# laurabragagnolo/SkelSplat

Hardware: AMD Instinct MI355X
Metric: rendered+backpropagated views/s (differentiable skeletal-Gaussian rasterizer fwd+bwd) (higher is better)
Workload: dtype f32

## Files before the change

include/skelsplat_hip.h:

```cpp
#ifndef SKELSPLAT_HIP_H
#define SKELSPLAT_HIP_H

#include <stddef.h>
#include <stdint.h>

#ifdef __cplusplus
extern "C" {
#endif

#define SKS_MAX_VIEWS 64
#define SKS_MAX_CHANNELS 32
#define SKS_SMALL_P 256

#define SKS_ANTIALIASING 1u
#define SKS_CLAMP01      2u
#define SKS_FORCE_BINNED 4u
#define SKS_DEBUG_SYNC   8u

#define SKS_NO_NT_STORES 16u

#define SKS_RAW_PARAMS   32u
#define SKS_RAW_GRADS    128u
#define SKS_BIN_CLEAN    64u
#define SKS_BIN_GROUPS_SHIFT 16
#define SKS_BIN_GROUPS(n) ((unsigned)(((n) - 1) & 7) << SKS_BIN_GROUPS_SHIFT)
#define SKS_FILL_LINEAR (1u << 21)
#define SKS_FILL_ROWS (1u << 22)
#define SKS_BWD_LDS_LIST (1u << 20)
#define SKS_BWD_WG_SHIFT 23
#define SKS_NO_EARLY_FILL (1u << 30)
#define SKS_EARLY_FILL(n) (((unsigned)(n) & 7u) << SKS_BIN_GROUPS_SHIFT)

const char* sks_last_error(void);
int sks_version(void);

int sks_scratch_bytes(int V, int P, int C, int W, int H, size_t bin_capacity,
                      size_t* geom_bytes, size_t* binning_bytes, size_t* accum_bytes);

#define SKS_REGIME_PATH        0
#define SKS_REGIME_COVER       1
#define SKS_REGIME_CW          2
#define SKS_REGIME_PPT         3
#define SKS_REGIME_HALF        4
#define SKS_REGIME_ROWMODE     5
#define SKS_REGIME_PB          6
#define SKS_REGIME_FSPLIT      7
#define SKS_REGIME_W_MAGIC     8
#define SKS_REGIME_BWD         9
#define SKS_REGIME_GX         10
#define SKS_REGIME_GY         11
#define SKS_REGIME_BPC        12
#define SKS_REGIME_WAVE_GROUPS 13
#define SKS_REGIME_LEAD       14
#define SKS_REGIME_INTS       16
int sks_launch_regime(int V, int P, int C, int W, int H, unsigned flags, int out_aligned128, int* out);

#define SKS_LIST_WAVE_SORT     0
#define SKS_LIST_WAVE_K        1
#define SKS_LIST_SORT_LDS      2
#define SKS_LIST_LONG_LIST     3
#define SKS_LIST_CLASSES       4
#define SKS_LIST_BAND_THREADS  5
#define SKS_LIST_REGIME_INTS   8
int sks_list_regime(int* out);

int sks_forward(int V, int P, int C, int W, int H,
                const float* viewmatrix, const float* projmatrix,
                const float* tanfovx , const float* tanfovy ,
                const float* means3D, const float* features, const float* opacities,
                const float* scales, const float* rotations, const float* cov3D_precomp,
                float scale_modifier, unsigned flags,
                float* out_color, float* out_invdepth, int* radii,
                void* geom, void* binning, size_t bin_capacity, int* num_rendered_dev,
                float* final_T, uint32_t* n_contrib, void* stream);

int sks_backward(int V, int P, int C, int W, int H,
                 const float* viewmatrix, const float* projmatrix,
                 const float* tanfovx , const float* tanfovy ,
                 const float* bg,
                 const float* means3D, const float* features, const float* opacities,
                 const float* scales, const float* rotations, const float* cov3D_precomp,
                 float scale_modifier, unsigned flags,
                 const int* radii, const void* geom, const void* binning, size_t bin_capacity,
                 const float* dL_dout_color, const float* dL_dout_invdepth,
                 void* accum,
                 float* dL_dmeans3D, float* dL_dmeans2D, float* dL_dopacity,
                 float* dL_dscales, float* dL_drotations, float* dL_dcov3D, float* dL_dfeatures,
                 float* dL_dmeans3D_mean ,
                 void* stream);

int sks_prefill_planes(int V, int P, int C, int W, int H, unsigned flags, int* planes_wave, int* planes_geom);
int sks_forward_prefilled(int V, int P, int C, int W, int H,
                          const float* viewmatrix, const float* projmatrix,
                          const float* tanfovx , const float* tanfovy ,
                          const float* means3D, const float* features, const float* opacities,
                          const float* scales, const float* rotations, const float* cov3D_precomp,
                          float scale_modifier, unsigned flags,
                          float* out_color, float* out_invdepth, int* radii,
                          void* geom, void* binning, size_t bin_capacity, int* num_rendered_dev,
                          float* final_T, uint32_t* n_contrib, int prefilled_planes, void* stream);
int sks_backward_prefill(int V, int P, int C, int W, int H,
                         const float* viewmatrix, const float* projmatrix,
                         const float* tanfovx , const float* tanfovy ,
                         const float* bg,
                         const float* means3D, const float* features, const float* opacities,
                         const float* scales, const float* rotations, const float* cov3D_precomp,
                         float scale_modifier, unsigned flags,
                         const int* radii, const void* geom, const void* binning, size_t bin_capacity,
                         const float* dL_dout_color, const float* dL_dout_invdepth,
                         void* accum,
                         float* dL_dmeans3D, float* dL_dmeans2D, float* dL_dopacity,
                         float* dL_dscales, float* dL_drotations, float* dL_dcov3D, float* dL_dfeatures,
                         float* dL_dmeans3D_mean,
                         float* next_color, float* next_invdepth, int planes_wave, int planes_geom, void* stream);

#define SKS_FB_NO_JOIN 1u
int sks_forward_backward(int V, int P, int C, int W, int H,
                         const float* viewmatrix, const float* projmatrix,
                         const float* tanfovx , const float* tanfovy ,
                         const float* means3D, const float* features, const float* opacities,
                         const float* scales, const float* rotations, const float* cov3D_precomp,
                         float scale_modifier, unsigned flags,
                         float* out_color, float* out_invdepth, int* radii,
                         void* geom, void* binning, size_t bin_capacity, int* num_rendered_dev,
                         const float* bg, const float* dL_dout_color, const float* dL_dout_invdepth, void* accum,
                         float* dL_dmeans3D, float* dL_dmeans2D, float* dL_dopacity,
                         float* dL_dscales, float* dL_drotations, float* dL_dcov3D, float* dL_dfeatures,
                         float* dL_dmeans3D_mean, void* stream, void* aux_stream, unsigned fb_flags);

int sks_mean_views(int V, int P, const float* dL_dmeans3D, int shard_world, float* mean_out , void* stream);

int sks_mark_visible(int P, const float* means3D, const float* viewmatrix, const float* projmatrix,
                     uint8_t* present, void* stream);

int sks_export_lists(int V, int W, int H, const void* binning, size_t bin_capacity,
                     uint32_t* point_list, uint32_t* ranges, void* stream);

int sks_masked_l2(int V, size_t n_per_view, const float* render, const float* gt, float* dL_unscaled, double* sums,
                  void* stream);
int sks_masked_l2_launch(size_t n_per_view, int* out );
int sks_masked_l2_loss(int V, size_t n_per_view, const float* render, const float* gt, float* dL_unscaled, double* sums,
                       float* loss , float* scale , int mean, void* stream);

#define SKS_SOFTARGMAX_STATS 6
size_t sks_softargmax_scratch_bytes(int planes, int W, int H);
int sks_softargmax_fwd(int planes, int W, int H, float beta, const float* img, float* xy ,
                       float* stats , void* scratch, size_t scratch_bytes, void* stream);
int sks_softargmax_bwd(int planes, int W, int H, float beta, const float* img, const float* stats ,
                       const float* dL_dxy , float* dL_dimg, void* stream);

int sks_heatmaps(int V, int J, int W, int H, const float* row, const float* col, const float* cmin, const float* den,
                 float* out, double* gt_totals, void* stream);
#define SKS_HEATMAP_MAX_RADIUS 262144
int sks_heatmap_factors(int V, int J, int W, int H, const float* means3D, const float* scales, const float* rotations,
                        float scale_modifier, const float* poses_2d, const float* viewmatrix, const float* tanfovx,
                        const float* tanfovy, float* row, float* col, float* cmin, float* den,
                        int frames ,
                        const int* view_wh ,
                        void* stream);
int sks_heatmap_totals(int V, int J, int W, int H, const float* row, const float* col, const float* cmin, const float* den,
                       const int* view_wh, double* gt_totals, void* stream);

int sks_triangulate(int N, int V, int J, const double* proj, size_t rig_stride, const float* poses_2d,
                    const double* poses_2d_f64, const unsigned char* valid, float* xyz, double* xyzw, int* n_used,
                    void* stream);

int sks_triangulate_robust(int N, int V, int J, const double* proj, size_t rig_stride, const float* poses_2d,
                           const double* poses_2d_f64, const unsigned char* valid, double reject_px, int min_inliers,
                           unsigned char* inliers, int* n_consensus, float* xyz, double* xyzw, int* n_used, void* stream);

int sks_fuse_predictions(int N, int V, int J, const double* proj, size_t rig_stride, const float* poses_3d,
                         const double* poses_3d_f64, const float* poses_2d, const double* poses_2d_f64,
                         const unsigned char* valid, int norm_f32, float* xyz, double* xyz_f64, double* reproj_err,
                         int* n_used, void* stream);

#define SKS_REFINE_MAX_ITERS 16
int sks_reproject(int N, int V, int J, const double* proj, size_t rig_stride, const float* xyz, const double* xyz_f64,
                  const float* poses_2d, const double* poses_2d_f64, const unsigned char* valid, double* uv, double* err,
                  unsigned char* in_front, double* per_joint, double* per_view, double* per_frame, int* n_used, void* stream);
int sks_eval_reprojection(int N, int V, int J, const double* err, const int* group_ids, int n_groups, double* out, void* stream);
int sks_triangulate_refine(int N, int V, int J, const double* proj, size_t rig_stride, const float* poses_2d,
                           const double* poses_2d_f64, const unsigned char* valid, const float* xyz0, const double* xyz0_f64,
                           double huber_px, int max_iters, float* xyz, double* xyz_f64, double* cost, int* iters, void* stream);

#define SKS_SMOOTH_MAX_JOINTS       256
#define SKS_SMOOTH_MAX_HALF_WINDOW  32
#define SKS_SMOOTH_BOX              0
#define SKS_SMOOTH_TRICUBE          1
#define SKS_SMOOTH_TILE       0
#define SKS_SMOOTH_GROUPS     1
#define SKS_SMOOTH_THREADS    2
#define SKS_SMOOTH_LDS_BYTES  3
#define SKS_SMOOTH_LAUNCH_INTS 4
int sks_smooth_sequence(int N, int J, const float* xyz, const float* cov6, const float* weights, const unsigned char* valid,
                        const int* group_ids, int half_window, int degree, int taper, double cov_floor, float* out_xyz,
                        float* out_vel, float* out_cov6, int* n_used, void* stream);
int sks_smooth_launch(int N, int J, int half_window, int* out );
int sks_eval_accel(int N, int J, const float* xyz, const float* gt, const int* group_ids, int n_groups, double* out, void* stream);

#define SKS_BONES_MAX_JOINTS   32
#define SKS_BONES_MAX_GROUPS   256
#define SKS_BONES_MAX_ITERS    16
#define SKS_BONES_MEASURE_GROUPS     0
#define SKS_BONES_MEASURE_THREADS    1
#define SKS_BONES_LENGTHS_GROUPS     2
#define SKS_BONES_LENGTHS_THREADS    3
#define SKS_BONES_LENGTHS_LDS_BYTES  4
#define SKS_BONES_PROJECT_GROUPS     5
#define SKS_BONES_PROJECT_THREADS    6
#define SKS_BONES_PROJECT_LDS_BYTES  7
#define SKS_BONES_LAUNCH_INTS        8
int sks_bone_measure(int N, int J, int B, const int* bones , const float* xyz, const float* cov6,
                     const unsigned char* valid, double max_sigma_mm, float* measured, void* stream);
int sks_bone_lengths(int N, int B, const float* measured, const int* groups, int n_groups, float* length, float* mad, int* n_used,
                     void* stream);
int sks_bone_project(int N, int J, int B, const int* bones , const float* xyz, const float* cov6,
                     const unsigned char* valid, const int* groups, int n_groups, const float* lengths, double cov_floor,
                     int max_iters, double tol_mm, float* out_xyz, float* residual, int* n_trips, int* n_active, void* stream);
int sks_bones_launch(int N, int J, int B, int n_groups, int* out );

int sks_fused_ssim_fwd(int B, int CH, int H, int W, float C1, float C2, const float* img1, const float* img2,
                       float* ssim_map, float* dm_dmu1, float* dm_dsigma1_sq, float* dm_dsigma12, void* stream);

int sks_fused_ssim_bwd(int B, int CH, int H, int W, float C1, float C2, const float* img1, const float* img2,
                       const float* dL_dmap, const float* dm_dmu1, const float* dm_dsigma1_sq, const float* dm_dsigma12,
                       float* dL_dimg1, void* stream);
int sks_fused_ssim_bwd_uniform(int B, int CH, int H, int W, const float* img1, const float* img2, const float* dL_value,
                               float dL_scale, int crop, const float* dm_dmu1, const float* dm_dsigma1_sq,
                               const float* dm_dsigma12, float* dL_dimg1, void* stream);
#define SKS_SSIM_SUM_SLOTS 64
#define SKS_SSIM_SCRATCH_BYTES (SKS_SSIM_SUM_SLOTS * 8)
int sks_fused_ssim_mean(int B, int CH, int H, int W, float C1, float C2, const float* img1, const float* img2, int crop,
                        float* dm_dmu1, float* dm_dsigma1_sq, float* dm_dsigma12, double* scratch, float* mean_out,
                        void* stream);

int sks_knn3_meandist2(int P, const float* points, float* mean_dist2, void* stream);
size_t sks_knn3_scratch_bytes(int P);
int sks_knn3_meandist2_grid(int P, const float* points, float* mean_dist2, void* scratch, size_t scratch_bytes, void* stream);

int sks_gt_tile_stats(int V, int C, int W, int H, const float* gt, float* tile_S, float* tile_N, double* totals, void* stream);
int sks_geometry(int V, int P, int C, int W, int H, const float* viewmatrix, const float* projmatrix,
                 const float* tanfovx , const float* tanfovy , const float* means3D,
                 const float* opacities, const float* scales, const float* rotations, const float* cov3D_precomp,
                 float scale_modifier, unsigned flags, int* radii, void* geom,
                 const int* view_wh , int frames ,
                 void* stream);
int sks_backward_fused_loss(int V, int P, int C, int W, int H, const float* viewmatrix, const float* projmatrix,
                            const float* tanfovx , const float* tanfovy , const float* bg,
                            const float* means3D, const float* features, const float* opacities, const float* scales,
                            const float* rotations, const float* cov3D_precomp, float scale_modifier, unsigned flags,
                            const int* radii, const void* geom, const float* gt, const float* tile_S, const float* tile_N,
                            const double* gt_totals, void* accum, float* dL_dmeans3D, float* dL_dmeans2D,
                            float* dL_dopacity, float* dL_dscales, float* dL_drotations, float* dL_dcov3D,
                            double* loss_sums, float* packed_raw_grads ,
                            const int* view_wh , const size_t* gt_offsets ,
                            const float* const* hm_factors , void* stream);

int sks_loop_pack_grads(int V, int P, const float* dL_dmeans3D, const float* dL_dscales, const float* dL_drotations,
                        const float* dL_dopacity, const float* raw_scaling, const float* raw_rotation,
                        const float* raw_opacity, const double* loss_sums, float* packed, void* stream);
int sks_loop_adam_step(int V, int P, const float* grads, float* slots, unsigned long long group_mask, int last_view,
                       float* xyz, float* scaling, float* rotation, float* opacity, float* exp_avg, float* exp_avg_sq,
                       int* counters, int acc_steps, const double* lr_sched ,
                       const double* lrs , const double* adam ,
                       float lambda_consistency, const int* limb ,
                       int shard_world ,
                       void* stream);
// ... 154 lines not shown
```

skelsplat_amd/_lib.py:

```python
import ctypes as C
import os

_HERE = os.path.dirname(os.path.abspath(__file__))
LIB_PATH = os.path.join(_HERE, "libskelsplat_hip.so")
_lib = None

SKS_MAX_VIEWS = 64
SKS_MAX_CHANNELS = 32
SKS_SMALL_P = 256
SKS_ANTIALIASING = 1
SKS_CLAMP01 = 2
SKS_FORCE_BINNED = 4
SKS_DEBUG_SYNC = 8
SKS_NO_NT_STORES = 16
SKS_RAW_PARAMS = 32
SKS_BIN_CLEAN = 64
SKS_RAW_GRADS = 128
SKS_FB_NO_JOIN = 1
SKS_BIN_GROUPS_SHIFT = 16
SKS_BWD_WG_SHIFT = 23
SKS_SSIM_SCRATCH_BYTES = 64 * 8
SKS_SOFTARGMAX_STATS = 6
SKS_REPORT_MAX_SAVES = 8
SKS_EVAL_MAX_GROUPS = 64
SKS_CALIBRATION_MAX_K = 8
SKS_REFINE_MAX_ITERS = 16
SKS_SMOOTH_MAX_JOINTS = 256
SKS_SMOOTH_MAX_HALF_WINDOW = 32
SKS_SMOOTH_BOX, SKS_SMOOTH_TRICUBE = 0, 1
SKS_SMOOTH_LAUNCH_INTS = 4
SKS_BONES_MAX_JOINTS = 32
SKS_BONES_MAX_GROUPS = 256
SKS_BONES_MAX_ITERS = 16
SKS_BONES_LAUNCH_INTS = 8
SKS_ALIGN_RIGID, SKS_ALIGN_SIMILARITY, SKS_ALIGN_SCALE = 0, 1, 2
SKS_PREVIEW_LAUNCH_INTS = 4
SKS_HEATMAP_MAX_RADIUS = 1 << 18


SKS_NO_EARLY_FILL = 1 << 30
SKS_BWD_LDS_LIST = 1 << 20
SKS_FILL_LINEAR = 1 << 21
SKS_FILL_ROWS = 1 << 22


def SKS_EARLY_FILL(n):
    return (int(n) & 7) << SKS_BIN_GROUPS_SHIFT


def SKS_BIN_GROUPS(n):
    return ((int(n) - 1) & 7) << SKS_BIN_GROUPS_SHIFT


_vp, _i, _u, _f, _sz = C.c_void_p, C.c_int, C.c_uint, C.c_float, C.c_size_t

_CAMERAS = (("V", _i), ("P", _i), ("C", _i), ("W", _i), ("H", _i), ("viewmatrix", _vp), ("projmatrix", _vp),
            ("tanfovx", _vp), ("tanfovy", _vp))
_GAUSSIANS = (("means3D", _vp), ("features", _vp), ("opacities", _vp), ("scales", _vp), ("rotations", _vp),
              ("cov3D_precomp", _vp), ("scale_modifier", _f), ("flags", _u))
_UPSTREAM = (("dL_dout_color", _vp), ("dL_dout_invdepth", _vp), ("accum", _vp))
_GRADS = (("dL_dmeans3D", _vp), ("dL_dmeans2D", _vp), ("dL_dopacity", _vp), ("dL_dscales", _vp), ("dL_drotations", _vp),
          ("dL_dcov3D", _vp), ("dL_dfeatures", _vp), ("dL_dmeans3D_mean", _vp))
_FORWARD_IO = (("out_color", _vp), ("out_invdepth", _vp), ("radii", _vp), ("geom", _vp), ("binning", _vp),
               ("bin_capacity", _sz), ("num_rendered_dev", _vp))
FORWARD_PARAMS = _CAMERAS + _GAUSSIANS + _FORWARD_IO + (("final_T", _vp), ("n_contrib", _vp), ("stream", _vp))
BACKWARD_PARAMS = _CAMERAS + (("bg", _vp),) + _GAUSSIANS + (("radii", _vp), ("geom", _vp), ("binning", _vp), ("bin_capacity", _sz)) \
    + _UPSTREAM + _GRADS + (("stream", _vp),)
FORWARD_PREFILLED_PARAMS = FORWARD_PARAMS[:-1] + (("prefilled_planes", _i), ("stream", _vp))
BACKWARD_PREFILL_PARAMS = BACKWARD_PARAMS[:-1] + (("next_color", _vp), ("next_invdepth", _vp), ("planes_wave", _i), ("planes_geom", _i),
                                                  ("stream", _vp))
FORWARD_BACKWARD_PARAMS = _CAMERAS + _GAUSSIANS + _FORWARD_IO + (("bg", _vp),) + _UPSTREAM + _GRADS \
    + (("stream", _vp), ("aux_stream", _vp), ("fb_flags", _u))

FWD, BWD, FWD_BWD = ({name: i for i, (name, _) in enumerate(params)}
                     for params in (FORWARD_PARAMS, BACKWARD_PARAMS, FORWARD_BACKWARD_PARAMS))
FWD_BWD_SOURCES = tuple(("fwd", FWD[n]) if n in FWD else ("bwd", BWD[n]) if n in BWD else None for n in FWD_BWD)

_ull = C.c_ulonglong
_VIEWS_DV = (("viewmatrix", _vp), ("projmatrix", _vp), ("views_dev", _vp))
RIG_SELECT_PARAMS = (("R", _i), ("V", _i), ("frames", _i), ("rig_ids", _vp), ("bank_viewmatrix", _vp), ("bank_projmatrix", _vp),
                     ("bank_tan", _vp), ("slot_wh", _vp), ("bank_proj", _vp), ("bank_sched", _vp), ("viewmatrix", _vp),
                     ("projmatrix", _vp), ("views_dev", _vp), ("proj", _vp), ("lr_sched_dev", _vp), ("error_word", _vp),
                     ("stream", _vp))
GEOMETRY_DV_PARAMS = (("V", _i), ("P", _i), ("C", _i), ("W", _i), ("H", _i)) + _VIEWS_DV + (
    ("means3D", _vp), ("opacities", _vp), ("scales", _vp), ("rotations", _vp), ("cov3D_precomp", _vp), ("scale_modifier", _f),
    ("flags", _u), ("radii", _vp), ("geom", _vp), ("frames", _i), ("stream", _vp))
HEATMAP_FACTORS_DV_PARAMS = (("V", _i), ("J", _i), ("W", _i), ("H", _i), ("means3D", _vp), ("scales", _vp), ("rotations", _vp),
                             ("scale_modifier", _f), ("poses_2d", _vp), ("viewmatrix", _vp), ("views_dev", _vp), ("row", _vp),
                             ("col", _vp), ("cmin", _vp), ("den", _vp), ("frames", _i), ("stream", _vp))
HEATMAP_TOTALS_DV_PARAMS = (("V", _i), ("J", _i), ("W", _i), ("H", _i), ("row", _vp), ("col", _vp), ("cmin", _vp), ("den", _vp),
                            ("views_dev", _vp), ("gt_totals", _vp), ("stream", _vp))
OPTIMISER_PARAMS = (("slots", _vp), ("group_mask", _ull), ("last_view", _i), ("xyz", _vp), ("scaling", _vp), ("rotation", _vp),
                    ("opacity", _vp), ("exp_avg", _vp), ("exp_avg_sq", _vp), ("counters", _vp), ("acc_steps", _i),
                    ("lr_sched", _vp), ("lrs", _vp), ("adam", _vp), ("lambda_consistency", _f), ("limb", _vp))
OPTIMISER_DV_PARAMS = tuple(("lr_sched_dev", ct) if name == "lr_sched" else (name, ct) for name, ct in OPTIMISER_PARAMS)
_ES = (("es_state", _vp), ("es_window", _i), ("es_tolerance", _f))
ES_PARAMS, ES_FRAMES_PARAMS = _ES + (("es_host_flag", _vp),), _ES + (("es_host_flags", _vp),)
_ADAM_STEP = (("V", _i), ("P", _i), ("grads", _vp)) + OPTIMISER_PARAMS + (("shard_world", _i),)
_STEP_RENDER = (("features", _vp), ("scale_modifier", _f), ("flags", _u), ("radii", _vp), ("geom", _vp), ("gt", _vp),
                ("gt_totals", _vp), ("accum", _vp), ("loss_sums", _vp), ("packed", _vp))
_STEP_HEATMAPS = (("view_wh", _vp), ("gt_offsets", _vp), ("frames", _i), ("hm_factors", _vp))
_STEP = _CAMERAS + _STEP_RENDER + OPTIMISER_PARAMS + _STEP_HEATMAPS
_STEP_DV = (("V", _i), ("P", _i), ("C", _i), ("W", _i), ("H", _i)) + _VIEWS_DV + _STEP_RENDER + OPTIMISER_DV_PARAMS + _STEP_HEATMAPS
LOOP_ADAM_STEP_PARAMS = _ADAM_STEP + (("stream", _vp),)
LOOP_ADAM_STEP_ES_PARAMS = _ADAM_STEP + (("loss_sums", _vp),) + ES_PARAMS + (("stream", _vp),)
LOOP_FUSED_STEP_PARAMS = _STEP + (("stream", _vp),)
LOOP_FUSED_STEP_ES_PARAMS = _STEP + ES_FRAMES_PARAMS + (("stream", _vp),)
LOOP_FUSED_STEP_DV_PARAMS = _STEP_DV + (("stream", _vp),)
LOOP_FUSED_STEP_ES_DV_PARAMS = _STEP_DV + ES_FRAMES_PARAMS + (("stream", _vp),)
STEP_PARAMS = {"sks_loop_adam_step": LOOP_ADAM_STEP_PARAMS, "sks_loop_adam_step_es": LOOP_ADAM_STEP_ES_PARAMS,
               "sks_loop_fused_step": LOOP_FUSED_STEP_PARAMS, "sks_loop_fused_step_es": LOOP_FUSED_STEP_ES_PARAMS}
DV_PARAMS = {"sks_rig_select": RIG_SELECT_PARAMS, "sks_geometry_dv": GEOMETRY_DV_PARAMS,
             "sks_heatmap_factors_dv": HEATMAP_FACTORS_DV_PARAMS, "sks_heatmap_totals_dv": HEATMAP_TOTALS_DV_PARAMS,
             "sks_loop_fused_step_dv": LOOP_FUSED_STEP_DV_PARAMS, "sks_loop_fused_step_es_dv": LOOP_FUSED_STEP_ES_DV_PARAMS}
VW_PARAMS = (("vw_mode", _i), ("vw_threshold", _f), ("vw_weights", _vp), ("vw_similarity", _vp))
VW_MODES = {None: 0, "scale": 1, "select": 2}
LOOP_ADAM_STEP_VW_PARAMS = LOOP_ADAM_STEP_ES_PARAMS[:-1] + VW_PARAMS + (("stream", _vp),)
LOOP_FUSED_STEP_VW_PARAMS = LOOP_FUSED_STEP_ES_PARAMS[:-1] + VW_PARAMS + (("stream", _vp),)
LOOP_FUSED_STEP_VW_DV_PARAMS = LOOP_FUSED_STEP_ES_DV_PARAMS[:-1] + VW_PARAMS + (("stream", _vp),)
VW_STEP_PARAMS = {"sks_loop_adam_step_vw": LOOP_ADAM_STEP_VW_PARAMS, "sks_loop_fused_step_vw": LOOP_FUSED_STEP_VW_PARAMS,
                  "sks_loop_fused_step_vw_dv": LOOP_FUSED_STEP_VW_DV_PARAMS}


def vw_mode(view_weighting):
    if view_weighting not in VW_MODES:
        raise ValueError(f"view_weighting = {view_weighting!r}: expected None, 'scale' or 'select'")
    return VW_MODES[view_weighting]


SIGNATURES = {
    "sks_last_error": (C.c_char_p, []),
    "sks_version": (_i, []),
    "sks_scratch_bytes": (_i, [_i, _i, _i, _i, _i, _sz, C.POINTER(_sz), C.POINTER(_sz), C.POINTER(_sz)]),
    "sks_launch_regime": (_i, [_i, _i, _i, _i, _i, _u, _i, C.POINTER(_i)]),
    "sks_list_regime": (_i, [C.POINTER(_i)]),
    "sks_forward": (_i, [ct for _, ct in FORWARD_PARAMS]),
    "sks_backward": (_i, [ct for _, ct in BACKWARD_PARAMS]),
    "sks_forward_backward": (_i, [ct for _, ct in FORWARD_BACKWARD_PARAMS]),
    "sks_forward_prefilled": (_i, [ct for _, ct in FORWARD_PREFILLED_PARAMS]),
    "sks_backward_prefill": (_i, [ct for _, ct in BACKWARD_PREFILL_PARAMS]),
    "sks_prefill_planes": (_i, [_i, _i, _i, _i, _i, _u, C.POINTER(_i), C.POINTER(_i)]),
    "sks_mark_visible": (_i, [_i, _vp, _vp, _vp, _vp, _vp]),
    "sks_mean_views": (_i, [_i, _i, _vp, _i, _vp, _vp]),
    "sks_export_lists": (_i, [_i, _i, _i, _vp, _sz, _vp, _vp, _vp]),
    "sks_masked_l2": (_i, [_i, _sz, _vp, _vp, _vp, _vp, _vp]),
    "sks_masked_l2_launch": (_i, [_sz, C.POINTER(_i)]),
    "sks_masked_l2_loss": (_i, [_i, _sz, _vp, _vp, _vp, _vp, _vp, _vp, _i, _vp]),
    "sks_fused_ssim_fwd": (_i, [_i, _i, _i, _i, _f, _f, _vp, _vp, _vp, _vp, _vp, _vp, _vp]),
    "sks_fused_ssim_bwd": (_i, [_i, _i, _i, _i, _f, _f, _vp, _vp, _vp, _vp, _vp, _vp, _vp, _vp]),
    "sks_fused_ssim_bwd_uniform": (_i, [_i, _i, _i, _i, _vp, _vp, _vp, _f, _i, _vp, _vp, _vp, _vp, _vp]),
    "sks_fused_ssim_mean": (_i, [_i, _i, _i, _i, _f, _f, _vp, _vp, _i, _vp, _vp, _vp, _vp, _vp, _vp]),
    "sks_knn3_meandist2": (_i, [_i, _vp, _vp, _vp]),
    "sks_knn3_scratch_bytes": (_sz, [_i]),
    "sks_knn3_meandist2_grid": (_i, [_i, _vp, _vp, _vp, _sz, _vp]),
    "sks_softargmax_scratch_bytes": (_sz, [_i, _i, _i]),
    "sks_softargmax_fwd": (_i, [_i, _i, _i, _f, _vp, _vp, _vp, _vp, _sz, _vp]),
    "sks_softargmax_bwd": (_i, [_i, _i, _i, _f, _vp, _vp, _vp, _vp, _vp]),
    "sks_heatmaps": (_i, [_i, _i, _i, _i, _vp, _vp, _vp, _vp, _vp, _vp, _vp]),
    "sks_heatmap_factors": (_i, [_i, _i, _i, _i, _vp, _vp, _vp, _f, _vp, _vp, _vp, _vp, _vp, _vp, _vp, _vp, _i, _vp, _vp]),
    "sks_heatmap_totals": (_i, [_i, _i, _i, _i, _vp, _vp, _vp, _vp, _vp, _vp, _vp]),
    "sks_gt_tile_stats": (_i, [_i, _i, _i, _i, _vp, _vp, _vp, _vp, _vp]),
    "sks_geometry": (_i, [_i, _i, _i, _i, _i, _vp, _vp, _vp, _vp, _vp, _vp, _vp, _vp, _vp, _f, _u, _vp, _vp, _vp, _i, _vp]),
    "sks_backward_fused_loss": (_i, [_i, _i, _i, _i, _i, _vp, _vp, _vp, _vp, _vp, _vp, _vp, _vp, _vp, _vp, _vp, _f, _u,
                                     _vp, _vp, _vp, _vp, _vp, _vp, _vp, _vp, _vp, _vp, _vp, _vp, _vp, _vp, _vp, _vp, _vp, _vp, _vp]),
    "sks_loop_pack_grads": (_i, [_i, _i, _vp, _vp, _vp, _vp, _vp, _vp, _vp, _vp, _vp, _vp]),
    "sks_loop_shard_floats": (_sz, [_i, _i, _i]),
    "sks_adam_multi": (_i, [_i, _vp, _vp, _vp, _vp, _vp, _vp, _vp, C.c_double, C.c_double, C.c_double, _vp]),
    "sks_triangulate": (_i, [_i, _i, _i, _vp, _sz, _vp, _vp, _vp, _vp, _vp, _vp, _vp]),
    "sks_triangulate_robust": (_i, [_i, _i, _i, _vp, _sz, _vp, _vp, _vp, C.c_double, _i, _vp, _vp, _vp, _vp, _vp, _vp]),
    "sks_fuse_predictions": (_i, [_i, _i, _i, _vp, _sz, _vp, _vp, _vp, _vp, _vp, _i, _vp, _vp, _vp, _vp, _vp]),
    "sks_reproject": (_i, [_i, _i, _i, _vp, _sz, _vp, _vp, _vp, _vp, _vp, _vp, _vp, _vp, _vp, _vp, _vp, _vp, _vp]),
    "sks_eval_reprojection": (_i, [_i, _i, _i, _vp, _vp, _i, _vp, _vp]),
    "sks_triangulate_refine": (_i, [_i, _i, _i, _vp, _sz, _vp, _vp, _vp, _vp, _vp, C.c_double, _i, _vp, _vp, _vp, _vp, _vp]),
    "sks_smooth_sequence": (_i, [_i, _i, _vp, _vp, _vp, _vp, _vp, _i, _i, _i, C.c_double, _vp, _vp, _vp, _vp, _vp]),
    "sks_smooth_launch": (_i, [_i, _i, _i, _vp]),
    "sks_eval_accel": (_i, [_i, _i, _vp, _vp, _vp, _i, _vp, _vp]),
    "sks_bone_measure": (_i, [_i, _i, _i, _vp, _vp, _vp, _vp, C.c_double, _vp, _vp]),
    "sks_bone_lengths": (_i, [_i, _i, _vp, _vp, _i, _vp, _vp, _vp, _vp]),
    "sks_bone_project": (_i, [_i, _i, _i, _vp, _vp, _vp, _vp, _vp, _i, _vp, C.c_double, _i, C.c_double, _vp, _vp, _vp, _vp, _vp]),
    "sks_bones_launch": (_i, [_i, _i, _i, _i, _vp]),
    **{name: (_i, [ct for _, ct in params]) for name, params in {**STEP_PARAMS, **DV_PARAMS, **VW_STEP_PARAMS}.items()},
    "sks_pose_errors": (_i, [_i, _i, _vp, _vp, _vp, _vp, _vp]),
    "sks_loop_report": (_i, [_i, _i, _i, _vp, _vp, _i, _vp, _vp, _vp, _i, _i, _vp, _vp, _vp, _i, _vp, _vp, _vp]),
    "sks_eval_sequence": (_i, [_i, _i, _vp, _vp, _vp, _i, _vp, _vp, _vp]),
    "sks_joint_uncertainty": (_i, [_i, _i, _vp, _vp, _vp, _f, _vp, _vp, _vp, _vp, _vp]),
    "sks_view_footprints": (_i, [_i, _i, _i, _i, _vp, _vp, _vp, _f, _vp, _vp, _vp, _vp, _vp, _i, _vp, _vp]),
    "sks_calibration": (_i, [_i, _i, _vp, _vp, _i, _vp, _vp, _vp]),
    "sks_align_poses": (_i, [_i, _i, _vp, _vp, _vp, _i, _vp, _vp, _vp, _vp, _vp]),
    "sks_eval_sequence_aligned": (_i, [_i, _i, _vp, _vp, _vp, _vp, _i, _vp, _sz, _vp, _vp]),
    "sks_eval_sequence_aligned_scratch_bytes": (_sz, [_i, _i]),
    "sks_preview_planes": (_i, [_i, _i, _i, _i, _vp, _vp, _vp, _vp, _vp]),
    "sks_preview_factors": (_i, [_i, _i, _i, _i, _vp, _vp, _vp, _vp, _vp, _vp, _vp, _vp, _vp]),
    "sks_preview_scratch_bytes": (_sz, [_i, _i, _i]),
    "sks_preview_launch": (_i, [_i, _i, _i, _vp]),
    "sks_prof_enable": (_i, [_i]),
    "sks_prof_spin": (_i, [C.c_double, _vp]),
    "sks_prof_read": (_i, [_i, C.POINTER(C.c_double), C.POINTER(C.c_longlong)]),
    "sks_prof_count": (_i, [_i, C.POINTER(C.c_longlong)]),
    "sks_prof_read_quantiles": (_i, [_i, C.POINTER(C.c_double), C.POINTER(C.c_double), C.POINTER(C.c_longlong)]),
}


_PREFILL_SYMBOLS = ("sks_forward_prefilled", "sks_backward_prefill", "sks_prefill_planes")
HAS_PREFILL = True


def load(build_if_missing=True):
    global _lib
    if _lib is not None:
        return _lib
    if build_if_missing:
        try:
            from . import build as _b
            if _b._stale():
                _b.build()
        except Exception as e:
            if not os.path.exists(LIB_PATH):
                raise ImportError(f"libskelsplat_hip.so is missing and could not be built: {e}") from e
    if not os.path.exists(LIB_PATH):
        raise ImportError(f"{LIB_PATH} not found; run `python -m skelsplat_amd.build`")
    override = os.environ.get("SKS_LIB_OVERRIDE")
    lib = C.CDLL(override or LIB_PATH)
    global HAS_PREFILL
    for name, (res, args) in SIGNATURES.items():
        if override and name in _PREFILL_SYMBOLS and not hasattr(lib, name):
            HAS_PREFILL = False
            continue
        if override and name in VW_STEP_PARAMS and not hasattr(lib, name):
            continue
        fn = getattr(lib, name)
        fn.restype = res
        fn.argtypes = args
    _lib = lib
    return lib


def check(rc, what):
    if rc != 0:
        msg = load().sks_last_error().decode(errors="replace")
        raise RuntimeError(f"{what} failed (code {rc}): {msg}")


def scratch_bytes(V, P, C_, W, H, bin_capacity=0):
    g, b, a = _sz(0), _sz(0), _sz(0)
    check(load().sks_scratch_bytes(V, P, C_, W, H, bin_capacity, C.byref(g), C.byref(b), C.byref(a)), "sks_scratch_bytes")
    return g.value, b.value, a.value


REGIME_FIELDS = ("path", "cover", "cw", "ppt", "half", "rowmode", "pb", "fsplit", "w_magic", "bwd", "gx", "gy", "bpc", "wave_groups",
                 "lead")
REGIME_INTS = 16
PATH_SMALL, PATH_BINNED = 0, 1
COVER_NONE, COVER_PER_VIEW, COVER_PER_PLANE = 0, 1, 2
BWD_WAVE, BWD_GATHER, BWD_TILE = 0, 1, 2


def launch_regime(V, P, C_, W, H, flags=0, out_aligned128=True):
    out = (_i * REGIME_INTS)()
    check(load().sks_launch_regime(V, P, C_, W, H, flags, 1 if out_aligned128 else 0, out), "sks_launch_regime")
    return {name: out[i] for i, name in enumerate(REGIME_FIELDS)}


LIST_REGIME_FIELDS = ("wave_sort", "wave_k", "sort_lds", "long_list", "classes", "band_threads")
LIST_REGIME_INTS = 8


def list_regime():
    out = (_i * LIST_REGIME_INTS)()
    check(load().sks_list_regime(out), "sks_list_regime")
    return {name: out[i] for i, name in enumerate(LIST_REGIME_FIELDS)}


def masked_l2_launch(n_per_view):
    out = (_i * 2)()
    check(load().sks_masked_l2_launch(n_per_view, out), "sks_masked_l2_launch")
    return out[0], out[1]


PREVIEW_LAUNCH_FIELDS = ("load_bytes", "store_bytes", "groups_sum", "groups_pack")


def preview_launch(W, H, aligned=True):
    out = (_i * SKS_PREVIEW_LAUNCH_INTS)()
    check(load().sks_preview_launch(W, H, 1 if aligned else 0, C.cast(out, _vp)), "sks_preview_launch")
    return {name: out[i] for i, name in enumerate(PREVIEW_LAUNCH_FIELDS)}


SMOOTH_LAUNCH_FIELDS = ("tile", "groups", "threads", "lds_bytes")


def smooth_launch(N, J, half_window):
    out = (_i * SKS_SMOOTH_LAUNCH_INTS)()
    check(load().sks_smooth_launch(N, J, half_window, C.cast(out, _vp)), "sks_smooth_launch")
    return {name: out[i] for i, name in enumerate(SMOOTH_LAUNCH_FIELDS)}


BONES_LAUNCH_FIELDS = ("measure_groups", "measure_threads", "lengths_groups", "lengths_threads", "lengths_lds_bytes",
                       "project_groups", "project_threads", "project_lds_bytes")


def bones_launch(N, J, B, n_groups=1):
    out = (_i * SKS_BONES_LAUNCH_INTS)()
    check(load().sks_bones_launch(N, J, B, n_groups, C.cast(out, _vp)), "sks_bones_launch")
    return {name: out[i] for i, name in enumerate(BONES_LAUNCH_FIELDS)}


def prefill_planes(V, P, C_, W, H, flags=0):
    nw, ng = _i(0), _i(0)
    check(load().sks_prefill_planes(V, P, C_, W, H, flags, C.byref(nw), C.byref(ng)), "sks_prefill_planes")
    return nw.value, ng.value


def ptr(t):
    if t is None or t.numel() == 0:
        return None
    return t.data_ptr()


def farray(vals):
    return (C.c_float * len(vals))(*[float(v) for v in vals])


def prof_count(kind):
    n = C.c_longlong(0)
    check(load().sks_prof_count(kind, C.byref(n)), "sks_prof_count")
    return n.value


def prof_enable(on, every=1, kinds=(0, 1), recorded=False):
    skip = sum(1 << (16 + k) for k in (0, 1) if k not in kinds)
    check(load().sks_prof_enable((min(0xffff, max(1, int(every))) | skip | ((1 << 18) if recorded else 0)) if on else 0),
          "sks_prof_enable")


def prof_read_quantiles(kind):
    q = (C.c_double * 3)()
    ms, n = C.c_double(0), C.c_longlong(0)
    check(load().sks_prof_read_quantiles(kind, q, C.byref(ms), C.byref(n)), "sks_prof_read_quantiles")
    return ms.value, n.value, (q[0], q[1], q[2])


def prof_read(kind):
    ms, n = C.c_double(0), C.c_longlong(0)
    check(load().sks_prof_read(kind, C.byref(ms), C.byref(n)), "sks_prof_read")
    return ms.value, n.value
```

skelsplat_amd/csrc/sks_common.inc:

```
thread_local char g_err[512] = "";

int fail(int code, const char* fmt, ...)
{
    va_list ap;
    va_start(ap, fmt);
    vsnprintf(g_err, sizeof(g_err), fmt, ap);
    va_end(ap);
    return code;
}

#define HIP_TRY(expr)                                                                          \
    do {                                                                                       \
        hipError_t e_ = (expr);                                                                \
        if (e_ != hipSuccess) return fail((int)e_, "%s: %s", #expr, hipGetErrorString(e_));    \
    } while (0)

#define STAGE_CHECK(name)                                                                      \
    do {                                                                                       \
        HIP_TRY(hipGetLastError());                                                            \
        if (flags & SKS_DEBUG_SYNC) {                                                          \
            hipError_t e_ = hipStreamSynchronize(st);                                          \
            if (e_ != hipSuccess) return fail((int)e_, "stage %s: %s", name, hipGetErrorString(e_)); \
        }                                                                                      \
    } while (0)

constexpr int PROF_MAX = 16384;
struct ProfKind {
    hipEvent_t b[PROF_MAX], e[PROF_MAX];
    int created = 0, n = 0;
    hipEvent_t xb[PROF_MAX], xe[PROF_MAX];
    bool hasx[PROF_MAX];
    int xcreated = 0;
};
struct ProfState {
    bool on = false;
    int every = 1;
    int skip = 0;
    bool recorded = false;
    int seen[2] = { 0, 0 };
    ProfKind kind[2];
    hipEvent_t park_b = nullptr, park_e = nullptr;
    bool parked = false;
    hipStream_t park_st = nullptr;
};
thread_local ProfState* tl_prof = nullptr;

struct ProfScope {
    ProfKind* k = nullptr;
    hipStream_t st;
    bool ext;
    bool began = false;
    ProfScope(int kind, hipStream_t s, bool ext_ = false, bool take_parked = false) : st(s), ext(ext_)
    {
        ProfState* ps = tl_prof;
        if (!ps) return;
        const bool parked = kind == 0 && ps->parked && take_parked && ps->park_st == s;
        if (kind == 0) ps->parked = false;
        if (!ps->on || ((ps->skip >> kind) & 1)) return;
        if (ps->seen[kind]++ % ps->every != 0) return;
        ProfKind& p = ps->kind[kind];
        if (p.n >= PROF_MAX) return;
        if (p.n >= p.created) {
            if (hipEventCreate(&p.b[p.created]) != hipSuccess || hipEventCreate(&p.e[p.created]) != hipSuccess) return;
            p.created++;
        }
        p.hasx[p.n] = false;
        if (parked) {
            while (p.xcreated <= p.n) {
                if (hipEventCreate(&p.xb[p.xcreated]) != hipSuccess || hipEventCreate(&p.xe[p.xcreated]) != hipSuccess) return;
                p.xcreated++;
            }
            hipEvent_t t = p.xb[p.n]; p.xb[p.n] = ps->park_b; ps->park_b = t;
            t = p.xe[p.n]; p.xe[p.n] = ps->park_e; ps->park_e = t;
            p.hasx[p.n] = true;
        }
        k = &p;
        if (ps->recorded) ext = false;
        if (!ext) (void)hipEventRecord(p.b[p.n], st);
    }
    hipEvent_t eb() const { return k->b[k->n]; }
    hipEvent_t ee() const { return k->e[k->n]; }
    ~ProfScope()
    {
        if (!k) return;
        if (!ext) (void)hipEventRecord(k->e[k->n], st);
        k->n++;
    }
};
inline bool prof_next_forward_sampled()
{
    const ProfState* ps = tl_prof;
    return ps && ps->on && !(ps->skip & 1) && ps->seen[0] % ps->every == 0 && ps->kind[0].n < PROF_MAX;
}
inline bool prof_has_parked(hipStream_t st) { return tl_prof && tl_prof->parked && tl_prof->park_st == st; }
inline void prof_park_begin(hipStream_t st)
{
    ProfState* ps = tl_prof;
    ps->parked = false;
    if (!ps->park_b && (hipEventCreate(&ps->park_b) != hipSuccess || hipEventCreate(&ps->park_e) != hipSuccess)) { ps->park_b = ps->park_e = nullptr; return; }
    ps->park_st = st;
    ps->parked = hipEventRecord(ps->park_b, st) == hipSuccess;
}
inline void prof_park_end(hipStream_t st)
{
    ProfState* ps = tl_prof;
    if (ps && ps->parked && ps->park_st == st && hipEventRecord(ps->park_e, st) != hipSuccess) ps->parked = false;
}
inline hipError_t prof_elapsed(ProfKind& p, int i, float* ms)
{
    hipError_t e = hipEventSynchronize(p.e[i]);
    if (e == hipSuccess) e = hipEventElapsedTime(ms, p.b[i], p.e[i]);
    if (e == hipSuccess && p.hasx[i]) {
        float x = 0;
        e = hipEventSynchronize(p.xe[i]);
        if (e == hipSuccess) e = hipEventElapsedTime(&x, p.xb[i], p.xe[i]);
        *ms += x;
    }
    return e;
}
#define SKS_LAUNCH(prof, kernel, grid, block, lds, stream, ...)                                                  \
    do {                                                                                                         \
        if ((prof).k)                                                                                            \
            hipExtLaunchKernelGGL(kernel, grid, block, lds, stream, (prof).began ? nullptr : (prof).eb(), (prof).ee(), 0, __VA_ARGS__); \
        else hipLaunchKernelGGL(kernel, grid, block, lds, stream, __VA_ARGS__);                                  \
    } while (0)
#define SKS_LAUNCH_FIRST(prof, kernel, grid, block, lds, stream, ...)                                            \
    do {                                                                                                         \
        if ((prof).k && (prof).ext) hipExtLaunchKernelGGL(kernel, grid, block, lds, stream, (prof).eb(), nullptr, 0, __VA_ARGS__); \
        else hipLaunchKernelGGL(kernel, grid, block, lds, stream, __VA_ARGS__);    \
        (prof).began = (prof).k != nullptr;                                                                      \
    } while (0)

constexpr int NACC = 8;
constexpr int BWD_SPLITS = 16;
constexpr int BWD_WG_PAIRS16 = 400;
constexpr int BWD_WG_PAIRS8 = 4096;

struct ViewTan {
    float x[SKS_MAX_VIEWS];
    float y[SKS_MAX_VIEWS];
    int w[SKS_MAX_VIEWS];
    int h[SKS_MAX_VIEWS];
};
struct ViewOff {
    unsigned long long off[SKS_MAX_VIEWS];
};
struct ViewTanDev {
    const float* x;
    const float* y;
    const int* w;
    const int* h;
    const double* sched;
};
inline ViewTanDev views_dev_from(const void* views_dev, const double* sched = nullptr)
{
    const ViewTan* t = (const ViewTan*)views_dev;
    return ViewTanDev{ t->x, t->y, t->w, t->h, sched };
}
inline bool fill_views(ViewTan& vt, ViewOff* vo, int V, int C, int W, int H, const float* tanfovx, const float* tanfovy,
                       const int* view_wh, const size_t* plane_off)
{
    for (int v = 0; v < V; v++) {
        vt.x[v] = tanfovx[v];
        vt.y[v] = tanfovy[v];
        vt.w[v] = view_wh ? view_wh[2 * v] : W;
        vt.h[v] = view_wh ? view_wh[2 * v + 1] : H;
        if (vt.w[v] < 1 || vt.h[v] < 1 || vt.w[v] > W || vt.h[v] > H) return false;
        if (vo) vo->off[v] = plane_off ? (unsigned long long)plane_off[v] : (unsigned long long)v * C * H * W;
    }
    return true;
}

struct Geom {
    float4* co;
    float4* xyd;
    uint4* rect;
    uint32_t* cover;
};

__host__ __device__ inline size_t align256(size_t x) { return (x + 255) & ~(size_t)255; }

struct Activated {
    float opacity, s[3], q[4], qnorm;
};
__device__ __forceinline__ Activated activate(bool raw, float op, const float s[3], const float q[4])
{
    Activated a;
    if (raw) {
        a.opacity = 1.0f / (1.0f + expf_fixed(-op));
#pragma unroll
        for (int k = 0; k < 3; k++) a.s[k] = expf_fixed(s[k]);
        const float nn = q[0] * q[0] + q[1] * q[1] + q[2] * q[2] + q[3] * q[3];
        a.qnorm = fmaxf(sqrtf(nn), 1e-12f);
#pragma unroll
        for (int k = 0; k < 4; k++) a.q[k] = q[k] / a.qnorm;
    } else {
        a.opacity = op;
        a.qnorm = 1.0f;
#pragma unroll
        for (int k = 0; k < 3; k++) a.s[k] = s[k];
#pragma unroll
        for (int k = 0; k < 4; k++) a.q[k] = q[k];
    }
    return a;
}

#ifndef SKS_COVER_MAX_WORDS
#define SKS_COVER_MAX_WORDS 6144
#endif
constexpr int COVER_MAX_WORDS = SKS_COVER_MAX_WORDS;
__host__ __device__ inline int cover_cw(int W) { return (1 + (((W + TILE - 1) / TILE) + 31) / 32 + 3) & ~3; }
inline bool cover_enabled(int P, int W, int H)
{
    return P <= SKS_SMALL_P && ((H + TILE - 1) / TILE) * cover_cw(W) <= COVER_MAX_WORDS;
}
inline bool cover_per_plane(int P, int W, int H, int C)
{
    return cover_enabled(P, W, H) && (C + 1) * ((H + TILE - 1) / TILE) * cover_cw(W) <= COVER_MAX_WORDS;
}
inline Geom geom_from(void* base, int V, int P, int W, int H)
{
    char* p = (char*)base;
    Geom g;
    size_t n = (size_t)V * P;
    g.co = (float4*)p; p += align256(n * sizeof(float4));
    g.xyd = (float4*)p; p += align256(n * sizeof(float4));
    g.rect = (uint4*)p; p += align256(n * sizeof(uint4));
    g.cover = cover_enabled(P, W, H) ? (uint32_t*)p : nullptr;
    return g;
}
inline size_t geom_bytes(int V, int P, int W, int H, int C)
{
    const int planes = cover_per_plane(P, W, H, C) ? C + 1 : 1;
    return 3 * align256((size_t)V * P * 16) + align256((size_t)V * planes * ((H + TILE - 1) / TILE) * cover_cw(W) * 4);
}

constexpr int BIN_WAVE_SORT = 64;
constexpr int WSORT_K = 4;
constexpr int SORT_LDS = 2048;
constexpr int LONG_LIST = 256;
constexpr int BIN_ROWS = 2;
constexpr int BIN_CLASSES = 8;
constexpr int BIN_HDR_CLASS = 8;
constexpr int BIN_MAX_GROUPS = 7;
#ifndef SKS_BIN_FB_GROUPS
#define SKS_BIN_FB_GROUPS 1
#endif
constexpr int BIN_FB_GROUPS = SKS_BIN_FB_GROUPS;
inline int bin_groups_default()
{
    static const int n = [] {
        const char* e = getenv("SKS_BIN_GROUPS");
        const int want = (e && atoi(e) > 0) ? atoi(e) : BIN_FB_GROUPS;
        return want < 1 ? 1 : (want > BIN_MAX_GROUPS ? BIN_MAX_GROUPS : want);
    }();
    return n;
}
inline void bin_groups(unsigned flags, int V, int& vg, int& ng)
{
    const unsigned field = (flags >> SKS_BIN_GROUPS_SHIFT) & 7u;
// ... 60 lines not shown
```

skelsplat_amd/csrc/sks_fwd_small.inc:

```
__device__ __forceinline__ float clamp01(float x) { return fminf(fmaxf(x, 0.0f), 1.0f); }

struct FwdArgs {
    int P, C, W, H;
    unsigned flags;
    Geom g;
    const float* features;
    float* out_color;
    float* out_invdepth;
    float* final_T;
    uint32_t* n_contrib;
    int tslots;
    unsigned cp1_magic;
    int ncomp;
    int cover_planes;
    unsigned w_magic;
};

inline int composite_slots(unsigned flags, int V, int P)
{
    const int t = (int)((flags >> 26) & 15u);
    return t ? t : ((long long)V * P <= 128 ? 4 : 8);
}

typedef float v4f __attribute__((ext_vector_type(4)));
// ... 256 lines not shown
            if (tid == 0) { s_n = 0; s_min = 0x7fffffff; }
            __syncthreads();
            if (tid < P) {
                const uint4 r = L.rect[tid];
                if ((int)r.x <= tx && tx < (int)r.z && (int)r.y <= ty && ty < (int)r.w) {
                    atomicMin(&s_min, tid);
                    const int sl = atomicAdd(&s_n, 1);
                    L.key[sl] = ((unsigned long long)__float_as_uint(gxyd[tid].z) << 32) | (unsigned)tid;
                }
            }
            __syncthreads();
            const int n = s_n;
            if (s_min == g) {
                if (tid < n) {
                    const unsigned long long key = L.key[tid];
                    int rank = 0;
                    for (int j = 0; j < n; j++) rank += (L.key[j] < key) ? 1 : 0;
                    const int id = (int)(unsigned)key;
                    const float4 xyd = gxyd[id];
                    L.xy[rank] = make_float2(xyd.x, xyd.y);
                    L.co[rank] = gco[id];
                    L.invd[rank] = xyd.w;
#pragma unroll
                    for (int ch = 0; ch < CG; ch++) L.feat[rank * CG + ch] = ch < C ? a.features[id * C + ch] : 0.0f;
                }
                __syncthreads();
                unsigned chm = 0xffffffffu;
                if (a.cover_planes) {
                    bool nz = false;
                    if (tid < CG)
                        for (int k = 0; k < n; k++) nz = nz || L.feat[k * CG + tid] != 0.0f;
                    if (tid < 64) {
                        const unsigned long long bl = __ballot(nz);
                        if (tid == 0) s_chm = (unsigned)bl;
                    }
                    __syncthreads();
                    chm = s_chm;
                }
                const int x = tx * TILE + (tid & 15), y = ty * TILE + (tid >> 4);
                if (x < W && y < H) {
                    const float pxf = (float)x, pyf = (float)y;
                    float T = 1.0f, inv = 0.0f, acc[CG];
#pragma unroll
                    for (int ch = 0; ch < CG; ch++) acc[ch] = 0.0f;
                    uint32_t contributor = 0, last = 0;
                    for (int k = 0; k < n; k++) {
                        contributor++;
                        const float2 xy = L.xy[k];
                        const float4 co = L.co[k];
                        const float dx = xy.x - pxf, dy = xy.y - pyf;
                        const float power = -0.5f * (co.x * dx * dx + co.z * dy * dy) - co.y * dx * dy;
                        if (power > 0.0f) continue;
                        const float alpha = fminf(0.99f, co.w * expf_fixed(power));
                        if (alpha < 1.0f / 255.0f) continue;
                        const float test_T = T * (1 - alpha);
                        if (test_T < 0.0001f) break;
#pragma unroll
                        for (int ch = 0; ch < CG; ch++) acc[ch] += L.feat[k * CG + ch] * alpha * T;
                        inv += L.invd[k] * alpha * T;
                        T = test_T;
                        last = contributor;
                    }
                    const size_t pix = (size_t)y * W + x;
#pragma unroll
                    for (int ch = 0; ch < CG; ch++)
                        if (ch < C && ((chm >> ch) & 1u)) outc[(size_t)ch * HW + pix] = do_clamp ? clamp01(acc[ch]) : acc[ch];
                    outi[pix] = inv;
                    if (a.final_T) a.final_T[(size_t)v * HW + pix] = T;
                    if (a.n_contrib) a.n_contrib[(size_t)v * HW + pix] = last;
                }
            }
            __syncthreads();
        }
        return;
    }
    fwd_fill_role<PPT, NT, HALF>(a, cp1_magic, xq, band_id, zid, gy, pb, cover);
}

struct EarlyFill {
    float* out_color;
    float* out_invdepth;
    int C, W, H, gy;
    int gplanes;
    int ngeom;
    int zid0;
    int fsplit, pb;
    unsigned cp1_magic;
    unsigned row_magic;
    unsigned fs_magic;
};

template <int PPT, bool NT>
__global__ __launch_bounds__(256) void k_geom_fwd_fill(EarlyFill f, int P, ViewTan vt, const float* __restrict__ vms,
                                                       const float* __restrict__ pms, const float* __restrict__ means,
                                                       const float* __restrict__ opac, const float* __restrict__ scales,
                                                       const float* __restrict__ rots, const float* __restrict__ cov3Dp, float smod,
                                                       unsigned flags, Geom g, int* __restrict__ radii,
                                                       const float* __restrict__ features, int cover_planes)
{
    const int b = blockIdx.x;
    if (b < f.ngeom) {
        const int v = f.gplanes == 1 ? b : (int)(((unsigned)b * f.cp1_magic) >> 20);
        extern __shared__ __attribute__((aligned(16))) char s_dyn[];
        geom_fwd_block((uint32_t*)s_dyn, 0, v, b - v * f.gplanes, P, f.W, f.H, vt, vms, pms, means, opac, scales, rots, cov3Dp, smod, flags, g, radii, 0,
                       nullptr, nullptr, features, f.C, nullptr, nullptr, cover_planes);
        return;
    }
    const unsigned e = (unsigned)(b - f.ngeom);
    const unsigned rows = (unsigned)(f.fsplit * f.gy);
    const unsigned zr = f.row_magic ? __umulhi(e, f.row_magic) : e;
    const unsigned rem = e - zr * rows;
    const int band = (int)(f.fs_magic ? __umulhi(rem, f.fs_magic) : rem);
    const int q = (int)rem - band * f.fsplit;
    const int zid = f.zid0 + (int)zr;
    const int v = (int)(((unsigned)zid * f.cp1_magic) >> 20);
    const int plane = zid - v * (f.C + 1);
    const size_t HW = (size_t)f.H * f.W;
    const int Nb = min(TILE, f.H - band * TILE) * f.W;
    float* out = (plane == f.C ? f.out_invdepth + (size_t)v * HW : f.out_color + ((size_t)v * f.C + plane) * HW) + (size_t)band * TILE * f.W;
    const int shift = (int)((reinterpret_cast<uintptr_t>(out) >> 2) & 31u);
    fill_bare<PPT, NT>(out, nullptr, nullptr, q * (256 * PPT) * f.pb + (int)threadIdx.x * PPT - shift, Nb, min(f.pb, 32));
}

struct PreFill {
    float* out_color;
    float* out_invdepth;
    int C, W, H, gy;
    int zid0;
    unsigned nfill;
    int fsplit, pb;
    int zs;
    unsigned cp1_magic;
    unsigned row_magic;
    unsigned fs_magic;
};

__device__ __forceinline__ void prefill_block(const PreFill& f, unsigned e)
{
    if (e >= f.nfill) return;
    const unsigned rows = (unsigned)(f.fsplit * f.gy);
    const unsigned zr = f.row_magic ? __umulhi(e, f.row_magic) : e;
    const unsigned rem = e - zr * rows;
    const int band = (int)(f.fs_magic ? __umulhi(rem, f.fs_magic) : rem);
    const int q = (int)rem - band * f.fsplit;
    const int zid = f.zid0 + (int)zr;
    const int v = (int)(((unsigned)zid * f.cp1_magic) >> 20);
    const int plane = zid - v * (f.C + 1);
    const size_t HW = (size_t)f.H * f.W;
    const int Nb = min(TILE, f.H - band * TILE) * f.W;
    float* out = (plane == f.C ? f.out_invdepth + (size_t)v * HW : f.out_color + ((size_t)v * f.C + plane) * HW) + (size_t)band * TILE * f.W;
    const int shift = (int)((reinterpret_cast<uintptr_t>(out) >> 2) & 31u);
    fill_bare<4, true>(out, nullptr, nullptr, q * 1024 * f.pb + (int)threadIdx.x * 4 - shift, Nb, min(f.pb, 32));
}
```

skelsplat_amd/csrc/sks_geom_fwd.inc:

```
template <class VT>
__device__ __forceinline__ uint4 geom_fwd_one(int P, const VT& vt, const float* __restrict__ vms,
                                              const float* __restrict__ pms, const float* __restrict__ means,
                                              const float* __restrict__ opac, const float* __restrict__ scales,
                                              const float* __restrict__ rots, const float* __restrict__ cov3Dp,
                                              float smod, unsigned flags, const Geom& g, int* __restrict__ radii,
                                              int v, int idx, bool live, bool store = true)
{
    const size_t o = (size_t)v * P + (live ? idx : 0);
    const float* V = vms + 16 * v;
    const float* PM = pms + 16 * v;
    const float tan_fovx = vt.x[v], tan_fovy = vt.y[v];
    const int W = vt.w[v], H = vt.h[v];
    const float focal_y = H / (2.0f * tan_fovy);
    const float focal_x = W / (2.0f * tan_fovx);
    const int gx = (W + TILE - 1) / TILE, gy = (H + TILE - 1) / TILE;

    int radius_out = 0;
    uint4 rect = make_uint4(0, 0, 0, 0);
    float4 co = make_float4(0, 0, 0, 0), xyd = make_float4(0, 0, 1.0f, 1.0f);

    const int li = live ? idx : 0;
    const float p_orig[3] = { means[3 * li], means[3 * li + 1], means[3 * li + 2] };
    float p_view[3];
    transformPoint4x3(p_orig, V, p_view);
    const bool culled = !(p_view[2] > 0.2f);
    if (live && !culled) {
        float p_hom[4];
        transformPoint4x4(p_orig, PM, p_hom);
        const float p_w = 1.0f / (p_hom[3] + 0.0000001f);
        const float p_proj[3] = { p_hom[0] * p_w, p_hom[1] * p_w, p_hom[2] * p_w };
        float cov3D[6];
        if (cov3Dp) {
#pragma unroll
            for (int i = 0; i < 6; i++) cov3D[i] = cov3Dp[6 * li + i];
        } else {
            const float s[3] = { scales[3 * li], scales[3 * li + 1], scales[3 * li + 2] };
            const float q[4] = { rots[4 * li], rots[4 * li + 1], rots[4 * li + 2], rots[4 * li + 3] };
            const Activated ac = activate(flags & SKS_RAW_PARAMS, 0.0f, s, q);
            computeCov3D(ac.s, smod, ac.q, cov3D);
        }
        Cov2D c;
        cov2d(p_orig, focal_x, focal_y, tan_fovx, tan_fovy, cov3D, V, c);
        float cov_x = c.cov.m[0][0], cov_y = c.cov.m[0][1], cov_z = c.cov.m[1][1];
        constexpr float h_var = 0.3f;
        const float det_cov = cov_x * cov_z - cov_y * cov_y;
        cov_x += h_var;
        cov_z += h_var;
        const float det_cov_plus_h_cov = cov_x * cov_z - cov_y * cov_y;
        float h_convolution_scaling = 1.0f;
        if (flags & SKS_ANTIALIASING) h_convolution_scaling = sqrtf(fmaxf(0.000025f, det_cov / det_cov_plus_h_cov));
        const float det = det_cov_plus_h_cov;
        if (det != 0.0f) {
            const float det_inv = 1.f / det;
            const float conic[3] = { cov_z * det_inv, -cov_y * det_inv, cov_x * det_inv };
            const float mid = 0.5f * (cov_x + cov_z);
            const float lambda1 = mid + sqrtf(fmaxf(0.1f, mid * mid - det));
            const float lambda2 = mid - sqrtf(fmaxf(0.1f, mid * mid - det));
            const float my_radius = ceilf(3.f * sqrtf(fmaxf(lambda1, lambda2)));
            const float px = ndc2Pix(p_proj[0], W), py = ndc2Pix(p_proj[1], H);
            int xmin, ymin, xmax, ymax;
            getRect(px, py, (int)my_radius, gx, gy, xmin, ymin, xmax, ymax);
            if ((xmax - xmin) * (ymax - ymin) != 0) {
                radius_out = (int)my_radius;
                rect = make_uint4(xmin, ymin, xmax, ymax);
                const float op_raw = opac[li];
                const float op = (flags & SKS_RAW_PARAMS) ? 1.0f / (1.0f + expf_fixed(-op_raw)) : op_raw;
                co = make_float4(conic[0], conic[1], conic[2], op * h_convolution_scaling);
                xyd = make_float4(px, py, p_view[2], 1 / p_view[2]);
            }
        }
    }
    if (live && store) {
        radii[o] = radius_out;
        g.co[o] = co;
        g.xyd[o] = xyd;
        g.rect[o] = rect;
    }
    return rect;
}

#ifndef SKS_GEOM_COVER_THREADS
#define SKS_GEOM_COVER_THREADS 256
#endif
__device__ __forceinline__ void geom_fwd_block(uint32_t* s_cov, int bx, int v, int pz, int P, int W, int H, const ViewTan& vt, const float* __restrict__ vms,
                                               const float* __restrict__ pms, const float* __restrict__ means,
                                               const float* __restrict__ opac, const float* __restrict__ scales,
                                               const float* __restrict__ rots, const float* __restrict__ cov3Dp,
                                               float smod, unsigned flags, const Geom& g, int* __restrict__ radii, int vf,
                                               uint32_t* __restrict__ count, uint32_t* __restrict__ touched,
                                               const float* __restrict__ features, int C,
                                               uint2* __restrict__ fmask, uint32_t* __restrict__ bin_hdr, int cover_planes)
{
    const int idx = bx * blockDim.x + threadIdx.x;
    const bool live = idx < P;
    if (vf > 0) {
        const int fr = v / vf;
        means += (size_t)fr * P * 3;
        opac += (size_t)fr * P;
        if (scales) scales += (size_t)fr * P * 3;
        if (rots) rots += (size_t)fr * P * 4;
        if (cov3Dp) cov3Dp += (size_t)fr * P * 6;
    }
    const uint4 rect = geom_fwd_one(P, vt, vms, pms, means, opac, scales, rots, cov3Dp, smod, flags, g, radii, v, idx, live, pz == 0);
    if (bin_hdr && bx == 0 && v == 0 && pz == 0 && threadIdx.x < 64) bin_hdr[threadIdx.x] = 0u;
    if (count) {
        const int wt = (int)(rect.z - rect.x), n = wt * (int)(rect.w - rect.y);
        if (live) touched[(size_t)v * P + idx] = (uint32_t)n;
        if (live && v == 0) {
            unsigned fm = 0u;
            float f0 = 0.0f;
            for (int ch = C - 1; ch >= 0; ch--) {
                const float f = features[(size_t)idx * C + ch];
                if (f != 0.0f) { fm |= 1u << ch; f0 = f; }
            }
            fmask[idx] = make_uint2(fm, __float_as_uint(f0));
        }
    }
    if (g.cover) {
        const int gy = (H + TILE - 1) / TILE;
        const int cw = cover_cw(W), pw = gy * cw;
        for (int i = threadIdx.x; i < pw; i += blockDim.x) s_cov[i] = 0u;
        __syncthreads();
        bool mine = live && rect.z > rect.x && rect.w > rect.y;
        if (mine && cover_planes && pz < C) mine = features[(size_t)idx * C + pz] != 0.0f;
        if (mine) {
#pragma nounroll
            for (unsigned y = rect.y; y < rect.w; y++) {
                atomicOr(&s_cov[y * cw], 1u);
#pragma nounroll
                for (unsigned w0 = rect.x >> 5; w0 <= (rect.z - 1u) >> 5; w0++) {
                    const unsigned lo = max(rect.x, w0 << 5) & 31u, hi = min(rect.z - 1u, (w0 << 5) + 31u) & 31u;
                    atomicOr(&s_cov[y * cw + 1 + w0], (0xffffffffu >> (31u - hi)) & (0xffffffffu << lo));
                }
            }
        }
        __syncthreads();
        uint32_t* out = g.cover + ((size_t)v * (cover_planes ? C + 1 : 1) + (cover_planes ? pz : 0)) * pw;
        for (int i = threadIdx.x; i < pw; i += blockDim.x) out[i] = s_cov[i];
    }
}

__global__ __launch_bounds__(SKS_GEOM_COVER_THREADS > 256 ? SKS_GEOM_COVER_THREADS : 256) void k_geom_fwd(int P, int W, int H, ViewTan vt, const float* __restrict__ vms,
                                                   const float* __restrict__ pms, const float* __restrict__ means,
                                                   const float* __restrict__ opac, const float* __restrict__ scales,
                                                   const float* __restrict__ rots, const float* __restrict__ cov3Dp,
                                                   float smod, unsigned flags, Geom g, int* __restrict__ radii, int vf,
                                                   uint32_t* __restrict__ count = nullptr, uint32_t* __restrict__ touched = nullptr,
                                                   const float* __restrict__ features = nullptr, int C = 0,
                                                   uint2* __restrict__ fmask = nullptr, uint32_t* __restrict__ bin_hdr = nullptr,
                                                   int cover_planes = 0)
{
    __shared__ uint32_t s_cov[COVER_MAX_WORDS];
    geom_fwd_block(s_cov, blockIdx.x, blockIdx.y, blockIdx.z, P, W, H, vt, vms, pms, means, opac, scales, rots, cov3Dp, smod, flags, g, radii, vf,
                   count, touched, features, C, fmask, bin_hdr, cover_planes);
}

__global__ __launch_bounds__(256) void k_geom_fwd_dv(int P, ViewTanDev vt, const float* __restrict__ vms, const float* __restrict__ pms,
                                                      const float* __restrict__ means, const float* __restrict__ opac,
                                                      const float* __restrict__ scales, const float* __restrict__ rots,
                                                      const float* __restrict__ cov3Dp, float smod, unsigned flags, Geom g,
                                                      int* __restrict__ radii, int vf)
{
    const int idx = blockIdx.x * 256 + threadIdx.x;
    const int v = blockIdx.y;
    if (vf > 0) {
        const int fr = v / vf;
        means += (size_t)fr * P * 3;
        opac += (size_t)fr * P;
        if (scales) scales += (size_t)fr * P * 3;
        if (rots) rots += (size_t)fr * P * 4;
        if (cov3Dp) cov3Dp += (size_t)fr * P * 6;
    }
    geom_fwd_one(P, vt, vms, pms, means, opac, scales, rots, cov3Dp, smod, flags, g, radii, v, idx, idx < P);
}

__global__ void k_mark_visible(int P, const float* __restrict__ means, const float* __restrict__ V,
                               uint8_t* __restrict__ present)
{
    const int idx = blockIdx.x * 256 + threadIdx.x;
    if (idx >= P) return;
    const float p[3] = { means[3 * idx], means[3 * idx + 1], means[3 * idx + 2] };
    float pv[3];
    transformPoint4x3(p, V, pv);
    const bool culled = !(pv[2] > 0.2f);
    present[idx] = !culled;
}
```

skelsplat_amd/csrc/sks_raster.hip:

```cpp
#include <hip/hip_runtime.h>
#include <hip/hip_ext.h>
#include <stdarg.h>
#include <stdlib.h>
#include <stdio.h>
#include <string.h>
#include <initializer_list>
#include <type_traits>

#include "../../include/skelsplat_hip.h"
#include "sks_math.h"
#include "sks_loop_dev.h"

using namespace sks;

namespace {

#include "sks_common.inc"
#include "sks_geom_fwd.inc"
#include "sks_fwd_small.inc"
#include "sks_bwd_small.inc"
#include "sks_geom_bwd.inc"
#include "sks_binned.inc"

inline int pick_cg(int C) { return C <= 4 ? 4 : C <= 16 ? 16 : C <= 20 ? 20 : 32; }
// ... 99 lines not shown
void launch_fwd_small(const FwdArgs& a_in, int V, int gy, int zfill, hipStream_t st, const ProfScope& prof)
{
    FwdArgs a = a_in;
    const int ncomp = a.tslots * a.P * V;
    a.ncomp = ncomp;
    int fsplit, pb;
    fill_geometry(a, a.g.cover != nullptr, false, fsplit, pb);
    if (zfill == 0) fsplit = 0;
    const int rows_zy = (zfill > 0 ? zfill : 1) * gy;
    const int xc = (ncomp + rows_zy - 1) / rows_zy;
    const int cap = (a.P + 15) & ~15;
    const size_t lds = DynList<CG>::bytes(cap, CG);
    dim3 grid(fsplit + xc, gy, zfill > 0 ? zfill : 1);
    const bool nt = !(a.flags & SKS_NO_NT_STORES);
    if (a.W % 4 == 0) {
        if (nt) SKS_LAUNCH(prof, (k_render_fwd_sparse<CG, 4, true>), grid, dim3(256), lds, st, a, a.cp1_magic, gy, fsplit, pb, (const uint32_t*)a.g.cover);
        else SKS_LAUNCH(prof, (k_render_fwd_sparse<CG, 4, false>), grid, dim3(256), lds, st, a, a.cp1_magic, gy, fsplit, pb, (const uint32_t*)a.g.cover);
    } else if (fill_half_mode(a)) {
        SKS_LAUNCH(prof, (k_render_fwd_sparse<CG, 4, true, true>), grid, dim3(256), lds, st, a, a.cp1_magic, gy, fsplit, pb, (const uint32_t*)a.g.cover);
    } else {
        SKS_LAUNCH(prof, (k_render_fwd_sparse<CG, 1, false>), grid, dim3(256), lds, st, a, a.cp1_magic, gy, fsplit, pb, (const uint32_t*)a.g.cover);
    }
}

#ifndef SKS_EARLY_FILL_BYTES
#define SKS_EARLY_FILL_BYTES (36u << 20)
#endif
inline int early_fill_planes(unsigned flags, int planes, size_t plane_bytes)
{
    const int field = (int)((flags >> SKS_BIN_GROUPS_SHIFT) & 7u);
    if (field == 7) return planes;
    if (field) return (planes * field + 15) / 16;
    const size_t want = ((size_t)SKS_EARLY_FILL_BYTES + plane_bytes / 2) / plane_bytes;
    return (int)(want < (size_t)(planes / 4) ? want : (size_t)(planes / 4));
}

inline unsigned magic32(unsigned d) { return (unsigned)(((1ull << 32) + d - 1) / d); }

bool early_fill_cut(const FwdArgs& a_in, int V, int gy, int gplanes, int zid0, int zid1, int& fsplit, int& pb)
{
    FwdArgs a = a_in;
    a.flags |= SKS_FILL_LINEAR;
    fill_geometry(a, true, false, fsplit, pb);
    const long long rows = (long long)fsplit * gy, nfill = rows * (zid1 - zid0);
    return fsplit >= 1 && pb >= 1 && nfill * rows < (1ll << 32) && (long long)V * gplanes + nfill < (1ll << 31);
}

void launch_geom_fill(const FwdArgs& a, const FwdCall& c, int gy, int gplanes, int zid0, int zid1, int fsplit, int pb, const ViewTan& vt,
                      ProfScope& prof)
{
    const hipStream_t st = c.stream;
    const long long rows = (long long)fsplit * gy, nfill = rows * (zid1 - zid0);
    const int ngeom = c.cam.V * gplanes;
    const EarlyFill f{ a.out_color, a.out_invdepth, a.C, a.W, a.H, gy, gplanes, ngeom, zid0, fsplit, pb, a.cp1_magic,
                       rows > 1 ? magic32((unsigned)rows) : 0u, fsplit > 1 ? magic32((unsigned)fsplit) : 0u };
    const dim3 grid((unsigned)(ngeom + nfill));
    const size_t lds = (size_t)gy * cover_cw(a.W) * 4;
    const bool nt = !(a.flags & SKS_NO_NT_STORES);
    const int ppt = (a.W % 4 == 0 || fill_half_mode(a)) ? 4 : 1;
#define SKS_GF_ARGS f, a.P, vt, c.cam.viewmatrix, c.cam.projmatrix, c.g.means3D, c.g.opacities, c.g.scales, c.g.rotations, c.g.cov3D_precomp, \
                    c.g.scale_modifier, a.flags, a.g, c.io.radii, a.features, a.cover_planes
    if (ppt == 4 && nt) SKS_LAUNCH_FIRST(prof, (k_geom_fwd_fill<4, true>), grid, dim3(256), lds, st, SKS_GF_ARGS);
    else if (ppt == 4) SKS_LAUNCH_FIRST(prof, (k_geom_fwd_fill<4, false>), grid, dim3(256), lds, st, SKS_GF_ARGS);
    else SKS_LAUNCH_FIRST(prof, (k_geom_fwd_fill<1, false>), grid, dim3(256), lds, st, SKS_GF_ARGS);
#undef SKS_GF_ARGS
}

#ifndef SKS_GEOM_BINNED_THREADS
#define SKS_GEOM_BINNED_THREADS 256
#endif
void launch_geom_fwd(const FwdCall& c, const ViewTan& vt, const Geom& g, const Bin& b, bool small, int gplanes, hipEvent_t done)
{
    const Cameras& cam = c.cam;
    const int gthreads = small ? 256 : SKS_GEOM_BINNED_THREADS;
    const dim3 grid((cam.P + gthreads - 1) / gthreads, cam.V, gplanes);
#define SKS_G_ARGS cam.P, cam.W, cam.H, vt, cam.viewmatrix, cam.projmatrix, c.g.means3D, c.g.opacities, c.g.scales, c.g.rotations, c.g.cov3D_precomp, \
                   c.g.scale_modifier, c.g.flags, g, c.io.radii, 0, b.count, b.touched, c.g.features, cam.C, b.fmask, b.hdr,                          \
                   (small && cover_per_plane(cam.P, cam.W, cam.H, cam.C)) ? 1 : 0
    if (done) hipExtLaunchKernelGGL(k_geom_fwd, grid, dim3(gthreads), 0, c.stream, nullptr, done, 0, SKS_G_ARGS);
    else hipLaunchKernelGGL(k_geom_fwd, grid, dim3(gthreads), 0, c.stream, SKS_G_ARGS);
#undef SKS_G_ARGS
}

template <int CG>
void launch_fwd_binned(const FwdArgs& a, const BinView& bv, int V, int gx, int gy, const uint32_t* cover, hipStream_t st)
{
    int fsplit, pb;
    fill_geometry(a, true, true, fsplit, pb);
    const int xc = ((gx + TGROUP - 1) / TGROUP + a.C) / (a.C + 1);
    dim3 grid(fsplit + xc, gy, (a.C + 1) * V);
    const bool nt = !(a.flags & SKS_NO_NT_STORES);
    if (a.W % 4 == 0) {
        if (nt) hipLaunchKernelGGL((k_render_fwd_binned<CG, 4, true>), grid, dim3(256), 0, st, a, bv, gx, gy, fsplit, pb, cover);
        else hipLaunchKernelGGL((k_render_fwd_binned<CG, 4, false>), grid, dim3(256), 0, st, a, bv, gx, gy, fsplit, pb, cover);
    } else if (fill_half_mode(a)) {
        hipLaunchKernelGGL((k_render_fwd_binned<CG, 4, true, true>), grid, dim3(256), 0, st, a, bv, gx, gy, fsplit, pb, cover);
    } else {
        hipLaunchKernelGGL((k_render_fwd_binned<CG, 1, false>), grid, dim3(256), 0, st, a, bv, gx, gy, fsplit, pb, cover);
    }
}

inline int bin_scan_bands(int gx) { return gx >= SCAN_T * 8 ? 1 : (SCAN_T * 8) / gx; }

inline int bwd_tile_blocks()
{
    static const int n = [] {
        int dev = 0, cus = 256;
        if (hipGetDevice(&dev) == hipSuccess) {
            hipDeviceProp_t pr;
            if (hipGetDeviceProperties(&pr, dev) == hipSuccess && pr.multiProcessorCount > 0) cus = pr.multiProcessorCount;
        }
        const char* e = getenv("SKS_BWD_TILE_BLOCKS");
        return (e && atoi(e) > 0) ? atoi(e) : cus * BWD_TILE_BLOCKS_PER_CU;
    }();
    return n;
}

inline int bwd_wave_groups(int V, int P, unsigned flags)
{
    unsigned t = (flags >> SKS_BWD_WG_SHIFT) & 7u;
    static const int env = [] { const char* e = getenv("SKS_BWD_WG"); return e ? atoi(e) : 0; }();
    if (!t && env > 0) t = (unsigned)env;
    if (t) return t > 5 ? 1 : (BWD_SPLITS >> (t - 1));
    const int pairs = V * P;
    return pairs <= BWD_WG_PAIRS16 ? 16 : (pairs <= BWD_WG_PAIRS8 ? 8 : 4);
}

template <bool ES = false>
inline void launch_bwd_loss(const BwdArgs& a, const ViewTan& vt, const ViewOff& vo, int V, hipStream_t st)
{
    const dim3 grid(a.P, V, bwd_wave_groups(V, a.P, a.flags));
    if (a.hm_row) with_cg(a.C, [&](auto cg) { hipLaunchKernelGGL((k_render_bwd_wave<decltype(cg)::value, false, true, true, ES>), grid, dim3(256), 0, st, a, vt, vo); });
    else with_cg(a.C, [&](auto cg) { hipLaunchKernelGGL((k_render_bwd_wave<decltype(cg)::value, false, true, false, ES>), grid, dim3(256), 0, st, a, vt, vo); });
}

struct PrefillReq {
    float* color;
    float* invdepth;
    int planes_wave, planes_geom;
};
#ifndef SKS_PREFILL_PASSES
#define SKS_PREFILL_PASSES 2
#endif
inline int prefill_passes()
{
    static const int n = [] { const char* e = getenv("SKS_PREFILL_PB"); return (e && atoi(e) > 0) ? atoi(e) : SKS_PREFILL_PASSES; }();
    return n > 32 ? 32 : n;
}
inline bool prefill_possible(int P, int W, int H, unsigned flags)
{
    return P >= 1 && P <= 64 && is_small(P, flags) && !(flags & (SKS_NO_NT_STORES | SKS_DEBUG_SYNC | SKS_BWD_LDS_LIST)) &&
           (W % 4 == 0 || (W % 4 == 2 && H % 2 == 0));
}
bool prefill_cut(PreFill& f, float* color, float* invdepth, int V, int C, int W, int H, int zid0, int nz, long long per_unit, long long max_units)
{
    const int gy = TileGrid(W, H).gy;
    const int passes = (TILE * W + fill_lead(color, invdepth, W, H) + 1023) / 1024;
    const int pb = prefill_passes();
    const int fsplit = (passes + pb - 1) / pb;
    const long long rows = (long long)fsplit * gy, nfill = rows * nz;
    if (zid0 < 0 || nz < 1 || zid0 + nz > (C + 1) * V || nfill * rows >= (1ll << 32) || (nfill + per_unit - 1) / per_unit > max_units) return false;
    f = PreFill{ color, invdepth, C, W, H, gy, zid0, (unsigned)nfill, fsplit, pb, 0, ((1u << 20) + (unsigned)C) / (unsigned)(C + 1),
                 rows > 1 ? magic32((unsigned)rows) : 0u, fsplit > 1 ? magic32((unsigned)fsplit) : 0u };
    return true;
}

inline bool bwd_small_wave(int P, unsigned flags) { return P <= 64 && !(flags & SKS_BWD_LDS_LIST); }

template <int CG>
void launch_bwd_small(const BwdArgs& a, const ViewTan& vt, const ViewOff& vo, int V, bool dfeat, hipStream_t st, const ProfScope& prof,
                      const PreFill* pf = nullptr)
{
    if (bwd_small_wave(a.P, a.flags)) {
        dim3 grid(a.P, V, bwd_wave_groups(V, a.P, a.flags));
        if (pf) {
            PreFill f = *pf;
            f.zs = (int)grid.z;
            grid.z += (unsigned)((f.nfill + (unsigned)(a.P * V) - 1) / (unsigned)(a.P * V));
            if (dfeat) SKS_LAUNCH(prof, (k_render_bwd_wave<CG, true, false, false, false, PreFill>), grid, dim3(256), 0, st, a, vt, vo, f);
            else SKS_LAUNCH(prof, (k_render_bwd_wave<CG, false, false, false, false, PreFill>), grid, dim3(256), 0, st, a, vt, vo, f);
            return;
        }
        if (dfeat) SKS_LAUNCH(prof, (k_render_bwd_wave<CG, true, false>), grid, dim3(256), 0, st, a, vt, vo);
        else SKS_LAUNCH(prof, (k_render_bwd_wave<CG, false, false>), grid, dim3(256), 0, st, a, vt, vo);
        return;
    }
    dim3 grid(a.P, V, BWD_SPLITS);
    const size_t lds = GatherLds<CG>::bytes((a.P + 15) & ~15, CG, a.C);
    if (lds > 48 * 1024) {
        (void)hipFuncSetAttribute(reinterpret_cast<const void*>(&k_render_bwd_gather<CG, true>),
                                  hipFuncAttributeMaxDynamicSharedMemorySize, (int)lds);
        (void)hipFuncSetAttribute(reinterpret_cast<const void*>(&k_render_bwd_gather<CG, false>),
                                  hipFuncAttributeMaxDynamicSharedMemorySize, (int)lds);
    }
    if (dfeat) SKS_LAUNCH(prof, (k_render_bwd_gather<CG, true>), grid, dim3(256), lds, st, a);
    else SKS_LAUNCH(prof, (k_render_bwd_gather<CG, false>), grid, dim3(256), lds, st, a);
}

__global__ void k_spin_us(unsigned long long ticks)
{
    const unsigned long long t0 = wall_clock64();
    while (wall_clock64() - t0 < ticks) __builtin_amdgcn_s_sleep(8);
}

struct FwdHook {
    hipEvent_t geom_done;
    int (*after_geom)(void* ctx);
    int (*after_group)(void* ctx, int g, int v0, int nv);
    void* ctx;
};
constexpr int FB_MAX_EVENTS = BIN_MAX_GROUPS;
constexpr int FB_OVERLAP_MAX_PAIRS = BWD_WG_PAIRS16;
struct FbEvents {
    hipEvent_t geom = nullptr, done = nullptr;
    hipEvent_t grp[FB_MAX_EVENTS] = {};
    int dev = -1;
};
thread_local FbEvents tl_fb_events;
int fb_events(int ngroups, FbEvents*& out)
{
    FbEvents& ev = tl_fb_events;
    int cur_dev = 0;
    HIP_TRY(hipGetDevice(&cur_dev));
    if (ev.geom && ev.dev != cur_dev) {
        (void)hipEventDestroy(ev.geom);
        (void)hipEventDestroy(ev.done);
        for (hipEvent_t& e : ev.grp)
            if (e) { (void)hipEventDestroy(e); e = nullptr; }
        ev.geom = ev.done = nullptr;
    }
    unsigned evf = hipEventDisableTiming | hipEventDisableSystemFence;
    if (const char* e = getenv("SKS_FB_EVENT_FLAGS")) evf = (unsigned)strtoul(e, nullptr, 0);
    if (!ev.geom) {
        ev.dev = cur_dev;
        HIP_TRY(hipEventCreateWithFlags(&ev.geom, evf));
        HIP_TRY(hipEventCreateWithFlags(&ev.done, evf));
    }
    for (int gi = 0; gi < ngroups && gi < FB_MAX_EVENTS; gi++)
        if (!ev.grp[gi]) HIP_TRY(hipEventCreateWithFlags(&ev.grp[gi], evf));
    out = &ev;
    return 0;
}

}

extern "C" {

const char* sks_last_error(void) { return g_err; }
void sks_set_error_(const char* msg)
{
    snprintf(g_err, sizeof(g_err), "%s", msg);
}
int sks_version(void) { return 14; }

int sks_scratch_bytes(int V, int P, int C, int W, int H, size_t bin_capacity, size_t* geom, size_t* binning, size_t* accum)
{
    if (int rc = check_common(V, P, C, W, H)) return rc;
    const TileGrid t(W, H);
    if (geom) *geom = geom_bytes(V, P > 0 ? P : 1, W, H, C);
    if (binning) *binning = bin_bytes(V, P, t.NT, bin_capacity, C + 1, (size_t)t.gy * cover_cw(W));
    if (accum) *accum = (size_t)V * (P > 0 ? P : 1) * BWD_SPLITS * (NACC + C) * sizeof(float);
    return 0;
}

int sks_launch_regime(int V, int P, int C, int W, int H, unsigned flags, int out_aligned128, int* out)
{
    if (int rc = check_common(V, P, C, W, H)) return rc;
    if (!out) return fail(-2, "sks_launch_regime: out must be provided");
    const TileGrid t(W, H);
    const bool small = is_small(P, flags);
    const bool cover = small && cover_enabled(P, W, H), per_plane = cover && cover_per_plane(P, W, H, C);
    FwdArgs a{};
    a.P = P, a.C = C, a.W = W, a.H = H, a.flags = flags;
    a.out_color = a.out_invdepth = (float*)(uintptr_t)(out_aligned128 ? 128 : 16);
    int fsplit = 0, pb = 0;
    fill_geometry(a, small ? cover : true, !small, fsplit, pb);
    const int ppt = (W % 4 == 0 || fill_half_mode(a)) ? 4 : 1;
    memset(out, 0, SKS_REGIME_INTS * sizeof(int));
    out[SKS_REGIME_PATH] = small ? 0 : 1;
    out[SKS_REGIME_COVER] = small ? (per_plane ? 2 : cover ? 1 : 0) : 2;
    out[SKS_REGIME_CW] = cover_cw(W);
    out[SKS_REGIME_PPT] = ppt;
    out[SKS_REGIME_HALF] = fill_half_mode(a) ? 1 : 0;
    out[SKS_REGIME_ROWMODE] = pb < 0 ? 1 : 0;
    out[SKS_REGIME_PB] = pb < 0 ? -pb : pb;
    out[SKS_REGIME_FSPLIT] = fsplit;
    out[SKS_REGIME_W_MAGIC] = fill_w_magic(W) ? 1 : 0;
    out[SKS_REGIME_BWD] = !small ? 2 : bwd_small_wave(P, flags) ? 0 : 1;
    out[SKS_REGIME_GX] = t.gx;
    out[SKS_REGIME_GY] = t.gy;
    out[SKS_REGIME_BPC] = small ? 0 : bin_scan_bands(t.gx);
    out[SKS_REGIME_LEAD] = fill_lead(a);
    out[SKS_REGIME_WAVE_GROUPS] = (small && bwd_small_wave(P, flags)) ? bwd_wave_groups(V, P, flags) : 0;
    return 0;
}

int sks_list_regime(int* out)
{
    if (!out) return fail(-2, "sks_list_regime: out must be provided");
    memset(out, 0, SKS_LIST_REGIME_INTS * sizeof(int));
    out[SKS_LIST_WAVE_SORT] = BIN_WAVE_SORT;
    out[SKS_LIST_WAVE_K] = 64 * WSORT_K;
    out[SKS_LIST_SORT_LDS] = SORT_LDS;
    out[SKS_LIST_LONG_LIST] = LONG_LIST;
    out[SKS_LIST_CLASSES] = BIN_CLASSES;
    out[SKS_LIST_BAND_THREADS] = BAND_TS;
    return 0;
}

}

namespace {

int forward_impl(const FwdCall& c, const FwdHook* hook, int prefilled)
{
    const Cameras& cam = c.cam;
    const int V = cam.V, P = cam.P, C = cam.C, W = cam.W, H = cam.H;
    const unsigned flags = c.g.flags;
    const size_t bin_capacity = c.io.bin_capacity;
    if (int rc = check_common(cam)) return rc;
    const hipStream_t st = c.stream;
    if (prefilled < 0 || prefilled > (C + 1) * V) return fail(-1, "prefilled_planes=%d out of range [0,%d]", prefilled, (C + 1) * V);
    if (!c.io.out_color || !c.io.out_invdepth) return fail(-2, "out_color / out_invdepth must be provided");
    if (((uintptr_t)c.io.out_color | (uintptr_t)c.io.out_invdepth) & 15u)
        return fail(-2, "out_color / out_invdepth must be 16-byte aligned (the planes are written with 16-byte stores)");
    const size_t HW = (size_t)H * W;
    if (P == 0) {
        HIP_TRY(hipMemsetAsync(c.io.out_color, 0, (size_t)V * C * HW * 4, st));
        HIP_TRY(hipMemsetAsync(c.io.out_invdepth, 0, (size_t)V * HW * 4, st));
        if (c.final_T) return fail(-2, "final_T not available for P == 0");
        return 0;
    }
    if (int rc = require({ cam.viewmatrix, cam.projmatrix, cam.tanfovx, cam.tanfovy, c.g.means3D, c.g.features, c.g.opacities, c.io.radii, c.io.geom }))
        return rc;
    if (int rc = need_cov(c.g.scales, c.g.rotations, c.g.cov3D_precomp)) return rc;
    ViewTan vt;
    ViewOff vo;
    fill_views(vt, &vo, V, C, W, H, cam.tanfovx, cam.tanfovy, nullptr, nullptr);
    Geom g = geom_from(c.io.geom, V, P, W, H);
    const TileGrid t(W, H);
    const int gx = t.gx, gy = t.gy, NT = t.NT;

    const bool small = is_small(P, flags);
    Bin b{};
    if (!small) {
        if (!c.io.binning) return fail(-2, "binned path needs a binning buffer");
        if (bin_capacity < 1) return fail(-1, "binned path needs bin_capacity >= 1");
        b = bin_from(c.io.binning, V, P, NT, bin_capacity);
    }
    if (!small) g.cover = nullptr;
    const int gplanes = (small && g.cover && cover_per_plane(P, W, H, C)) ? C + 1 : 1;
    FwdArgs a{ P, C, W, H, flags, g, c.g.features, c.io.out_color, c.io.out_invdepth, c.final_T, c.n_contrib, composite_slots(flags, V, P),
               ((1u << 20) + (unsigned)C) / (unsigned)(C + 1), 0, (!small || (g.cover && cover_per_plane(P, W, H, C))) ? 1 : 0,
               fill_w_magic(W) };
    const int planes = (C + 1) * V;
    int pre = 0;
    if (prefilled > 0 && small && !hook && !c.final_T && !c.n_contrib && !(flags & SKS_DEBUG_SYNC) &&
        !(prof_next_forward_sampled() && !prof_has_parked(st)))
        pre = prefilled;
    const int zp = planes - pre;
    int early = 0;
    if (small && !hook && g.cover && !c.final_T && !c.n_contrib && !(flags & (SKS_DEBUG_SYNC | SKS_NO_EARLY_FILL))) {
        early = early_fill_planes(flags, planes, HW * 4);
        if (early > zp) early = zp;
    }
    int efs = 0, epb = 0;
    if (early > 0 && early_fill_cut(a, V, gy, gplanes, zp - early, zp, efs, epb)) {
        ProfScope prof(0, st, true, pre > 0);
        launch_geom_fill(a, c, gy, gplanes, zp - early, zp, efs, epb, vt, prof);
        with_cg(C, [&](auto cg) { launch_fwd_small<decltype(cg)::value>(a, V, gy, zp - early, st, prof); });
        HIP_TRY(hipGetLastError());
        return 0;
    }
    launch_geom_fwd(c, vt, g, b, small, gplanes, (hook && small) ? hook->geom_done : nullptr);
    STAGE_CHECK("geometry");
    if (hook && small && hook->after_geom) {
        if (int rc = hook->after_geom(hook->ctx)) return rc;
    }

    if (small) {
        {
            ProfScope prof(0, st, true, pre > 0);
            with_cg(C, [&](auto cg) { launch_fwd_small<decltype(cg)::value>(a, V, gy, zp, st, prof); });
        }
        STAGE_CHECK("render(small)");
        return 0;
    }
    uint32_t* cover = b.coverp;
    const int cw = cover_cw(W);
    hipLaunchKernelGGL(k_bin_band_count, dim3(gy, V), dim3(BAND_TC), (size_t)2 * gx * 4, st, P, gx, g, b);
    int vg, ng;
    bin_groups(flags, V, vg, ng);
    {
        const int bpc = bin_scan_bands(gx);
        const int nchunk_t = (gy + bpc - 1) / bpc, nchunk_g = (P + SCAN_G - 1) / SCAN_G;
        hipLaunchKernelGGL(k_bin_scan, dim3(nchunk_t + nchunk_g, V), dim3(SCAN_T), (size_t)bpc * cw * 4, st, P, gx, gy, cw, bpc,
                           nchunk_t, bin_capacity, b, cover, c.io.num_rendered_dev, V, C + 1, vg);
    }
    hipLaunchKernelGGL(k_bin_band_scatter, dim3(gy, V), dim3(BAND_TS), (size_t)2 * gx * 4, st, P, gx, bin_capacity, g, b, C, cw);
    STAGE_CHECK("binning");
    const BinView bv_all = bin_view(b, NT, bin_capacity);
    {
        ProfScope prof(0, st);
        for (int gi = 0; gi < ng; gi++) {
            const int v0 = gi * vg, nv = (V - v0 < vg) ? V - v0 : vg;
            FwdArgs ag = a;
            ag.out_color = a.out_color + (size_t)v0 * C * HW;
            ag.out_invdepth = a.out_invdepth + (size_t)v0 * HW;
            if (a.final_T) ag.final_T = a.final_T + (size_t)v0 * HW;
            if (a.n_contrib) ag.n_contrib = a.n_contrib + (size_t)v0 * HW;
            BinView bv = bv_all;
            bv.ranges += (size_t)v0 * NT;
            bv.tidx += (size_t)v0 * NT;
            bv.aux += (size_t)v0 * NT * TILE * TILE;
            bv.e_co += (size_t)v0 * bin_capacity;
            bv.e_xyd += (size_t)v0 * bin_capacity;
            bv.e_ids += (size_t)v0 * bin_capacity;
            bv.part += (size_t)v0 * bin_capacity * BIN_ROWS * NACC;
            const uint32_t* cov_g = cover + (size_t)v0 * (C + 1) * gy * cw;
            with_cg(C, [&](auto cg) { launch_fwd_binned<decltype(cg)::value>(ag, bv, nv, gx, gy, cov_g, st); });
            if (hook && hook->after_group)
                if (int rc = hook->after_group(hook->ctx, gi, v0, nv)) return rc;
        }
    }
    STAGE_CHECK("render(binned)");
    return 0;
}

constexpr unsigned BWD_RENDER = 1u, BWD_GEOM = 2u;
int backward_impl(const BwdCall& c, unsigned phases, int group, const PrefillReq* pre)
{
    const Cameras& cam = c.cam;
    const int V = cam.V, P = cam.P, C = cam.C, W = cam.W, H = cam.H;
    const unsigned flags = c.g.flags;
    const Grads& gr = c.grads;
    if (int rc = check_common(cam)) return rc;
    if (P == 0) return 0;
    const hipStream_t st = c.stream;
    if (int rc = require({ cam.viewmatrix, cam.projmatrix, cam.tanfovx, cam.tanfovy, c.g.means3D, c.g.features, c.g.opacities, c.radii, c.geom,
                           c.up.dL_dout_color, c.up.accum, gr.dL_dmeans3D, gr.dL_dmeans2D, gr.dL_dopacity }))
        return rc;
    if (int rc = need_cov(c.g.scales, c.g.rotations, c.g.cov3D_precomp)) return rc;
    ViewTan vt;
    ViewOff vo;
    fill_views(vt, &vo, V, C, W, H, cam.tanfovx, cam.tanfovy, nullptr, nullptr);
    Geom g = geom_from(const_cast<void*>(c.geom), V, P, W, H);
    const TileGrid t(W, H);
    const int gx = t.gx, NT = t.NT;
    BwdArgs a{ P, C, W, H, flags, g, c.g.features, c.bg, c.up.dL_dout_color, c.up.dL_dout_invdepth, (float*)c.up.accum, nullptr, nullptr };
    const bool dfeat = gr.dL_dfeatures != nullptr;
    const bool small = is_small(P, flags);
    int vg = V, ng = 1;
    if (!small) bin_groups(flags, V, vg, ng);
    if (group >= ng) return fail(-1, "view group %d of %d", group, ng);
    const bool geom_all = gr.dL_dmeans3D_mean && V * P <= 256 && small;
    PreFill pfw{}, pfg{};
    bool have_pfw = false, have_pfg = false;
    if (pre && pre->planes_wave + pre->planes_geom > 0) {
        const int planes = (C + 1) * V, n = pre->planes_wave + pre->planes_geom;
        const int n_geom = geom_all ? pre->planes_geom : 0, nw = n - n_geom;
        if (nw > 0) {
            if (!prefill_cut(pfw, pre->color, pre->invdepth, V, C, W, H, planes - n, nw, (long long)P * V, 65535 - BWD_SPLITS))
                return fail(-1, "sks_backward_prefill: %d planes of %dx%d do not fit the compositing backward's launch", nw, W, H);
            have_pfw = true;
        }
        if (n_geom > 0) {
            if (!prefill_cut(pfg, pre->color, pre->invdepth, V, C, W, H, planes - n_geom, n_geom, 1, (1ll << 31) - 2))
                return fail(-1, "sks_backward_prefill: %d planes of %dx%d do not fit the geometry backward's launch", n_geom, W, H);
            have_pfg = true;
        }
        if (prof_next_forward_sampled()) prof_park_begin(st);
    }
    if ((phases & BWD_RENDER) && small) {
        ProfScope prof(1, st, true);
        const PreFill* pf = have_pfw ? &pfw : nullptr;
        with_cg(C, [&](auto cg) { launch_bwd_small<decltype(cg)::value>(a, vt, vo, V, dfeat, st, prof, pf); });
        STAGE_CHECK("render-backward(small)");
    } else if (phases & BWD_RENDER) {
        if (!c.binning) return fail(-2, "binned path needs the forward's binning buffer");
        Bin b = bin_from(const_cast<void*>(c.binning), V, P, NT, c.bin_capacity);
        BinView bv = bin_view(b, NT, c.bin_capacity);
        if (dfeat && group <= 0) HIP_TRY(hipMemsetAsync(c.up.accum, 0, (size_t)V * P * (NACC + C) * sizeof(float), st));
        dim3 grid(bwd_tile_blocks());
        const unsigned magic_nt = magic32((unsigned)NT), magic_gx = magic32((unsigned)gx);
        const bool extra = c.bg != nullptr || c.up.dL_dout_invdepth != nullptr;
        for (int gi = group < 0 ? 0 : group; gi < (group < 0 ? ng : group + 1); gi++) {
            const uint4* tl = b.tlist + (size_t)gi * vg * NT;
            const uint32_t* hd = b.hdr + gi * BIN_CLASSES;
            ProfScope prof(1, st);
            if (dfeat) hipLaunchKernelGGL((k_render_bwd_tile<true, true>), grid, dim3(BWD_TILE_THREADS), 0, st, a, bv, gx, V, magic_nt, magic_gx, tl, hd);
            else if (extra) hipLaunchKernelGGL((k_render_bwd_tile<false, true>), grid, dim3(BWD_TILE_THREADS), 0, st, a, bv, gx, V, magic_nt, magic_gx, tl, hd);
            else hipLaunchKernelGGL((k_render_bwd_tile<false, false>), grid, dim3(BWD_TILE_THREADS), 0, st, a, bv, gx, V, magic_nt, magic_gx, tl, hd);
        }
        STAGE_CHECK("render-backward(binned)");
    }
    if (!(phases & BWD_GEOM)) return 0;
    GeomBwdArgs ga{ P, C, W, H, flags, cam.viewmatrix, cam.projmatrix, c.g.means3D, c.g.opacities, c.g.scales, c.g.rotations, c.g.cov3D_precomp,
                    c.g.scale_modifier, c.radii, (const float*)c.up.accum, small ? BWD_SPLITS : 0, nullptr, nullptr, nullptr, gr.dL_dmeans3D, gr.dL_dmeans2D,
                    gr.dL_dopacity, gr.dL_dscales, gr.dL_drotations, gr.dL_dcov3D, gr.dL_dfeatures };
    if (!small) {
        Bin b = bin_from(const_cast<void*>(c.binning), V, P, NT, c.bin_capacity);
        ga.rect = g.rect;
        ga.goff = b.goff;
        ga.part = b.part;
        ga.cap = c.bin_capacity;
        ga.bin_hdr = b.hdr;
    }
    if (geom_all) {
        if (have_pfg) hipLaunchKernelGGL((k_geom_bwd_all<PreFill>), dim3(1u + pfg.nfill), dim3(256), 0, st, ga, vt, V, gr.dL_dmeans3D_mean, pfg);
        else hipLaunchKernelGGL((k_geom_bwd_all<>), dim3(1), dim3(256), 0, st, ga, vt, V, gr.dL_dmeans3D_mean);
    } else {
        if (small) hipLaunchKernelGGL(k_geom_bwd, dim3((P + 255) / 256, V), dim3(256), 0, st, ga, vt);
        else {
            const int v0 = group < 0 ? 0 : group * vg, nv = group < 0 ? V : ((V - v0 < vg) ? V - v0 : vg);
            ga.v0 = v0;
            hipLaunchKernelGGL(k_geom_bwd_binned, dim3((P + GEOMB_G - 1) / GEOMB_G, nv), dim3(256), 0, st, ga, vt);
        }
        if (gr.dL_dmeans3D_mean && (small || group < 0 || group == ng - 1))
            hipLaunchKernelGGL(k_mean_views, dim3((3 * P + 255) / 256), dim3(256), 0, st, V, P, gr.dL_dmeans3D, gr.dL_dmeans3D_mean);
    }
    if (have_pfw || have_pfg) prof_park_end(st);
    STAGE_CHECK("geometry-backward");
    return 0;
}

const float NO_TAN[SKS_MAX_VIEWS] = {};
const double NO_SCHED[5] = { 1.0, 1.0, 1.0, 0.0, 1.0 };
int loop_fused_step_impl(const StepCall& c)
{
    const Cameras& cam = c.cam;
    const sksloop::Optimiser& opt = c.opt;
    const int V = cam.V, P = cam.P, C = cam.C, W = cam.W, H = cam.H, frames = c.hm.frames;
    const float* const* const hm_factors = c.hm.hm_factors;
    if (int rc = check_common(cam)) return rc;
    if (P < 1 || P > 64) return fail(-1, "fused step needs 1 <= P <= 64 (got %d)", P);
    if (int rc = check_frames(V, frames)) return rc;
    if (c.vw.mode < 0 || c.vw.mode > 2) return fail(-1, "fused step: vw_mode = %d, expected 0 (off), 1 (scale) or 2 (select)", c.vw.mode);
    if (c.es.es_state && (c.es.es_window < 1 || c.es.es_window > sksloop::ES_MAX_WINDOW))
        return fail(-1, "fused step: early-stopping window %d out of range [1, %d]", c.es.es_window, sksloop::ES_MAX_WINDOW);
    const int Vf = V / frames;
    if (int rc = require({ cam.viewmatrix, cam.projmatrix, cam.tanfovx, cam.tanfovy, c.r.features, c.r.radii, c.r.geom,
                           c.r.gt ? (const void*)c.r.gt : (const void*)hm_factors, c.r.gt_totals, c.r.accum, c.r.loss_sums, c.r.packed }))
        return rc;
    if (int rc = check_hm_factors(hm_factors)) return rc;
    const hipStream_t st = c.stream;
    ViewTan vt;
    ViewOff vo;
    if (!fill_views(vt, &vo, V, C, W, H, cam.tanfovx, cam.tanfovy, c.hm.view_wh, c.hm.gt_offsets)) return bad_view_wh();
    if (int rc = check_wh_offsets(hm_factors, c.hm.view_wh, c.hm.gt_offsets)) return rc;
    const unsigned flags = c.r.flags | SKS_RAW_PARAMS | SKS_CLAMP01;
    sksloop::AdamArgs aa;
    if (const char* err = sksloop::fill_adam_args(aa, Vf, P, c.r.packed, opt)) return fail(-2, "%s", err);
    const bool es = c.es.es_state != nullptr;
    if (es) { aa.es_state = c.es.es_state; aa.es_window = c.es.es_window; aa.es_tol = c.es.es_tolerance; aa.es_host_flag = c.es.es_host_flags; }
    Geom g = geom_from(c.r.geom, V, P, W, H);
    g.cover = nullptr;
    BwdArgs a{ P, C, W, H, flags, g, c.r.features, nullptr, c.r.gt, nullptr, (float*)c.r.accum, nullptr, nullptr };
    if (hm_factors) { a.hm_row = hm_factors[0]; a.hm_col = hm_factors[1]; a.hm_cmin = hm_factors[2]; a.hm_den = hm_factors[3]; }
    if (es) { a.es_stop = c.es.es_state + 1; a.es_stride = 2 + 2 * c.es.es_window; a.es_views = Vf; }
    {
        ProfScope prof(1, st);
        if (!es) launch_bwd_loss(a, vt, vo, V, st);
        else launch_bwd_loss<true>(a, vt, vo, V, st);
    }
    STAGE_CHECK("render-backward(fused loss)");
    GeomBwdArgs ga{ P, C, W, H, flags, cam.viewmatrix, cam.projmatrix, opt.xyz, opt.opacity, opt.scaling, opt.rotation, nullptr, c.r.scale_modifier,
                    c.r.radii, (const float*)c.r.accum, BWD_SPLITS, c.r.gt_totals, c.r.loss_sums, c.r.packed, nullptr, nullptr, nullptr, nullptr,
                    nullptr, nullptr, nullptr };
    if (c.vw.mode) {
        const sksloop::ViewWeightArgs vw = c.vw;
        if (c.views_dev) {
            const ViewTanDev vd = views_dev_from(c.views_dev, c.lr_sched_dev);
            if (es) hipLaunchKernelGGL((k_step_tail_vw<true, ViewTanDev>), dim3(frames), dim3(256), 0, st, ga, vd, aa, Vf, g, c.r.radii, vw);
            else hipLaunchKernelGGL((k_step_tail_vw<false, ViewTanDev>), dim3(frames), dim3(256), 0, st, ga, vd, aa, Vf, g, c.r.radii, vw);
        } else if (es) hipLaunchKernelGGL(k_step_tail_vw<true>, dim3(frames), dim3(256), 0, st, ga, vt, aa, Vf, g, c.r.radii, vw);
        else hipLaunchKernelGGL(k_step_tail_vw<false>, dim3(frames), dim3(256), 0, st, ga, vt, aa, Vf, g, c.r.radii, vw);
    } else if (c.views_dev) {
        const ViewTanDev vd = views_dev_from(c.views_dev, c.lr_sched_dev);
        if (es) hipLaunchKernelGGL((k_step_tail<true, ViewTanDev>), dim3(frames), dim3(256), 0, st, ga, vd, aa, Vf, g, c.r.radii);
        else hipLaunchKernelGGL((k_step_tail<false, ViewTanDev>), dim3(frames), dim3(256), 0, st, ga, vd, aa, Vf, g, c.r.radii);
    } else if (es) hipLaunchKernelGGL(k_step_tail<true>, dim3(frames), dim3(256), 0, st, ga, vt, aa, Vf, g, c.r.radii);
    else hipLaunchKernelGGL(k_step_tail<false>, dim3(frames), dim3(256), 0, st, ga, vt, aa, Vf, g, c.r.radii);
    STAGE_CHECK("step tail");
    return 0;
}

}

extern "C" {

#define SKS_TAKE_CAMERAS(r)                                                                                                                    \
    ((r).V = V, (r).P = P, (r).C = C, (r).W = W, (r).H = H, (r).viewmatrix = viewmatrix, (r).projmatrix = projmatrix, (r).tanfovx = tanfovx, (r).tanfovy = tanfovy)
#define SKS_TAKE_GAUSSIANS(r)                                                                                                                  \
    ((r).means3D = means3D, (r).features = features, (r).opacities = opacities, (r).scales = scales, (r).rotations = rotations,                \
     (r).cov3D_precomp = cov3D_precomp, (r).scale_modifier = scale_modifier, (r).flags = flags)
#define SKS_TAKE_FORWARD_IO(r)                                                                                                                 \
    ((r).out_color = out_color, (r).out_invdepth = out_invdepth, (r).radii = radii, (r).geom = geom, (r).binning = binning,                    \
     (r).bin_capacity = bin_capacity, (r).num_rendered_dev = num_rendered_dev)
#define SKS_TAKE_UPSTREAM(r) ((r).dL_dout_color = dL_dout_color, (r).dL_dout_invdepth = dL_dout_invdepth, (r).accum = accum)
#define SKS_TAKE_GRADS(r)                                                                                                                      \
    ((r).dL_dmeans3D = dL_dmeans3D, (r).dL_dmeans2D = dL_dmeans2D, (r).dL_dopacity = dL_dopacity, (r).dL_dscales = dL_dscales,                 \
     (r).dL_drotations = dL_drotations, (r).dL_dcov3D = dL_dcov3D, (r).dL_dfeatures = dL_dfeatures, (r).dL_dmeans3D_mean = dL_dmeans3D_mean)
#define SKS_TAKE_FWD_CALL(c, ft, nc) \
    (SKS_TAKE_CAMERAS((c).cam), SKS_TAKE_GAUSSIANS((c).g), SKS_TAKE_FORWARD_IO((c).io), (c).final_T = (ft), (c).n_contrib = (nc), (c).stream = (hipStream_t)stream)
#define SKS_TAKE_BWD_CALL(c)                                                                                                                   \
    (SKS_TAKE_CAMERAS((c).cam), (c).bg = bg, SKS_TAKE_GAUSSIANS((c).g), (c).radii = radii, (c).geom = geom, (c).binning = binning,             \
     (c).bin_capacity = bin_capacity, SKS_TAKE_UPSTREAM((c).up), SKS_TAKE_GRADS((c).grads), (c).stream = (hipStream_t)stream)
#define SKS_TAKE_STEP_CALL(c, sched)                                                                                                           \
    (SKS_TAKE_CAMERAS((c).cam), (c).r.features = features, (c).r.scale_modifier = scale_modifier, (c).r.flags = flags, (c).r.radii = radii,    \
     (c).r.geom = geom, (c).r.gt = gt, (c).r.gt_totals = gt_totals, (c).r.accum = accum, (c).r.loss_sums = loss_sums, (c).r.packed = packed,   \
     SKS_TAKE_OPTIMISER((c).opt, sched), (c).hm.view_wh = view_wh, (c).hm.gt_offsets = gt_offsets, (c).hm.frames = frames,                     \
     (c).hm.hm_factors = hm_factors, (c).stream = (hipStream_t)stream)
#define SKS_TAKE_ES(r) ((r).es_state = es_state, (r).es_window = es_window, (r).es_tolerance = es_tolerance, (r).es_host_flags = es_host_flags)

int sks_forward(int V, int P, int C, int W, int H, const float* viewmatrix, const float* projmatrix,
                const float* tanfovx, const float* tanfovy, const float* means3D, const float* features,
                const float* opacities, const float* scales, const float* rotations, const float* cov3D_precomp,
                float scale_modifier, unsigned flags, float* out_color, float* out_invdepth, int* radii, void* geom,
                void* binning, size_t bin_capacity, int* num_rendered_dev, float* final_T, uint32_t* n_contrib,
                void* stream)
{
    FwdCall c;
    SKS_TAKE_FWD_CALL(c, final_T, n_contrib);
    return forward_impl(c, nullptr, 0);
}

int sks_backward(int V, int P, int C, int W, int H, const float* viewmatrix, const float* projmatrix,
                 const float* tanfovx, const float* tanfovy, const float* bg, const float* means3D,
                 const float* features, const float* opacities, const float* scales, const float* rotations,
                 const float* cov3D_precomp, float scale_modifier, unsigned flags, const int* radii, const void* geom,
                 const void* binning, size_t bin_capacity, const float* dL_dout_color, const float* dL_dout_invdepth,
                 void* accum, float* dL_dmeans3D, float* dL_dmeans2D, float* dL_dopacity, float* dL_dscales,
                 float* dL_drotations, float* dL_dcov3D, float* dL_dfeatures, float* dL_dmeans3D_mean, void* stream)
{
    BwdCall c;
    SKS_TAKE_BWD_CALL(c);
    return backward_impl(c, BWD_RENDER | BWD_GEOM, -1, nullptr);
}

int sks_forward_prefilled(int V, int P, int C, int W, int H, const float* viewmatrix, const float* projmatrix,
                          const float* tanfovx, const float* tanfovy, const float* means3D, const float* features,
                          const float* opacities, const float* scales, const float* rotations, const float* cov3D_precomp,
                          float scale_modifier, unsigned flags, float* out_color, float* out_invdepth, int* radii, void* geom,
                          void* binning, size_t bin_capacity, int* num_rendered_dev, float* final_T, uint32_t* n_contrib,
                          int prefilled_planes, void* stream)
{
    FwdCall c;
    SKS_TAKE_FWD_CALL(c, final_T, n_contrib);
    return forward_impl(c, nullptr, prefilled_planes);
}

int sks_backward_prefill(int V, int P, int C, int W, int H, const float* viewmatrix, const float* projmatrix,
                         const float* tanfovx, const float* tanfovy, const float* bg, const float* means3D,
                         const float* features, const float* opacities, const float* scales, const float* rotations,
                         const float* cov3D_precomp, float scale_modifier, unsigned flags, const int* radii, const void* geom,
                         const void* binning, size_t bin_capacity, const float* dL_dout_color, const float* dL_dout_invdepth,
                         void* accum, float* dL_dmeans3D, float* dL_dmeans2D, float* dL_dopacity, float* dL_dscales,
                         float* dL_drotations, float* dL_dcov3D, float* dL_dfeatures, float* dL_dmeans3D_mean,
                         float* next_color, float* next_invdepth, int planes_wave, int planes_geom, void* stream)
{
    if (int rc = check_common(V, P, C, W, H)) return rc;
    if (planes_wave < 0 || planes_geom < 0 || (long long)planes_wave + planes_geom > (long long)(C + 1) * V)
        return fail(-1, "sks_backward_prefill: planes_wave=%d planes_geom=%d out of range (the call has %d planes)", planes_wave, planes_geom, (C + 1) * V);
    const PrefillReq req{ next_color, next_invdepth, planes_wave, planes_geom };
    if (planes_wave + planes_geom > 0) {
        if (!prefill_possible(P, W, H, flags & ~SKS_NO_NT_STORES))
            return fail(-1, "sks_backward_prefill: no prefill for this call (wave-resident small path with 16-byte non-temporal stores only: "
                            "1 <= P <= 64, W %% 4 == 0 or W %% 4 == 2 with an even H, no SKS_NO_NT_STORES / SKS_DEBUG_SYNC / SKS_FORCE_BINNED)");
        if (!next_color || !next_invdepth) return fail(-2, "sks_backward_prefill: next_color / next_invdepth must be provided");
        if (((uintptr_t)next_color | (uintptr_t)next_invdepth) & 15u) return fail(-2, "next_color / next_invdepth must be 16-byte aligned");
    }
    BwdCall c;
    SKS_TAKE_BWD_CALL(c);
    return backward_impl(c, BWD_RENDER | BWD_GEOM, -1, planes_wave + planes_geom > 0 ? &req : nullptr);
}

#ifndef SKS_PREFILL_WAVE_BYTES
#define SKS_PREFILL_WAVE_BYTES 56000000u
#endif
#ifndef SKS_PREFILL_GEOM_BYTES
#define SKS_PREFILL_GEOM_BYTES 28000000u
#endif
int sks_prefill_planes(int V, int P, int C, int W, int H, unsigned flags, int* planes_wave, int* planes_geom)
{
    if (int rc = check_common(V, P, C, W, H)) return rc;
    if (!planes_wave || !planes_geom) return fail(-2, "sks_prefill_planes: planes_wave / planes_geom must be provided");
    *planes_wave = *planes_geom = 0;
    if (!prefill_possible(P, W, H, flags) || !cover_enabled(P, W, H)) return 0;
    const int planes = (C + 1) * V;
    const size_t plane_bytes = (size_t)H * W * 4;
    const int early = (flags & SKS_NO_EARLY_FILL) ? 0 : early_fill_planes(flags, planes, plane_bytes);
    int room = planes / 2 - early;
    if (room <= 0) return 0;
    if (W % 4 != 0 || C > 20 || V * P < 51 || V * P > 85 || bwd_wave_groups(V, P, flags) != 16) return 0;
    long long nw = ((long long)SKS_PREFILL_WAVE_BYTES + plane_bytes / 2) / plane_bytes;
    long long ng = ((long long)SKS_PREFILL_GEOM_BYTES + plane_bytes / 2) / plane_bytes;
    if (nw > room) nw = room;
    if (ng > room - nw) ng = room - nw;
    PreFill f;
    if (nw > 0 && !prefill_cut(f, nullptr, nullptr, V, C, W, H, planes - (int)(nw + ng), (int)nw, (long long)P * V, 65535 - BWD_SPLITS)) nw = 0;
    if (ng > 0 && !prefill_cut(f, nullptr, nullptr, V, C, W, H, planes - (int)ng, (int)ng, 1, (1ll << 31) - 2)) ng = 0;
    *planes_wave = (int)nw;
    *planes_geom = (int)ng;
    return 0;
}

int sks_forward_backward(int V, int P, int C, int W, int H, const float* viewmatrix, const float* projmatrix,
                         const float* tanfovx, const float* tanfovy, const float* means3D, const float* features,
                         const float* opacities, const float* scales, const float* rotations, const float* cov3D_precomp,
                         float scale_modifier, unsigned flags, float* out_color, float* out_invdepth, int* radii, void* geom,
                         void* binning, size_t bin_capacity, int* num_rendered_dev, const float* bg,
                         const float* dL_dout_color, const float* dL_dout_invdepth, void* accum, float* dL_dmeans3D,
                         float* dL_dmeans2D, float* dL_dopacity, float* dL_dscales, float* dL_drotations, float* dL_dcov3D,
                         float* dL_dfeatures, float* dL_dmeans3D_mean, void* stream, void* aux_stream, unsigned fb_flags)
{
    const bool small = is_small(P, flags);
    int vg = V, ng = 1;
    if (!small && V >= 1) bin_groups(flags, V, vg, ng);
    const hipStream_t st = (hipStream_t)stream, aux = (hipStream_t)aux_stream;
    FwdCall fwd;
    SKS_TAKE_FWD_CALL(fwd, nullptr, nullptr);
    BwdCall bwd;
    SKS_TAKE_BWD_CALL(bwd);
    struct Ctx {
        const BwdCall& bwd;
        hipStream_t s;
        bool ext, handed;
        int rc_aux;
    } c{ bwd, st, true, false, 0 };
    {
        static const bool ext_off = [] { const char* e = getenv("SKS_FB_EXT"); return e && atoi(e) == 0; }();
        if (ext_off) c.ext = false;
    }
    const bool no_join = (fb_flags & SKS_FB_NO_JOIN) != 0;
    const bool crowded = small && (long long)V * P > FB_OVERLAP_MAX_PAIRS && !no_join;
    if (!aux_stream || aux_stream == stream || P == 0 || (flags & SKS_DEBUG_SYNC) || (!small && ng < 2) || crowded) {
        fwd.g.flags |= SKS_NO_EARLY_FILL;
        if (int rc = forward_impl(fwd, nullptr, 0)) return rc;
        if (int rc = backward_impl(bwd, BWD_RENDER | BWD_GEOM, -1, nullptr)) return rc;
        if (no_join && aux_stream && aux_stream != stream) {
            FbEvents* ev = nullptr;
            if (int rc = fb_events(0, ev)) return rc;
            HIP_TRY(hipEventRecord(ev->done, st));
            HIP_TRY(hipStreamWaitEvent(aux, ev->done, 0));
        }
        return 0;
    }
    FbEvents* evp = nullptr;
    if (int rc = fb_events(small ? 0 : ng, evp)) return rc;
    FbEvents& ev = *evp;
    bwd.stream = aux;
    struct Run {
        static int after_geom(void* p)
        {
            Ctx& k = *(Ctx*)p;
            FbEvents& e = tl_fb_events;
            if (!k.ext) HIP_TRY(hipEventRecord(e.geom, k.s));
            HIP_TRY(hipStreamWaitEvent(k.bwd.stream, e.geom, 0));
            k.handed = true;
            return k.rc_aux = backward_impl(k.bwd, BWD_RENDER | BWD_GEOM, -1, nullptr);
        }
        static int after_group(void* p, int g, int, int)
        {
            Ctx& k = *(Ctx*)p;
            FbEvents& e = tl_fb_events;
            HIP_TRY(hipEventRecord(e.grp[g], k.s));
            HIP_TRY(hipStreamWaitEvent(k.bwd.stream, e.grp[g], 0));
            k.handed = true;
            return k.rc_aux = backward_impl(k.bwd, BWD_RENDER | BWD_GEOM, g, nullptr);
        }
    };
    const FwdHook hook{ (small && c.ext) ? ev.geom : nullptr, small ? &Run::after_geom : nullptr, small ? nullptr : &Run::after_group, &c };
    int rc = forward_impl(fwd, &hook, 0);
    if (rc == 0 && !c.handed) rc = fail(-3, "sks_forward_backward: the forward did not reach the point the backward starts from");
    if (c.handed && (!no_join || rc != 0)) {
        const hipError_t e1 = hipEventRecord(ev.done, aux);
        const hipError_t e2 = e1 == hipSuccess ? hipStreamWaitEvent(c.s, ev.done, 0) : e1;
        if (rc == 0 && e2 != hipSuccess) rc = fail((int)e2, "sks_forward_backward: joining the two streams: %s", hipGetErrorString(e2));
    }
    return rc;
}

int sks_mean_views(int V, int P, const float* dL_dmeans3D, int shard_world, float* mean_out, void* stream)
{
    if (V < 1 || P < 1 || shard_world < 1) return fail(-1, "mean_views: bad shape");
    if (!dL_dmeans3D || !mean_out) return fail(-2, "mean_views: missing pointer");
    hipLaunchKernelGGL(k_mean_views, dim3((3 * P + 255) / 256), dim3(256), 0, (hipStream_t)stream, V, P, dL_dmeans3D, mean_out,
                       shard_world);
    HIP_TRY(hipGetLastError());
    return 0;
}

int sks_gt_tile_stats(int V, int C, int W, int H, const float* gt, float* tile_S, float* tile_N, double* totals, void* stream)
{
    if (int rc = check_common(V, 1, C, W, H)) return rc;
    if (!gt || !totals) return fail(-2, "gt_tile_stats: missing pointer");
    hipStream_t st = (hipStream_t)stream;
    HIP_TRY(hipMemsetAsync(totals, 0, (size_t)V * 2 * sizeof(double), st));
    dim3 grid(TileGrid(W, H).gy, C, V);
    hipLaunchKernelGGL(k_gt_tile_stats, grid, dim3(256), 0, st, C, W, H, gt, tile_S, tile_N, totals);
    HIP_TRY(hipGetLastError());
    return 0;
}

int sks_backward_fused_loss(int V, int P, int C, int W, int H, const float* viewmatrix, const float* projmatrix,
                            const float* tanfovx, const float* tanfovy, const float* bg, const float* means3D,
                            const float* features, const float* opacities, const float* scales, const float* rotations,
                            const float* cov3D_precomp, float scale_modifier, unsigned flags, const int* radii,
                            const void* geom, const float* gt, const float* tile_S, const float* tile_N,
                            const double* gt_totals, void* accum, float* dL_dmeans3D, float* dL_dmeans2D,
                            float* dL_dopacity, float* dL_dscales, float* dL_drotations, float* dL_dcov3D,
                            double* loss_sums, float* packed_raw_grads, const int* view_wh, const size_t* gt_offsets,
                            const float* const* hm_factors, void* stream)
{
    if (int rc = check_common(V, P, C, W, H)) return rc;
    if (P < 1 || P > 64) return fail(-1, "fused-loss backward needs 1 <= P <= 64 (got %d)", P);
    hipStream_t st = (hipStream_t)stream;
    if (int rc = require({ viewmatrix, projmatrix, tanfovx, tanfovy, means3D, features, opacities, radii, geom,
                           gt ? (const void*)gt : (const void*)hm_factors, gt_totals, accum, dL_dmeans3D, dL_dmeans2D, dL_dopacity, loss_sums }))
        return rc;
    if (int rc = check_hm_factors(hm_factors)) return rc;
    if (int rc = need_cov(scales, rotations, cov3D_precomp)) return rc;
    ViewTan vt;
    ViewOff vo;
    if (!fill_views(vt, &vo, V, C, W, H, tanfovx, tanfovy, view_wh, gt_offsets)) return bad_view_wh();
    if (int rc = check_wh_offsets(hm_factors, view_wh, gt_offsets)) return rc;
    Geom g = geom_from(const_cast<void*>(geom), V, P, W, H);
    BwdArgs a{ P, C, W, H, flags | SKS_CLAMP01, g, features, bg, gt, nullptr, (float*)accum, tile_S, tile_N };
    if (hm_factors) { a.hm_row = hm_factors[0]; a.hm_col = hm_factors[1]; a.hm_cmin = hm_factors[2]; a.hm_den = hm_factors[3]; }
    {
        ProfScope prof(1, st);
        launch_bwd_loss(a, vt, vo, V, st);
    }
    STAGE_CHECK("fused loss + render-backward");
    GeomBwdArgs ga{ P, C, W, H, flags, viewmatrix, projmatrix, means3D, opacities, scales, rotations, cov3D_precomp,
                    scale_modifier, radii, (const float*)accum, BWD_SPLITS, gt_totals, loss_sums, packed_raw_grads, dL_dmeans3D, dL_dmeans2D,
                    dL_dopacity, dL_dscales, dL_drotations, dL_dcov3D, nullptr };
    hipLaunchKernelGGL(k_geom_bwd, dim3((P + 255) / 256, V), dim3(256), 0, st, ga, vt);
    STAGE_CHECK("geometry-backward");
    return 0;
}

int sks_geometry(int V, int P, int C, int W, int H, const float* viewmatrix, const float* projmatrix, const float* tanfovx,
                 const float* tanfovy, const float* means3D, const float* opacities, const float* scales,
                 const float* rotations, const float* cov3D_precomp, float scale_modifier, unsigned flags, int* radii,
                 void* geom, const int* view_wh, int frames, void* stream)
{
    if (int rc = check_common(V, P, C, W, H)) return rc;
    if (P < 1) return fail(-1, "P must be positive");
    if (int rc = check_frames(V, frames)) return rc;
    if (int rc = require({ viewmatrix, projmatrix, tanfovx, tanfovy, means3D, opacities, radii, geom })) return rc;
    if (int rc = need_cov(scales, rotations, cov3D_precomp)) return rc;
    hipStream_t st = (hipStream_t)stream;
    ViewTan vt;
    if (!fill_views(vt, nullptr, V, C, W, H, tanfovx, tanfovy, view_wh, nullptr)) return bad_view_wh();
    Geom g = geom_from(geom, V, P, W, H);
    g.cover = nullptr;
    hipLaunchKernelGGL(k_geom_fwd, dim3((P + 255) / 256, V), dim3(256), 0, st, P, W, H, vt, viewmatrix, projmatrix,
                       means3D, opacities, scales, rotations, cov3D_precomp, scale_modifier, flags, g, radii,
// ... 6 lines not shown
                    const float* means3D, const float* opacities, const float* scales, const float* rotations,
                    const float* cov3D_precomp, float scale_modifier, unsigned flags, int* radii, void* geom, int frames,
                    void* stream)
{
    if (int rc = check_common(V, P, C, W, H)) return rc;
    if (P < 1) return fail(-1, "P must be positive");
    if (int rc = check_frames(V, frames)) return rc;
    if (int rc = require({ viewmatrix, projmatrix, views_dev, means3D, opacities, radii, geom })) return rc;
    if (int rc = need_cov(scales, rotations, cov3D_precomp)) return rc;
    hipStream_t st = (hipStream_t)stream;
    Geom g = geom_from(geom, V, P, W, H);
    g.cover = nullptr;
    hipLaunchKernelGGL(k_geom_fwd_dv, dim3((P + 255) / 256, V), dim3(256), 0, st, P, views_dev_from(views_dev), viewmatrix,
                       projmatrix, means3D, opacities, scales, rotations, cov3D_precomp, scale_modifier, flags, g, radii,
                       frames > 1 ? V / frames : 0);
    STAGE_CHECK("geometry");
    return 0;
}

int sks_loop_fused_step(int V, int P, int C, int W, int H, const float* viewmatrix, const float* projmatrix,
                        const float* tanfovx, const float* tanfovy, const float* features, float scale_modifier,
                        unsigned flags, int* radii, void* geom, const float* gt, const double* gt_totals, void* accum,
                        double* loss_sums, float* packed, float* slots, unsigned long long group_mask, int last_view,
                        float* xyz, float* scaling, float* rotation, float* opacity, float* exp_avg, float* exp_avg_sq,
                        int* counters, int acc_steps, const double* lr_sched, const double* lrs, const double* adam,
                        float lambda_consistency, const int* limb, const int* view_wh, const size_t* gt_offsets, int frames,
                        const float* const* hm_factors, void* stream)
{
    StepCall c{};
    SKS_TAKE_STEP_CALL(c, lr_sched);
    return loop_fused_step_impl(c);
}

int sks_loop_fused_step_es(int V, int P, int C, int W, int H, const float* viewmatrix, const float* projmatrix,
                           const float* tanfovx, const float* tanfovy, const float* features, float scale_modifier,
                           unsigned flags, int* radii, void* geom, const float* gt, const double* gt_totals, void* accum,
                           double* loss_sums, float* packed, float* slots, unsigned long long group_mask, int last_view,
                           float* xyz, float* scaling, float* rotation, float* opacity, float* exp_avg, float* exp_avg_sq,
                           int* counters, int acc_steps, const double* lr_sched, const double* lrs, const double* adam,
                           float lambda_consistency, const int* limb, const int* view_wh, const size_t* gt_offsets, int frames,
                           const float* const* hm_factors, int* es_state, int es_window, float es_tolerance,
                           int* es_host_flags, void* stream)
{
    if (!es_state)
        return fail(-2, "loop_fused_step_es: es_state is required (sks_loop_fused_step is the step without a criterion)");
    if (es_window < 1 || es_window > sksloop::ES_MAX_WINDOW)
        return fail(-1, "loop_fused_step_es: window %d out of range [1, %d]", es_window, sksloop::ES_MAX_WINDOW);
    StepCall c{};
    SKS_TAKE_STEP_CALL(c, lr_sched);
    SKS_TAKE_ES(c.es);
    return loop_fused_step_impl(c);
}

int sks_loop_fused_step_dv(int V, int P, int C, int W, int H, const float* viewmatrix, const float* projmatrix,
                           const void* views_dev, const float* features, float scale_modifier, unsigned flags, int* radii,
                           void* geom, const float* gt, const double* gt_totals, void* accum, double* loss_sums, float* packed,
                           float* slots, unsigned long long group_mask, int last_view, float* xyz, float* scaling,
                           float* rotation, float* opacity, float* exp_avg, float* exp_avg_sq, int* counters, int acc_steps,
                           const double* lr_sched_dev, const double* lrs, const double* adam, float lambda_consistency,
                           const int* limb, const int* view_wh, const size_t* gt_offsets, int frames,
                           const float* const* hm_factors, void* stream)
{
    if (!views_dev || !lr_sched_dev) return fail(-2, "loop_fused_step_dv: views_dev and lr_sched_dev are required");
    const float *const tanfovx = NO_TAN, *const tanfovy = NO_TAN;
    StepCall c{};
    SKS_TAKE_STEP_CALL(c, NO_SCHED);
    c.views_dev = views_dev, c.lr_sched_dev = lr_sched_dev;
    return loop_fused_step_impl(c);
}

int sks_loop_fused_step_es_dv(int V, int P, int C, int W, int H, const float* viewmatrix, const float* projmatrix,
                              const void* views_dev, const float* features, float scale_modifier, unsigned flags, int* radii,
                              void* geom, const float* gt, const double* gt_totals, void* accum, double* loss_sums,
                              float* packed, float* slots, unsigned long long group_mask, int last_view, float* xyz,
                              float* scaling, float* rotation, float* opacity, float* exp_avg, float* exp_avg_sq, int* counters,
                              int acc_steps, const double* lr_sched_dev, const double* lrs, const double* adam,
                              float lambda_consistency, const int* limb, const int* view_wh, const size_t* gt_offsets,
                              int frames, const float* const* hm_factors, int* es_state, int es_window, float es_tolerance,
                              int* es_host_flags, void* stream)
{
    if (!views_dev || !lr_sched_dev) return fail(-2, "loop_fused_step_es_dv: views_dev and lr_sched_dev are required");
    if (!es_state)
        return fail(-2, "loop_fused_step_es_dv: es_state is required (sks_loop_fused_step_dv is the step without a criterion)");
    if (es_window < 1 || es_window > sksloop::ES_MAX_WINDOW)
        return fail(-1, "loop_fused_step_es_dv: window %d out of range [1, %d]", es_window, sksloop::ES_MAX_WINDOW);
    const float *const tanfovx = NO_TAN, *const tanfovy = NO_TAN;
    StepCall c{};
    SKS_TAKE_STEP_CALL(c, NO_SCHED);
    c.views_dev = views_dev, c.lr_sched_dev = lr_sched_dev;
    SKS_TAKE_ES(c.es);
    return loop_fused_step_impl(c);
}

#define SKS_TAKE_VW(r) ((r).mode = vw_mode, (r).threshold = vw_threshold, (r).weights = vw_weights, (r).similarity = vw_similarity)
int sks_loop_fused_step_vw(int V, int P, int C, int W, int H, const float* viewmatrix, const float* projmatrix,
                           const float* tanfovx, const float* tanfovy, const float* features, float scale_modifier,
                           unsigned flags, int* radii, void* geom, const float* gt, const double* gt_totals, void* accum,
                           double* loss_sums, float* packed, float* slots, unsigned long long group_mask, int last_view,
                           float* xyz, float* scaling, float* rotation, float* opacity, float* exp_avg, float* exp_avg_sq,
                           int* counters, int acc_steps, const double* lr_sched, const double* lrs, const double* adam,
                           float lambda_consistency, const int* limb, const int* view_wh, const size_t* gt_offsets, int frames,
                           const float* const* hm_factors, int* es_state, int es_window, float es_tolerance,
                           int* es_host_flags, int vw_mode, float vw_threshold, float* vw_weights, float* vw_similarity,
                           void* stream)
{
    StepCall c{};
    SKS_TAKE_STEP_CALL(c, lr_sched);
    if (es_state) SKS_TAKE_ES(c.es);
    SKS_TAKE_VW(c.vw);
    return loop_fused_step_impl(c);
}

int sks_loop_fused_step_vw_dv(int V, int P, int C, int W, int H, const float* viewmatrix, const float* projmatrix,
                              const void* views_dev, const float* features, float scale_modifier, unsigned flags, int* radii,
                              void* geom, const float* gt, const double* gt_totals, void* accum, double* loss_sums,
                              float* packed, float* slots, unsigned long long group_mask, int last_view, float* xyz,
                              float* scaling, float* rotation, float* opacity, float* exp_avg, float* exp_avg_sq, int* counters,
                              int acc_steps, const double* lr_sched_dev, const double* lrs, const double* adam,
                              float lambda_consistency, const int* limb, const int* view_wh, const size_t* gt_offsets,
                              int frames, const float* const* hm_factors, int* es_state, int es_window, float es_tolerance,
                              int* es_host_flags, int vw_mode, float vw_threshold, float* vw_weights, float* vw_similarity,
                              void* stream)
{
    if (!views_dev || !lr_sched_dev) return fail(-2, "loop_fused_step_vw_dv: views_dev and lr_sched_dev are required");
    const float *const tanfovx = NO_TAN, *const tanfovy = NO_TAN;
    StepCall c{};
    SKS_TAKE_STEP_CALL(c, NO_SCHED);
    c.views_dev = views_dev, c.lr_sched_dev = lr_sched_dev;
    if (es_state) SKS_TAKE_ES(c.es);
    SKS_TAKE_VW(c.vw);
    return loop_fused_step_impl(c);
}

int sks_prof_spin(double microseconds, void* stream)
{
    if (!(microseconds >= 0.0) || microseconds > 1e6) return fail(-1, "prof_spin: 0 .. 1e6 us");
    hipLaunchKernelGGL(k_spin_us, dim3(1), dim3(64), 0, (hipStream_t)stream, (unsigned long long)(microseconds * 100.0));
    HIP_TRY(hipGetLastError());
    return 0;
}

int sks_prof_enable(int on)
{
    if (!tl_prof) {
        if (!on) return 0;
        tl_prof = new ProfState();
    }
    tl_prof->on = on != 0;
    tl_prof->every = (on & 0xffff) > 1 ? (on & 0xffff) : 1;
    tl_prof->skip = (on >> 16) & 3;
    tl_prof->recorded = (on >> 18) & 1;
    tl_prof->seen[0] = tl_prof->seen[1] = 0;
    tl_prof->parked = false;
    return 0;
}

int sks_prof_count(int kind, long long* launches)
{
    if (kind < 0 || kind > 1 || !launches) return fail(-2, "bad profile query");
    *launches = tl_prof ? tl_prof->kind[kind].n : 0;
    return 0;
}

int sks_prof_read(int kind, double* total_ms, long long* launches)
{
    if (kind < 0 || kind > 1 || !total_ms || !launches) return fail(-2, "bad profile query");
    if (!tl_prof) { *total_ms = 0.0; *launches = 0; return 0; }
    ProfKind& p = tl_prof->kind[kind];
    double tot = 0;
    for (int i = 0; i < p.n; i++) {
        float ms = 0;
        HIP_TRY(prof_elapsed(p, i, &ms));
        tot += ms;
    }
    *total_ms = tot;
    *launches = p.n;
    p.n = 0;
    return 0;
}

int sks_prof_read_quantiles(int kind, double* q_ms , double* total_ms, long long* launches)
{
    if (kind < 0 || kind > 1 || !q_ms || !total_ms || !launches) return fail(-2, "bad profile query");
    if (!tl_prof) { q_ms[0] = q_ms[1] = q_ms[2] = 0.0; *total_ms = 0.0; *launches = 0; return 0; }
    ProfKind& p = tl_prof->kind[kind];
    static thread_local float t[PROF_MAX];
    double tot = 0;
    for (int i = 0; i < p.n; i++) {
        HIP_TRY(prof_elapsed(p, i, &t[i]));
        tot += t[i];
    }
    const int n = p.n;
    for (int i = 1; i < n; i++) {
        const float v = t[i];
        int j = i - 1;
        for (; j >= 0 && t[j] > v; j--) t[j + 1] = t[j];
        t[j + 1] = v;
    }
    q_ms[0] = n ? t[(int)(0.1 * (n - 1) + 0.5)] : 0.0;
    q_ms[1] = n ? t[(n - 1) / 2] : 0.0;
    q_ms[2] = n ? t[(int)(0.9 * (n - 1) + 0.5)] : 0.0;
    *total_ms = tot;
    *launches = n;
    p.n = 0;
    return 0;
}

int sks_mark_visible(int P, const float* means3D, const float* viewmatrix, const float* projmatrix, uint8_t* present,
                     void* stream)
{
    (void)projmatrix;
    if (P < 0) return fail(-1, "P negative");
    if (P == 0) return 0;
    if (int rc = require({ means3D, viewmatrix, present })) return rc;
    hipLaunchKernelGGL(k_mark_visible, dim3((P + 255) / 256), dim3(256), 0, (hipStream_t)stream, P, means3D, viewmatrix, present);
    HIP_TRY(hipGetLastError());
    return 0;
}

int sks_export_lists(int V, int W, int H, const void* binning, size_t bin_capacity, uint32_t* point_list,
                     uint32_t* ranges, void* stream)
{
    if (int rc = require({ binning, point_list, ranges })) return rc;
    const int NT = TileGrid(W, H).NT;
    Bin b = bin_from(const_cast<void*>(binning), V, 1, NT, bin_capacity);
    const size_t m = bin_capacity > (size_t)NT ? bin_capacity : (size_t)NT;
    hipLaunchKernelGGL(k_export_lists, dim3((unsigned)((m + 255) / 256), V), dim3(256), 0, (hipStream_t)stream, NT,
                       bin_capacity, b.ranges, b.nrend, point_list, ranges);
    hipLaunchKernelGGL(k_export_sorted, dim3((NT + 3) / 4, V), dim3(256), 0, (hipStream_t)stream, bin_view(b, NT, bin_capacity),
                       point_list);
    HIP_TRY(hipGetLastError());
    return 0;
}

}
```

skelsplat_amd/rasterizer.py:

```python
from collections import namedtuple
from typing import NamedTuple, Optional

import operator
import os

import torch
import torch.nn as nn

from . import _arena, _lib
from ._arena import _BIN_CAP_HINT, _BIN_CAP_SEEN, _BIN_PROBE
from ._base import (ForwardState, ViewBatch, _accum, _bg_channels, _f32c, _f32c_params, _fresh, _grad_dict,
                    _need_gpu, _scratch_bytes_cached, reset_scratch)
from ._tuning import (PLAIN_STORES, TUNE_CANDIDATES, TUNE_CANDIDATES_FRESH, TUNE_CANDIDATES_WITH_PLAIN, TUNE_WARM,
                      _FILL_BITS, _FILL_TUNE, _FILL_TUNE_LOG, _MEASURING, _pick, _time_candidates, _tune_flag_bits, fill_tuning,
                      tune_name)
from .sparse import (GtStats, HeatmapFactors, HeatmapSet, backward_fused_loss, geometry_views, gt_tile_stats,
                     loop_fused_step)

_ENV_TUNE = int(os.environ.get("SKS_FWD_TUNE", "0"), 0)
AUTOTUNE = os.environ.get("SKS_AUTOTUNE", "1") != "0"


class GaussianRasterizationSettings(NamedTuple):
    image_height: int
    image_width: int
    tanfovx: float
    tanfovy: float
    bg: torch.Tensor
    scale_modifier: float
    viewmatrix: torch.Tensor
    projmatrix: torch.Tensor
    sh_degree: int
    campos: torch.Tensor
    prefiltered: bool
    debug: bool
    antialiasing: bool


class Workspace:

    def __init__(self, prefill=None):
        self._t = {}
        self._plans = {}
        self._aux = {}
        self._pending_join = None
        if prefill is not None and prefill != 0:
            prefill = (int(prefill[0]), int(prefill[1]))
        self._prefill = prefill
        self._pf = None
        self._pf_off = prefill == 0

    def aux_stream(self, dev_index):
        st = self._aux.get(dev_index)
        if st is None:
            st = self._aux[dev_index] = torch.cuda.Stream(device=dev_index)
        return st

    def join(self, dev_index):
        torch.cuda.current_stream(dev_index).wait_stream(self.aux_stream(dev_index))
        self._pending_join = None

    def tune(self, step_fn, candidates=None, reps=8, rounds=3, confirm=True):
        plan = self._plans.get("fwd")
        if plan is None or torch.cuda.is_current_stream_capturing():
            return None, {}
        candidates = TUNE_CANDIDATES if candidates is None else candidates
        args, dev_index = plan.args, plan.dev_index
        base = args[_F_FLAGS] & ~_FILL_BITS

        def set_bits(bits):
            args[_F_FLAGS] = base | bits
        times = _time_candidates(set_bits, step_fn, candidates, reps, rounds, dev_index)
        best, med = _pick(times, candidates, set_bits, step_fn, reps, dev_index, confirm)
        set_bits(_tune_flag_bits(best))
        key = (dev_index, *(args[_lib.FWD[n]] for n in ("V", "P", "C", "W", "H")), "workspace")
        _FILL_TUNE[key] = _tune_flag_bits(best)
        _FILL_TUNE_LOG[key] = {tune_name(c): round(v, 2) for c, v in med.items()}
        return best, med

    def settle(self):
        if self._pending_join is not None:
            self.join(self._pending_join)

    def get(self, name, shape, dtype, device):
        key = (name, tuple(shape), dtype, device)
        t = self._t.get(key)
        if t is None:
            t = torch.empty(shape, dtype=dtype, device=device)
            self._t[key] = t
        return t


class _Prefill:
    __slots__ = ("shape", "sets", "results", "cur", "note", "fargs", "bplan", "bargs", "rule")

    def __init__(self, shape, color, invdepth, radii, st, args):
        self.shape = shape
        self.sets = [(color, invdepth), None]
        self.results = [(color, invdepth, radii, st), None]
        self.cur, self.note = 0, None
        self.fargs = list(args[:-1]) + [0, None]
        self.bplan = self.bargs = None
        self.rule = {}


_PREFILL_MAX_SET_BYTES = 1 << 30


def _sig(t):
    if t is None or t.numel() == 0:
        return None
    if t.dtype is not torch.float32 or not t.is_cuda or not t.is_contiguous():
        return False
    return (t.data_ptr(), t.shape)


_FwdRecord = namedtuple("_FwdRecord", "key keep args dev_index result arena")
_BwdRecord = namedtuple("_BwdRecord", "key keep args dev_index result")
_Block = namedtuple("_Block", "args dev_index dev shape")

_F_V, _F_FLAGS, _F_COLOR, _F_INVDEPTH, _F_RADII, _F_GEOM, _F_NUM_RENDERED = (
    _lib.FWD[n] for n in ("V", "flags", "out_color", "out_invdepth", "radii", "geom", "num_rendered_dev"))
_B_RADII, _B_GEOM, _B_DL_COLOR, _B_DL_INVDEPTH = (_lib.BWD[n] for n in ("radii", "geom", "dL_dout_color", "dL_dout_invdepth"))
_B_DFEAT = _lib.BWD["dL_dfeatures"]
_GRAD_SLOTS = tuple((k, _lib.BWD[n]) for k, n in (
    ("means3D", "dL_dmeans3D"), ("means2D", "dL_dmeans2D"), ("opacities", "dL_dopacity"), ("scales", "dL_dscales"),
    ("rotations", "dL_drotations"), ("cov3D", "dL_dcov3D"), ("features", "dL_dfeatures")))
_FB_STREAM, _FB_AUX_STREAM, _FB_FLAGS = (_lib.FWD_BWD[n] for n in ("stream", "aux_stream", "fb_flags"))
_FB_GATHER = operator.itemgetter(*(_lib.FWD["stream"] if src is None else src[1] + (len(_lib.FWD) if src[0] == "bwd" else 0)
                                   for src in _lib.FWD_BWD_SOURCES))


def _replay(fn, args, dev_index, stream_slot=-1):
    args[stream_slot] = torch._C._cuda_getCurrentRawStream(dev_index)
    if torch._C._cuda_getDevice() == dev_index:
        return fn(*args)
    with torch.cuda.device(dev_index):
        return fn(*args)


def forward_views(views: ViewBatch, means3D, features, opacities, scales, rotations, cov3D_precomp,
                  scale_modifier=1.0, antialiasing=False, clamp01=False, debug=False, force_binned=False,
                  bin_capacity=None, want_aux=False, tune_flags=0, check_capacity=True, workspace=None, plans=None):
    lib = _lib.load()
    key = None
    if features is not None and features.numel() and means3D is not None and means3D.dim() == 2 and means3D.shape[0] \
            and features.numel() // means3D.shape[0] > _lib.SKS_MAX_CHANNELS:
        return _forward_views_wide(views, means3D, features, opacities, scales, rotations, cov3D_precomp, scale_modifier, antialiasing,
                                   clamp01, debug, force_binned, bin_capacity, want_aux, tune_flags, check_capacity)
    if not want_aux and (workspace is not None or plans is not None):
        key = _fwd_key(views, means3D, features, opacities, scales, rotations, cov3D_precomp, scale_modifier, antialiasing,
                       clamp01, debug, force_binned, bin_capacity, tune_flags, check_capacity)
    if key is not None and workspace is None:
        hit = plans.get(key)
        if hit is not None:
            args_t, dev_index, dev, (V, P, C, H, W, gbytes, flags) = hit
            color = torch.empty((V, C, H, W), dtype=torch.float32, device=dev)
            invdepth = torch.empty((V, 1, H, W), dtype=torch.float32, device=dev)
            radii = torch.empty((V, P), dtype=torch.int32, device=dev)
            geom = torch.empty((gbytes,), dtype=torch.uint8, device=dev)
            args = list(args_t)
            args[_F_COLOR], args[_F_INVDEPTH], args[_F_RADII], args[_F_GEOM] = color.data_ptr(), invdepth.data_ptr(), radii.data_ptr(), geom.data_ptr()
            _lib.check(_replay(lib.sks_forward, args, dev_index), "sks_forward")
            st = ForwardState(views, P, C, flags, scale_modifier, radii, geom)
            st.plan_key = key
            return color, invdepth, radii, st
    if workspace is not None:
        workspace.settle()
    if key is not None and workspace is not None:
        plan = workspace._plans.get("fwd")
        if plan is not None and plan.key == key:
            pf = workspace._pf
            if pf is not None:
                rc = _forward_two_sets(lib, workspace, pf, plan)
                if rc != 0:
                    del workspace._plans["fwd"]
                    workspace._pf = None
                _lib.check(rc, "sks_forward")
                return pf.results[pf.cur]
            ticket = _replay_ticket(workspace, plan)
            rc = _replay(lib.sks_forward, plan.args, plan.dev_index)
            if rc != 0:
                del workspace._plans["fwd"]
            _lib.check(rc, "sks_forward")
            if ticket is None or (_arena.finish(ticket) or 0) <= ticket.cap:
                return plan.result
            del workspace._plans["fwd"]
    if workspace is not None and workspace._pf is not None:
        workspace._pf.note = None
    if views.mixed:
        raise RuntimeError("the dense forward writes one (V,C,H,W) tensor: all views of the batch must share the image size")
    if means3D is None or means3D.dim() != 2 or means3D.shape[1] != 3:
        raise RuntimeError("means3D must have dimensions (num_points, 3)")
    _need_gpu(means3D, "means3D")
    if means3D.shape[0] == 0:
        dev, V, W, H = means3D.device, views.V, views.W, views.H
        C = int(features.shape[-1])
        st = ForwardState(views, 0, C, 0, scale_modifier, torch.zeros((V, 0), dtype=torch.int32, device=dev))
        out = (torch.zeros((V, C, H, W), device=dev), torch.zeros((V, 1, H, W), device=dev), st.radii, st)
        if want_aux:
            out += (torch.ones((V, H, W), device=dev), torch.zeros((V, H, W), dtype=torch.int32, device=dev))
        return out
    means3D, features, opacities, scales, rotations, cov3D_precomp = _f32c_params(means3D, features, opacities, scales, rotations, cov3D_precomp)
    dev = means3D.device
    P = means3D.shape[0]
    feat2 = features.reshape(P, -1)
    C = feat2.shape[1]
    V, W, H = views.V, views.W, views.H
    flags = (_lib.SKS_ANTIALIASING if antialiasing else 0) | (_lib.SKS_CLAMP01 if clamp01 else 0) | \
            (_lib.SKS_DEBUG_SYNC if debug else 0) | (_lib.SKS_FORCE_BINNED if force_binned else 0) | int(tune_flags) | _ENV_TUNE
    if plans is not None and workspace is None and AUTOTUNE and not flags & _FILL_BITS and not _MEASURING[0] and not force_binned \
            and (dev.index, V, P, C, W, H, "fresh") not in _FILL_TUNE:
        tune_forward(views, means3D, feat2, opacities, scales, rotations, cov3D_precomp, scale_modifier, antialiasing, clamp01,
                     tune_flags=tune_flags)
    if not flags & _FILL_BITS and not _MEASURING[0]:
        flags |= _FILL_TUNE.get((dev.index, V, P, C, W, H, "workspace" if workspace is not None else "fresh"), 0)
    binned = force_binned or P > _lib.SKS_SMALL_P
    ticket = _arena.begin((dev.index, V, P, C, W, H), bin_capacity, check_capacity, torch.cuda.is_current_stream_capturing()) if binned else None
    cap = ticket.cap if binned else int(bin_capacity or 0)
    gbytes, bbytes, _ = _scratch_bytes_cached(V, max(P, 1), C, W, H, cap)
    def new(name, shape, dtype):
        if workspace is None:
            return torch.empty(shape, dtype=dtype, device=dev)
        return workspace.get(("fwd", name), shape, dtype, dev)

    color = new("color", (V, C, H, W), torch.float32)
    invdepth = new("invdepth", (V, 1, H, W), torch.float32)
    radii = new("radii", (V, P), torch.int32)
    geom = new("geom", (gbytes,), torch.uint8)
    binning = new("binning", (bbytes,), torch.uint8) if binned else None
    nrend = None if not binned else new("nrend", (V + 1,), torch.int32) if ticket.device else ticket.host
    final_T = torch.empty((V, H, W), dtype=torch.float32, device=dev) if want_aux else None
    n_contrib = torch.empty((V, H, W), dtype=torch.int32, device=dev) if want_aux else None
    args = [V, P, C, W, H, views.viewmatrix.data_ptr(), views.projmatrix.data_ptr(), views.tanfovx,
            views.tanfovy, _lib.ptr(means3D), _lib.ptr(feat2), _lib.ptr(opacities), _lib.ptr(scales),
            _lib.ptr(rotations), _lib.ptr(cov3D_precomp), float(scale_modifier), flags,
            color.data_ptr(), invdepth.data_ptr(), _lib.ptr(radii), geom.data_ptr(),
            _lib.ptr(binning), cap, _lib.ptr(nrend), _lib.ptr(final_T), _lib.ptr(n_contrib), None]
    _lib.check(_replay(lib.sks_forward, args, dev.index), "sks_forward")
    if binned:
        need = _arena.finish(ticket, nrend)
        if need is not None and need > cap:
            return forward_views(views, means3D, features, opacities, scales, rotations, cov3D_precomp, scale_modifier,
                                 antialiasing, clamp01, debug, force_binned, _arena.grown(need), want_aux, tune_flags,
                                 check_capacity, workspace)
    st = ForwardState(views, P, C, flags, scale_modifier, radii, geom, binning, cap, nrend)
    if want_aux:
        return color, invdepth, radii, st, final_T, n_contrib
    if key is None or not _recordable(key):
        return color, invdepth, radii, st
    if workspace is None:
        if not binned and P:
            if len(plans) > 64:
                plans.clear()
            plans[key] = _Block(list(args), dev.index, dev, (V, P, C, H, W, gbytes, flags))
            plans[("keep", key)] = (views, means3D, feat2, opacities, scales, rotations, cov3D_precomp)
            st.plan_key = key
    elif not torch.cuda.is_current_stream_capturing():
        keep = (means3D, feat2, opacities, scales, rotations, cov3D_precomp)
        arena = (ticket.key, cap, True if check_capacity is True else "lazy") if binned and check_capacity else None
        workspace._plans["fwd"] = _FwdRecord(key, (views, keep), args, dev.index, (color, invdepth, radii, st), arena)
        workspace._pf = None
        if not binned and P and not workspace._pf_off and _lib.HAS_PREFILL and 4 * (C + 1) * V * H * W <= _PREFILL_MAX_SET_BYTES:
            workspace._pf = _Prefill((V, P, C, W, H), color, invdepth, radii, st, args)
    else:
        workspace._pf_off = True
    return color, invdepth, radii, st


def _forward_two_sets(lib, workspace, pf, plan):
    note, pf.note = pf.note, None
    args = plan.args
    if note is not None:
        if workspace._pf_off or torch.cuda.is_current_stream_capturing():
            workspace._pf_off = True
        elif note[1] == torch._C._cuda_getCurrentRawStream(plan.dev_index):
            other = 1 - pf.cur
            color, invdepth = pf.sets[other]
            fargs = pf.fargs
            fargs[_F_FLAGS], fargs[_F_COLOR], fargs[_F_INVDEPTH], fargs[-2] = args[_F_FLAGS], color.data_ptr(), invdepth.data_ptr(), note[0]
            rc = _replay(lib.sks_forward_prefilled, fargs, plan.dev_index)
            if rc == 0:
                pf.cur = other
                args[_F_COLOR], args[_F_INVDEPTH] = fargs[_F_COLOR], fargs[_F_INVDEPTH]
            return rc
    elif not workspace._pf_off and torch.cuda.is_current_stream_capturing():
        workspace._pf_off = True
    return _replay(lib.sks_forward, args, plan.dev_index)


def _backward_prefill(lib, workspace, plan):
    pf = workspace._pf
    if pf is None or workspace._pf_off or plan.key[0] != id(pf.results[0][3]):
        return None
    if torch.cuda.is_current_stream_capturing():
        workspace._pf_off, pf.note = True, None
        return None
    fplan = workspace._plans.get("fwd")
    if fplan is None:
        return None
    fflags = fplan.args[_F_FLAGS]
    n = pf.rule.get(fflags)
    if n is None:
        V, P, C, W, H = pf.shape
        n = pf.rule[fflags] = _lib.prefill_planes(V, P, C, W, H, fflags) if workspace._prefill is None else workspace._prefill
    if workspace._prefill is None and plan.args[_B_DFEAT] is not None:
        return None
    if n[0] + n[1] == 0:
        return None
    if pf.sets[1] is None:
        color, invdepth, radii, st = pf.results[0]
        c2 = workspace.get(("fwd", "color2"), color.shape, color.dtype, color.device)
        i2 = workspace.get(("fwd", "invdepth2"), invdepth.shape, invdepth.dtype, invdepth.device)
        pf.sets[1], pf.results[1] = (c2, i2), (c2, i2, radii, st)
    if pf.bplan is not plan:
        pf.bplan, pf.bargs = plan, list(plan.args[:-1]) + [None, None, 0, 0, None]
    color, invdepth = pf.sets[1 - pf.cur]
    bargs = pf.bargs
    bargs[-5], bargs[-4], bargs[-3], bargs[-2] = color.data_ptr(), invdepth.data_ptr(), n[0], n[1]
    pf.note = None
    rc = _replay(lib.sks_backward_prefill, bargs, plan.dev_index)
    if rc == 0:
        pf.note = (n[0] + n[1], bargs[-1])
    return rc


def _replay_ticket(workspace, plan):
    if plan.arena is None:
        return None
    try:
        ticket = _arena.begin(*plan.arena, torch.cuda.is_current_stream_capturing())
    except RuntimeError:
        workspace._plans.pop("fwd", None)
        raise
    plan.args[_F_NUM_RENDERED] = _lib.ptr(ticket.host)
    plan.result[3].num_rendered_dev = ticket.host
    return ticket


def _forward_views_wide(views, means3D, features, opacities, scales, rotations, cov3D_precomp, scale_modifier, antialiasing, clamp01,
                        debug, force_binned, bin_capacity, want_aux, tune_flags, check_capacity):
    if want_aux:
        raise RuntimeError("final_T / n_contrib are not available beyond SKS_MAX_CHANNELS channels")
    if views.mixed:
        raise RuntimeError("the dense forward writes one (V,C,H,W) tensor: all views of the batch must share the image size")
    _need_gpu(means3D, "means3D")
    P = means3D.shape[0]
    feat2 = _f32c(features, "features").reshape(P, -1)
    C, V, W, H, dev = feat2.shape[1], views.V, views.W, views.H, means3D.device
    M = _lib.SKS_MAX_CHANNELS
    color = torch.empty((V, C, H, W), dtype=torch.float32, device=dev)
    invdepth = torch.empty((V, 1, H, W), dtype=torch.float32, device=dev)
    radii = torch.empty((V, P), dtype=torch.int32, device=dev)
    st = ForwardState(views, P, C, 0, scale_modifier, radii)
    st.chunks = []
    for v in range(V):
        one = ViewBatch(views.viewmatrix[v:v + 1], views.projmatrix[v:v + 1], [views.tanfovx[v]], [views.tanfovy[v]], W, H)
        for c0 in range(0, C, M):
            c1 = min(C, c0 + M)
            fc = feat2[:, c0:c1].contiguous()
            col, inv, rad, sub = forward_views(one, means3D, fc, opacities, scales, rotations, cov3D_precomp, scale_modifier,
                                               antialiasing, clamp01, debug, force_binned, bin_capacity, False, tune_flags, check_capacity)
            color[v, c0:c1].copy_(col[0])
            if c0 == 0:
                invdepth[v].copy_(inv[0])
                radii[v].copy_(rad[0])
            st.chunks.append((v, c0, c1, fc, sub))
    return color, invdepth, radii, st


def _backward_views_wide(st, means3D, opacities, scales, rotations, cov3D_precomp, dL_dcolor, dL_dinvdepth, bg, want_dfeatures,
                         tune_flags):
    dev, V, P, C = means3D.device, st.views.V, st.P, st.C
    dL_dcolor = _f32c(dL_dcolor, "dL_dout_color").reshape(V, C, st.views.H, st.views.W)
    dL_dinvdepth = _f32c(dL_dinvdepth, "dL_dout_invdepth")
    out = _grad_dict(_fresh(torch.zeros, dev), V, P, C, scales is not None and scales.numel(),
                     rotations is not None and rotations.numel(), want_dfeatures)
    bgC = _bg_channels(bg, C, dev)
    for v, c0, c1, fc, sub in st.chunks:
        g = backward_views(sub, means3D, fc, opacities, scales, rotations, cov3D_precomp, dL_dcolor[v:v + 1, c0:c1],
                           None if (dL_dinvdepth is None or c0) else dL_dinvdepth.reshape(V, 1, st.views.H, st.views.W)[v:v + 1],
                           None if bgC is None else bgC[c0:c1], want_dfeatures, tune_flags)
        for k in ("means3D", "means2D", "opacities", "cov3D", "scales", "rotations"):
            if out[k] is not None:
                out[k][v] += g[k][0]
        if want_dfeatures:
            out["features"][v, :, c0:c1] = g["features"][0]
    return out


def _fwd_key(views, means3D, features, opacities, scales, rotations, cov3D_precomp, scale_modifier, antialiasing, clamp01, debug,
             force_binned, bin_capacity, tune_flags, check_capacity):
    return (id(views), (_sig(means3D), _sig(features), _sig(opacities), _sig(scales), _sig(rotations), _sig(cov3D_precomp)),
            scale_modifier, antialiasing, clamp01, debug, force_binned, bin_capacity, tune_flags, check_capacity)


def _bwd_key(st, means3D, features, opacities, scales, rotations, cov3D_precomp, dL_dcolor, dL_dinvdepth, bg, want_dfeatures,
             tune_flags, want_mean, out_means3D, stream):
    return (id(st), (_sig(means3D), _sig(features), _sig(opacities), _sig(scales), _sig(rotations), _sig(cov3D_precomp),
                     _sig(dL_dcolor), _sig(dL_dinvdepth)), None if bg is None else (id(bg), bg._version), want_dfeatures, tune_flags,
            want_mean, None if out_means3D is None else out_means3D.data_ptr(), stream)


def _recordable(key):
    _owner, sigs, *_switches = key
    return all(sg is not False for sg in sigs)


def backward_views(st: ForwardState, means3D, features, opacities, scales, rotations, cov3D_precomp, dL_dcolor,
                   dL_dinvdepth=None, bg=None, want_dfeatures=False, tune_flags=0, workspace=None, want_mean=False,
                   out_means3D=None, plans=None):
    lib = _lib.load()
    key = pkey = None
    if st.chunks is not None:
        if want_mean or out_means3D is not None:
            raise RuntimeError("want_mean / out_means3D are not available beyond SKS_MAX_CHANNELS channels")
        return _backward_views_wide(st, means3D, opacities, scales, rotations, cov3D_precomp, dL_dcolor, dL_dinvdepth, bg,
                                    want_dfeatures, tune_flags)
    if plans is not None and workspace is None and st.plan_key is not None and out_means3D is None and not want_mean \
            and _sig(dL_dcolor) is not False and (dL_dinvdepth is None or _sig(dL_dinvdepth) is not False):
        stream = torch._C._cuda_getCurrentRawStream(st.geom.device.index)
        pkey = ("bwd", st.plan_key, dL_dcolor.shape, dL_dinvdepth is None, None if bg is None else (id(bg), bg._version),
                want_dfeatures, tune_flags, stream)
        hit = plans.get(pkey)
        if hit is not None:
            args_t, dev_index, dev, shape = hit
            out = _grad_dict(_fresh(torch.empty, dev), *shape, want_dfeatures)
            args = list(args_t)
            args[_B_RADII], args[_B_GEOM], args[_B_DL_COLOR], args[_B_DL_INVDEPTH] = \
                st.radii.data_ptr(), st.geom.data_ptr(), dL_dcolor.data_ptr(), _lib.ptr(dL_dinvdepth)
            for k, i in _GRAD_SLOTS:
                g = out[k]
                args[i] = None if g is None else g.data_ptr()
            rc = _replay(lib.sks_backward, args, dev_index)
            if rc != 0:
                reset_scratch()
                plans.pop(pkey, None)
            _lib.check(rc, "sks_backward")
            return out
    if workspace is not None:
        workspace.settle()
    if workspace is not None and st.P:
        key = _bwd_key(st, means3D, features, opacities, scales, rotations, cov3D_precomp, dL_dcolor, dL_dinvdepth, bg,
                       want_dfeatures, tune_flags, want_mean, out_means3D, torch._C._cuda_getCurrentRawStream(st.geom.device.index))
        plan = workspace._plans.get("bwd")
        if plan is not None and plan.key == key:
            rc = _backward_prefill(lib, workspace, plan)
            if rc is None:
                rc = _replay(lib.sks_backward, plan.args, plan.dev_index)
            if rc != 0:
                reset_scratch()
                del workspace._plans["bwd"]
            _lib.check(rc, "sks_backward")
            return plan.result
    if st.P == 0:
        dev = means3D.device
        empty = _grad_dict(_fresh(torch.zeros, dev), st.views.V, 0, st.C, True, True, want_dfeatures)
        if want_mean:
            empty["means3D_mean"] = torch.zeros((0, 3), dtype=torch.float32, device=dev)
        return empty
    means3D, features, opacities, scales, rotations, cov3D_precomp = _f32c_params(means3D, features, opacities, scales, rotations, cov3D_precomp)
    dev = means3D.device
    V, P, C, W, H = st.views.V, st.P, st.C, st.views.W, st.views.H
    feat2 = features.reshape(P, -1)
    dL_dcolor, dL_dinvdepth = _f32c(dL_dcolor, "dL_dout_color"), _f32c(dL_dinvdepth, "dL_dout_invdepth")
    if dL_dcolor.numel() != V * C * H * W:
        raise RuntimeError("dL_dout_color has the wrong number of elements")
    bgC = _bg_channels(bg, C, dev)
    e = _fresh(torch.empty, dev) if workspace is None else lambda name, *s: workspace.get(("bwd", name), s, torch.float32, dev)
    out = _grad_dict(e, V, P, C, scales is not None, rotations is not None, want_dfeatures)
    if want_mean:
        out["means3D_mean"] = e("m3mean", P, 3)
    if out_means3D is not None:
        if tuple(out_means3D.shape) != (V, P, 3) or out_means3D.dtype != torch.float32 or not out_means3D.is_contiguous() \
                or out_means3D.device != dev:
            raise ValueError(f"out_means3D must be a contiguous fp32 (V,P,3) = {(V, P, 3)} tensor on {dev}")
        out["means3D"] = out_means3D
# ... 279 lines not shown
```

Measured before the change: 69860.

## Host zero-fill of leftover planes inside the small-P hosted forward kernel

```diff
diff --git a/include/skelsplat_hip.h b/include/skelsplat_hip.h
--- a/include/skelsplat_hip.h
+++ b/include/skelsplat_hip.h
@@ -113,6 +113,19 @@
                          float* dL_dscales, float* dL_drotations, float* dL_dcov3D, float* dL_dfeatures,
                          float* dL_dmeans3D_mean,
                          float* next_color, float* next_invdepth, int planes_wave, int planes_geom, void* stream);
+
+#define SKS_NO_HOSTED_FORWARD (1u << 19)
+int sks_hosting_planes(int V, int P, int C, int W, int H, unsigned flags, int* host_planes);
+int sks_forward_hosting(int V, int P, int C, int W, int H,
+                        const float* viewmatrix, const float* projmatrix,
+                        const float* tanfovx , const float* tanfovy ,
+                        const float* means3D, const float* features, const float* opacities,
+                        const float* scales, const float* rotations, const float* cov3D_precomp,
+                        float scale_modifier, unsigned flags,
+                        float* out_color, float* out_invdepth, int* radii,
+                        void* geom, void* binning, size_t bin_capacity, int* num_rendered_dev,
+                        float* final_T, uint32_t* n_contrib,
+                        float* other_color, float* other_invdepth, int host_planes, void* stream);
 
 #define SKS_FB_NO_JOIN 1u
 int sks_forward_backward(int V, int P, int C, int W, int H,
diff --git a/skelsplat_amd/_lib.py b/skelsplat_amd/_lib.py
--- a/skelsplat_amd/_lib.py
+++ b/skelsplat_amd/_lib.py
@@ -39,6 +39,7 @@
 
 
 SKS_NO_EARLY_FILL = 1 << 30
+SKS_NO_HOSTED_FORWARD = 1 << 19
 SKS_BWD_LDS_LIST = 1 << 20
 SKS_FILL_LINEAR = 1 << 21
 SKS_FILL_ROWS = 1 << 22
@@ -69,6 +70,7 @@
 FORWARD_PREFILLED_PARAMS = FORWARD_PARAMS[:-1] + (("prefilled_planes", _i), ("stream", _vp))
 BACKWARD_PREFILL_PARAMS = BACKWARD_PARAMS[:-1] + (("next_color", _vp), ("next_invdepth", _vp), ("planes_wave", _i), ("planes_geom", _i),
                                                   ("stream", _vp))
+FORWARD_HOSTING_PARAMS = FORWARD_PARAMS[:-1] + (("other_color", _vp), ("other_invdepth", _vp), ("host_planes", _i), ("stream", _vp))
 FORWARD_BACKWARD_PARAMS = _CAMERAS + _GAUSSIANS + _FORWARD_IO + (("bg", _vp),) + _UPSTREAM + _GRADS \
     + (("stream", _vp), ("aux_stream", _vp), ("fb_flags", _u))
 
@@ -140,6 +142,8 @@
     "sks_forward_prefilled": (_i, [ct for _, ct in FORWARD_PREFILLED_PARAMS]),
     "sks_backward_prefill": (_i, [ct for _, ct in BACKWARD_PREFILL_PARAMS]),
     "sks_prefill_planes": (_i, [_i, _i, _i, _i, _i, _u, C.POINTER(_i), C.POINTER(_i)]),
+    "sks_forward_hosting": (_i, [ct for _, ct in FORWARD_HOSTING_PARAMS]),
+    "sks_hosting_planes": (_i, [_i, _i, _i, _i, _i, _u, C.POINTER(_i)]),
     "sks_mark_visible": (_i, [_i, _vp, _vp, _vp, _vp, _vp]),
     "sks_mean_views": (_i, [_i, _i, _vp, _i, _vp, _vp]),
     "sks_export_lists": (_i, [_i, _i, _i, _vp, _sz, _vp, _vp, _vp]),
@@ -203,6 +207,8 @@
 
 _PREFILL_SYMBOLS = ("sks_forward_prefilled", "sks_backward_prefill", "sks_prefill_planes")
 HAS_PREFILL = True
+_HOSTING_SYMBOLS = ("sks_forward_hosting", "sks_hosting_planes")
+HAS_HOSTING = True
 
 
 def load(build_if_missing=True):
@@ -221,10 +227,13 @@
         raise ImportError(f"{LIB_PATH} not found; run `python -m skelsplat_amd.build`")
     override = os.environ.get("SKS_LIB_OVERRIDE")
     lib = C.CDLL(override or LIB_PATH)
-    global HAS_PREFILL
+    global HAS_PREFILL, HAS_HOSTING
     for name, (res, args) in SIGNATURES.items():
         if override and name in _PREFILL_SYMBOLS and not hasattr(lib, name):
             HAS_PREFILL = False
+            continue
+        if override and name in _HOSTING_SYMBOLS and not hasattr(lib, name):
+            HAS_HOSTING = False
             continue
         if override and name in VW_STEP_PARAMS and not hasattr(lib, name):
             continue
@@ -311,6 +320,14 @@
     return nw.value, ng.value
 
 
+def hosting_planes(V, P, C_, W, H, flags=0):
+    if not HAS_HOSTING:
+        return 0
+    hp = _i(0)
+    check(load().sks_hosting_planes(V, P, C_, W, H, flags, C.byref(hp)), "sks_hosting_planes")
+    return hp.value
+
+
 def ptr(t):
     if t is None or t.numel() == 0:
         return None
diff --git a/skelsplat_amd/csrc/sks_common.inc b/skelsplat_amd/csrc/sks_common.inc
--- a/skelsplat_amd/csrc/sks_common.inc
+++ b/skelsplat_amd/csrc/sks_common.inc
@@ -42,6 +42,9 @@
     hipEvent_t park_b = nullptr, park_e = nullptr;
     bool parked = false;
     hipStream_t park_st = nullptr;
+    int host_idx = -1;
+    hipStream_t host_st = nullptr;
+    bool host_open = false;
 };
 thread_local ProfState* tl_prof = nullptr;
 
@@ -56,6 +59,7 @@
         if (!ps) return;
         const bool parked = kind == 0 && ps->parked && take_parked && ps->park_st == s;
         if (kind == 0) ps->parked = false;
+        if (kind == 0) ps->host_idx = -1;
         if (!ps->on || ((ps->skip >> kind) & 1)) return;
         if (ps->seen[kind]++ % ps->every != 0) return;
         ProfKind& p = ps->kind[kind];
@@ -106,6 +110,44 @@
     ProfState* ps = tl_prof;
     if (ps && ps->parked && ps->park_st == st && hipEventRecord(ps->park_e, st) != hipSuccess) ps->parked = false;
 }
+inline void prof_host_note(const ProfScope& prof, hipStream_t st)
+{
+    ProfState* ps = tl_prof;
+    if (!ps || !prof.k) return;
+    ps->host_idx = prof.k->n;
+    ps->host_st = st;
+}
+inline bool prof_host_begin(hipStream_t st)
+{
+    ProfState* ps = tl_prof;
+    if (!ps) return false;
+    const int i = ps->host_idx;
+    ps->host_idx = -1;
+    ps->host_open = false;
+    ProfKind& p = ps->kind[0];
+    if (i < 0 || i >= p.n || ps->host_st != st || p.hasx[i]) return false;
+    while (p.xcreated <= i) {
+        if (hipEventCreate(&p.xb[p.xcreated]) != hipSuccess || hipEventCreate(&p.xe[p.xcreated]) != hipSuccess) return false;
+        p.xcreated++;
+    }
+    ps->host_open = hipEventRecord(p.xb[i], st) == hipSuccess;
+    if (ps->host_open) { ps->host_idx = i; ps->parked = false; }
+    return ps->host_open;
+}
+inline void prof_host_end(hipStream_t st)
+{
+    ProfState* ps = tl_prof;
+    if (!ps || !ps->host_open) return;
+    const int i = ps->host_idx;
+    ps->host_open = false;
+    ps->host_idx = -1;
+    ProfKind& p = ps->kind[0];
+    if (i >= 0 && i < p.n && hipEventRecord(p.xe[i], st) == hipSuccess) p.hasx[i] = true;
+}
+inline void prof_host_drop()
+{
+    if (tl_prof) { tl_prof->host_idx = -1; tl_prof->host_open = false; }
+}
 inline hipError_t prof_elapsed(ProfKind& p, int i, float* ms)
 {
     hipError_t e = hipEventSynchronize(p.e[i]);
diff --git a/skelsplat_amd/csrc/sks_fwd_small.inc b/skelsplat_amd/csrc/sks_fwd_small.inc
--- a/skelsplat_amd/csrc/sks_fwd_small.inc
+++ b/skelsplat_amd/csrc/sks_fwd_small.inc
@@ -432,3 +432,132 @@
     const int shift = (int)((reinterpret_cast<uintptr_t>(out) >> 2) & 31u);
     fill_bare<4, true>(out, nullptr, nullptr, q * 1024 * f.pb + (int)threadIdx.x * 4 - shift, Nb, min(f.pb, 32));
 }
+
+template <int CG>
+struct HostGeomLds {
+    float4* co;
+    float4* xyd;
+    float* feat;
+    __device__ HostGeomLds(char* base, int cap)
+    {
+        co = (float4*)base; base += (size_t)cap * 16;
+        xyd = (float4*)base; base += (size_t)cap * 16;
+        feat = (float*)base;
+    }
+    static size_t bytes(int cap, int cg) { return (size_t)cap * (16 + 16 + 4 * (size_t)cg); }
+};
+
+#ifndef SKS_HOST_WAVES_ATTR
+#define SKS_HOST_WAVES_ATTR
+#endif
+template <int CG>
+__global__ __launch_bounds__(256) SKS_HOST_WAVES_ATTR void k_render_fwd_hosting(FwdArgs a, PreFill f, ViewTan vt, const float* __restrict__ vms,
+                                                           const float* __restrict__ pms, const float* __restrict__ means,
+                                                           const float* __restrict__ opac, const float* __restrict__ scales,
+                                                           const float* __restrict__ rots, const float* __restrict__ cov3Dp, float smod,
+                                                           int* __restrict__ radii)
+{
+    const int cb = blockIdx.x;
+    if (cb >= a.ncomp) {
+        prefill_block(f, (unsigned)(cb - a.ncomp));
+        return;
+    }
+    extern __shared__ __attribute__((aligned(16))) char s_dyn[];
+    __shared__ int s_n, s_min;
+    __shared__ unsigned s_chm;
+    const int tid = threadIdx.x;
+    const int P = a.P, C = a.C, W = a.W, H = a.H;
+    const size_t HW = (size_t)H * W;
+    const int T_SLOTS = a.tslots;
+    const int slot = cb % T_SLOTS;
+    const int g = (cb / T_SLOTS) % P;
+    const int v = cb / (T_SLOTS * P);
+    const int cap = (P + 15) & ~15;
+    DynList<CG> L(s_dyn, cap);
+    HostGeomLds<CG> G((char*)(L.feat + (size_t)cap * CG), cap);
+    if (tid < P) {
+        float4 co, xyd;
+        const uint4 r = geom_fwd_one(P, vt, vms, pms, means, opac, scales, rots, cov3Dp, smod, a.flags, a.g, radii, v, tid, true,
+                                     slot == 0 && tid == g, &co, &xyd);
+        L.rect[tid] = r;
+        G.co[tid] = co;
+        G.xyd[tid] = xyd;
+#pragma unroll
+        for (int ch = 0; ch < CG; ch++) G.feat[tid * CG + ch] = ch < C ? a.features[tid * C + ch] : 0.0f;
+    }
+    __syncthreads();
+    const uint4 rg = L.rect[g];
+    const int wt = (int)(rg.z - rg.x), ht = (int)(rg.w - rg.y);
+    const int ntiles = wt * ht;
+    if (slot >= ntiles) return;
+    float* outc = a.out_color + (size_t)v * C * HW;
+    float* outi = a.out_invdepth + (size_t)v * HW;
+    const bool do_clamp = a.flags & SKS_CLAMP01;
+    for (int t = slot; t < ntiles; t += T_SLOTS) {
+        const int ty = (int)rg.y + t / wt, tx = (int)rg.x + t % wt;
+        if (tid == 0) { s_n = 0; s_min = 0x7fffffff; }
+        __syncthreads();
+        if (tid < P) {
+            const uint4 r = L.rect[tid];
+            if ((int)r.x <= tx && tx < (int)r.z && (int)r.y <= ty && ty < (int)r.w) {
+                atomicMin(&s_min, tid);
+                const int sl = atomicAdd(&s_n, 1);
+                L.key[sl] = ((unsigned long long)__float_as_uint(G.xyd[tid].z) << 32) | (unsigned)tid;
+            }
+        }
+        __syncthreads();
+        const int n = s_n;
+        if (s_min == g) {
+            if (tid < n) {
+                const unsigned long long key = L.key[tid];
+                int rank = 0;
+                for (int j = 0; j < n; j++) rank += (L.key[j] < key) ? 1 : 0;
+                const int id = (int)(unsigned)key;
+                const float4 xyd = G.xyd[id];
+                L.xy[rank] = make_float2(xyd.x, xyd.y);
+                L.co[rank] = G.co[id];
+                L.invd[rank] = xyd.w;
+#pragma unroll
+                for (int ch = 0; ch < CG; ch++) L.feat[rank * CG + ch] = G.feat[id * CG + ch];
+            }
+            __syncthreads();
+            bool nz = false;
+            if (tid < CG)
+                for (int k = 0; k < n; k++) nz = nz || L.feat[k * CG + tid] != 0.0f;
+            if (tid < 64) {
+                const unsigned long long bl = __ballot(nz);
+                if (tid == 0) s_chm = (unsigned)bl;
+            }
+            __syncthreads();
+            const unsigned chm = s_chm;
+            const int x = tx * TILE + (tid & 15), y = ty * TILE + (tid >> 4);
+            if (x < W && y < H) {
+                const float pxf = (float)x, pyf = (float)y;
+                float T = 1.0f, inv = 0.0f, acc[CG];
+#pragma unroll
+                for (int ch = 0; ch < CG; ch++) acc[ch] = 0.0f;
+                for (int k = 0; k < n; k++) {
+                    const float2 xy = L.xy[k];
+                    const float4 co = L.co[k];
+                    const float dx = xy.x - pxf, dy = xy.y - pyf;
+                    const float power = -0.5f * (co.x * dx * dx + co.z * dy * dy) - co.y * dx * dy;
+                    if (power > 0.0f) continue;
+                    const float alpha = fminf(0.99f, co.w * expf_fixed(power));
+                    if (alpha < 1.0f / 255.0f) continue;
+                    const float test_T = T * (1 - alpha);
+                    if (test_T < 0.0001f) break;
+#pragma unroll
+                    for (int ch = 0; ch < CG; ch++) acc[ch] += L.feat[k * CG + ch] * alpha * T;
+                    inv += L.invd[k] * alpha * T;
+                    T = test_T;
+                }
+                const size_t pix = (size_t)y * W + x;
+#pragma unroll
+                for (int ch = 0; ch < CG; ch++)
+                    if (ch < C && ((chm >> ch) & 1u)) outc[(size_t)ch * HW + pix] = do_clamp ? clamp01(acc[ch]) : acc[ch];
+                outi[pix] = inv;
+            }
+        }
+        __syncthreads();
+    }
+}
diff --git a/skelsplat_amd/csrc/sks_geom_fwd.inc b/skelsplat_amd/csrc/sks_geom_fwd.inc
--- a/skelsplat_amd/csrc/sks_geom_fwd.inc
+++ b/skelsplat_amd/csrc/sks_geom_fwd.inc
@@ -4,7 +4,8 @@
                                               const float* __restrict__ opac, const float* __restrict__ scales,
                                               const float* __restrict__ rots, const float* __restrict__ cov3Dp,
                                               float smod, unsigned flags, const Geom& g, int* __restrict__ radii,
-                                              int v, int idx, bool live, bool store = true)
+                                              int v, int idx, bool live, bool store = true,
+                                              float4* co_out = nullptr, float4* xyd_out = nullptr)
 {
     const size_t o = (size_t)v * P + (live ? idx : 0);
     const float* V = vms + 16 * v;
@@ -76,6 +77,8 @@
         g.xyd[o] = xyd;
         g.rect[o] = rect;
     }
+    if (co_out) *co_out = co;
+    if (xyd_out) *xyd_out = xyd;
     return rect;
 }
 
diff --git a/skelsplat_amd/csrc/sks_raster.hip b/skelsplat_amd/csrc/sks_raster.hip
--- a/skelsplat_amd/csrc/sks_raster.hip
+++ b/skelsplat_amd/csrc/sks_raster.hip
@@ -275,11 +275,12 @@
     return P >= 1 && P <= 64 && is_small(P, flags) && !(flags & (SKS_NO_NT_STORES | SKS_DEBUG_SYNC | SKS_BWD_LDS_LIST)) &&
            (W % 4 == 0 || (W % 4 == 2 && H % 2 == 0));
 }
-bool prefill_cut(PreFill& f, float* color, float* invdepth, int V, int C, int W, int H, int zid0, int nz, long long per_unit, long long max_units)
+bool prefill_cut(PreFill& f, float* color, float* invdepth, int V, int C, int W, int H, int zid0, int nz, long long per_unit, long long max_units,
+                 int pb_tune = 0)
 {
     const int gy = TileGrid(W, H).gy;
     const int passes = (TILE * W + fill_lead(color, invdepth, W, H) + 1023) / 1024;
-    const int pb = prefill_passes();
+    const int pb = pb_tune > 0 ? (pb_tune > 32 ? 32 : pb_tune) : prefill_passes();
     const int fsplit = (passes + pb - 1) / pb;
     const long long rows = (long long)fsplit * gy, nfill = rows * nz;
     if (zid0 < 0 || nz < 1 || zid0 + nz > (C + 1) * V || nfill * rows >= (1ll << 32) || (nfill + per_unit - 1) / per_unit > max_units) return false;
@@ -547,6 +548,71 @@
         }
     }
     STAGE_CHECK("render(binned)");
+    return 0;
+}
+
+inline int hosting_passes(unsigned flags, int W, int lead)
+{
+    const int tune = (int)((flags >> 8) & 0xff);
+    if (tune > 0) return tune > 32 ? 32 : tune;
+    const int passes = (TILE * W + lead + 1023) / 1024;
+    return passes / 8 > 2 ? (passes + 4) / 8 : 2;
+}
+inline bool hosting_possible(int P, int W, int H, unsigned flags) { return prefill_possible(P, W, H, flags) && !(flags & SKS_NO_HOSTED_FORWARD); }
+inline bool hosting_cut(PreFill& f, float* color, float* invdepth, int V, int P, int C, int W, int H, unsigned flags, int host_planes)
+{
+    const long long ncomp = (long long)composite_slots(flags, V, P) * P * V;
+    return prefill_cut(f, color, invdepth, V, C, W, H, 0, host_planes, 1, (1ll << 31) - 2 - ncomp, hosting_passes(flags, W, fill_lead(color, invdepth, W, H)));
+}
+
+int forward_hosting_impl(const FwdCall& c, float* other_color, float* other_invdepth, int host_planes)
+{
+    const Cameras& cam = c.cam;
+    const int V = cam.V, P = cam.P, C = cam.C, W = cam.W, H = cam.H;
+    const unsigned flags = c.g.flags;
+    if (int rc = check_common(cam)) return rc;
+    const hipStream_t st = c.stream;
+    const int planes = (C + 1) * V;
+    if (host_planes < 0 || host_planes > planes) return fail(-1, "sks_forward_hosting: host_planes=%d out of range [0,%d]", host_planes, planes);
+    if (!hosting_possible(P, W, H, flags))
+        return fail(-1, "sks_forward_hosting: no hosted forward for this call (wave-resident small path with 16-byte non-temporal stores only: "
+                        "1 <= P <= 64, W %% 4 == 0 or W %% 4 == 2 with an even H, no SKS_NO_NT_STORES / SKS_DEBUG_SYNC / SKS_FORCE_BINNED / "
+                        "SKS_NO_HOSTED_FORWARD)");
+    if (c.final_T || c.n_contrib) return fail(-1, "sks_forward_hosting: final_T / n_contrib are not available (sks_forward writes them)");
+    if (!c.io.out_color || !c.io.out_invdepth) return fail(-2, "out_color / out_invdepth must be provided");
+    if (((uintptr_t)c.io.out_color | (uintptr_t)c.io.out_invdepth) & 15u)
+        return fail(-2, "out_color / out_invdepth must be 16-byte aligned (the planes are written with 16-byte stores)");
+    if (int rc = require({ cam.viewmatrix, cam.projmatrix, cam.tanfovx, cam.tanfovy, c.g.means3D, c.g.features, c.g.opacities, c.io.radii, c.io.geom }))
+        return rc;
+    if (int rc = need_cov(c.g.scales, c.g.rotations, c.g.cov3D_precomp)) return rc;
+    PreFill f{};
+    if (host_planes > 0) {
+        if (!other_color || !other_invdepth) return fail(-2, "sks_forward_hosting: other_color / other_invdepth must be provided");
+        if (((uintptr_t)other_color | (uintptr_t)other_invdepth) & 15u) return fail(-2, "other_color / other_invdepth must be 16-byte aligned");
+        if (other_color == c.io.out_color || other_invdepth == c.io.out_invdepth)
+            return fail(-2, "sks_forward_hosting: the other set must not be the set the call renders into");
+        if (!hosting_cut(f, other_color, other_invdepth, V, P, C, W, H, flags, host_planes))
+            return fail(-1, "sks_forward_hosting: %d planes of %dx%d do not fit the launch", host_planes, W, H);
+    }
+    ViewTan vt;
+    fill_views(vt, nullptr, V, C, W, H, cam.tanfovx, cam.tanfovy, nullptr, nullptr);
+    Geom g = geom_from(c.io.geom, V, P, W, H);
+    g.cover = nullptr;
+    FwdArgs a{ P, C, W, H, flags, g, c.g.features, c.io.out_color, c.io.out_invdepth, nullptr, nullptr, composite_slots(flags, V, P),
+               ((1u << 20) + (unsigned)C) / (unsigned)(C + 1), 0, 0, fill_w_magic(W) };
+    a.ncomp = a.tslots * P * V;
+    const int cap = (P + 15) & ~15;
+    {
+        ProfScope prof(0, st, true, false);
+        with_cg(C, [&](auto cg) {
+            constexpr int CG = decltype(cg)::value;
+            const size_t lds = DynList<CG>::bytes(cap, CG) + HostGeomLds<CG>::bytes(cap, CG);
+            SKS_LAUNCH(prof, (k_render_fwd_hosting<CG>), dim3((unsigned)a.ncomp + f.nfill), dim3(256), lds, st, a, f, vt, cam.viewmatrix, cam.projmatrix,
+                       c.g.means3D, c.g.opacities, c.g.scales, c.g.rotations, c.g.cov3D_precomp, c.g.scale_modifier, c.io.radii);
+        });
+        prof_host_note(prof, st);
+    }
+    HIP_TRY(hipGetLastError());
     return 0;
 }
 
@@ -592,7 +658,9 @@
                 return fail(-1, "sks_backward_prefill: %d planes of %dx%d do not fit the geometry backward's launch", n_geom, W, H);
             have_pfg = true;
         }
-        if (prof_next_forward_sampled()) prof_park_begin(st);
+        if (!prof_host_begin(st) && prof_next_forward_sampled()) prof_park_begin(st);
+    } else {
+        prof_host_drop();
     }
     if ((phases & BWD_RENDER) && small) {
         ProfScope prof(1, st, true);
@@ -642,7 +710,7 @@
         if (gr.dL_dmeans3D_mean && (small || group < 0 || group == ng - 1))
             hipLaunchKernelGGL(k_mean_views, dim3((3 * P + 255) / 256), dim3(256), 0, st, V, P, gr.dL_dmeans3D, gr.dL_dmeans3D_mean);
     }
-    if (have_pfw || have_pfg) prof_park_end(st);
+    if (have_pfw || have_pfg) { prof_host_end(st); prof_park_end(st); }
     STAGE_CHECK("geometry-backward");
     return 0;
 }
@@ -828,6 +896,31 @@
     return 0;
 }
 
+int sks_hosting_planes(int V, int P, int C, int W, int H, unsigned flags, int* host_planes)
+{
+    if (!host_planes) return fail(-2, "sks_hosting_planes: host_planes must be provided");
+    *host_planes = 0;
+    int nw = 0, ng = 0;
+    if (int rc = sks_prefill_planes(V, P, C, W, H, flags, &nw, &ng)) return rc;
+    if (nw + ng == 0 || !hosting_possible(P, W, H, flags)) return 0;
+    const int hp = (C + 1) * V - nw - ng;
+    PreFill f;
+    if (hp > 0 && hosting_cut(f, nullptr, nullptr, V, P, C, W, H, flags, hp)) *host_planes = hp;
+    return 0;
+}
+
+int sks_forward_hosting(int V, int P, int C, int W, int H, const float* viewmatrix, const float* projmatrix,
+                        const float* tanfovx, const float* tanfovy, const float* means3D, const float* features,
+                        const float* opacities, const float* scales, const float* rotations, const float* cov3D_precomp,
+                        float scale_modifier, unsigned flags, float* out_color, float* out_invdepth, int* radii, void* geom,
+                        void* binning, size_t bin_capacity, int* num_rendered_dev, float* final_T, uint32_t* n_contrib,
+                        float* other_color, float* other_invdepth, int host_planes, void* stream)
+{
+    FwdCall c;
+    SKS_TAKE_FWD_CALL(c, final_T, n_contrib);
+    return forward_hosting_impl(c, other_color, other_invdepth, host_planes);
+}
+
 int sks_forward_backward(int V, int P, int C, int W, int H, const float* viewmatrix, const float* projmatrix,
                          const float* tanfovx, const float* tanfovy, const float* means3D, const float* features,
                          const float* opacities, const float* scales, const float* rotations, const float* cov3D_precomp,
@@ -1140,6 +1233,7 @@
     tl_prof->recorded = (on >> 18) & 1;
     tl_prof->seen[0] = tl_prof->seen[1] = 0;
     tl_prof->parked = false;
+    prof_host_drop();
     return 0;
 }
 
@@ -1164,6 +1258,7 @@
     *total_ms = tot;
     *launches = p.n;
     p.n = 0;
+    if (kind == 0) prof_host_drop();
     return 0;
 }
 
@@ -1191,6 +1286,7 @@
     *total_ms = tot;
     *launches = n;
     p.n = 0;
+    if (kind == 0) prof_host_drop();
     return 0;
 }
 
diff --git a/skelsplat_amd/rasterizer.py b/skelsplat_amd/rasterizer.py
--- a/skelsplat_amd/rasterizer.py
+++ b/skelsplat_amd/rasterizer.py
@@ -39,7 +39,7 @@
 
 class Workspace:
 
-    def __init__(self, prefill=None):
+    def __init__(self, prefill=None, hosted=None):
         self._t = {}
         self._plans = {}
         self._aux = {}
@@ -49,6 +49,9 @@
         self._prefill = prefill
         self._pf = None
         self._pf_off = prefill == 0
+        self._hosted = hosted
+        self.hosted_forwards = 0
+        self.recovery_fills = 0
 
     def aux_stream(self, dev_index):
         st = self._aux.get(dev_index)
@@ -92,16 +95,19 @@
 
 
 class _Prefill:
-    __slots__ = ("shape", "sets", "results", "cur", "note", "fargs", "bplan", "bargs", "rule")
+    __slots__ = ("shape", "sets", "results", "cur", "note", "front", "fargs", "hargs", "bplan", "bargs", "rule", "hrule", "misses")
 
     def __init__(self, shape, color, invdepth, radii, st, args):
         self.shape = shape
         self.sets = [(color, invdepth), None]
         self.results = [(color, invdepth, radii, st), None]
-        self.cur, self.note = 0, None
+        self.cur, self.note, self.front = 0, None, None
         self.fargs = list(args[:-1]) + [0, None]
+        self.hargs = list(args[:-1]) + [None, None, 0, None]
         self.bplan = self.bargs = None
         self.rule = {}
+        self.hrule = {}
+        self.misses = 0
 
 
 _PREFILL_MAX_SET_BYTES = 1 << 30
@@ -187,7 +193,7 @@
                 return plan.result
             del workspace._plans["fwd"]
     if workspace is not None and workspace._pf is not None:
-        workspace._pf.note = None
+        workspace._pf.note = workspace._pf.front = None
     if views.mixed:
         raise RuntimeError("the dense forward writes one (V,C,H,W) tensor: all views of the batch must share the image size")
     if means3D is None or means3D.dim() != 2 or means3D.shape[1] != 3:
@@ -270,6 +276,7 @@
 
 def _forward_two_sets(lib, workspace, pf, plan):
     note, pf.note = pf.note, None
+    pf.front = None
     args = plan.args
     if note is not None:
         if workspace._pf_off or torch.cuda.is_current_stream_capturing():
@@ -277,6 +284,20 @@
         elif note[1] == torch._C._cuda_getCurrentRawStream(plan.dev_index):
             other = 1 - pf.cur
             color, invdepth = pf.sets[other]
+            V, _P, C, _W, _H = pf.shape
+            hp = _hosted_planes(workspace, pf, args[_F_FLAGS])
+            if hp and note[0] >= (C + 1) * V:
+                hargs = pf.hargs
+                left = pf.sets[pf.cur]
+                hargs[_F_FLAGS], hargs[_F_COLOR], hargs[_F_INVDEPTH] = args[_F_FLAGS], color.data_ptr(), invdepth.data_ptr()
+                hargs[-4], hargs[-3], hargs[-2] = left[0].data_ptr(), left[1].data_ptr(), hp
+                rc = _replay(lib.sks_forward_hosting, hargs, plan.dev_index)
+                if rc == 0:
+                    pf.cur = other
+                    args[_F_COLOR], args[_F_INVDEPTH] = hargs[_F_COLOR], hargs[_F_INVDEPTH]
+                    pf.front, pf.misses = (hp, note[1]), 0
+                    workspace.hosted_forwards += 1
+                return rc
             fargs = pf.fargs
             fargs[_F_FLAGS], fargs[_F_COLOR], fargs[_F_INVDEPTH], fargs[-2] = args[_F_FLAGS], color.data_ptr(), invdepth.data_ptr(), note[0]
             rc = _replay(lib.sks_forward_prefilled, fargs, plan.dev_index)
@@ -294,7 +315,7 @@
     if pf is None or workspace._pf_off or plan.key[0] != id(pf.results[0][3]):
         return None
     if torch.cuda.is_current_stream_capturing():
-        workspace._pf_off, pf.note = True, None
+        workspace._pf_off, pf.note, pf.front = True, None, None
         return None
     fplan = workspace._plans.get("fwd")
     if fplan is None:
@@ -322,7 +343,38 @@
     rc = _replay(lib.sks_backward_prefill, bargs, plan.dev_index)
     if rc == 0:
         pf.note = (n[0] + n[1], bargs[-1])
+        if _hosted_planes(workspace, pf, fflags):
+            front = pf.front
+            V, _P, C, _W, _H = pf.shape
+            planes = (C + 1) * V
+            if front is not None and front[1] == bargs[-1] and front[0] + n[0] + n[1] >= planes:
+                pf.note = (planes, bargs[-1])
+            elif pf.misses < _HOSTED_MAX_MISSES:
+                color.zero_(), invdepth.zero_()
+                pf.front, pf.note = (planes, bargs[-1]), (planes, bargs[-1])
+                pf.misses += 1
+                workspace.recovery_fills += 1
     return rc
+
+
+_HOSTED_MAX_MISSES = 2
+_NO_HOSTED_ENV = os.environ.get("SKS_NO_HOSTED_FORWARD", "0") not in ("", "0")
+
+
+def _hosted_planes(workspace, pf, fflags):
+    hp = pf.hrule.get(fflags)
+    if hp is None:
+        V, P, C, W, H = pf.shape
+        if workspace._hosted is False or _NO_HOSTED_ENV or not _lib.HAS_HOSTING:
+            hp = 0
+        elif workspace._prefill is None:
+            hp = _lib.hosting_planes(V, P, C, W, H, fflags)
+        elif workspace._hosted and not fflags & (_lib.SKS_NO_HOSTED_FORWARD | _lib.SKS_NO_NT_STORES):
+            hp = max((C + 1) * V - sum(workspace._prefill), 0)
+        else:
+            hp = 0
+        pf.hrule[fflags] = hp
+    return hp
 
 
 def _replay_ticket(workspace, plan):
```

Result: slower. 68480 (-2.0%).
